# liuzuxin/FSRL

Measured on AMD Instinct MI355X. Metric: policy-updates/sec (PPO-Lagrangian update(), SafetyCarCircle-v0 shape, 256x256 MLP, 20k-step buffer), higher is better.
Workload: dtype f32; 1 GPU; configs[1] PPO-Lag update: repeat 4, clip 0.5, KL stop off, batch 256, N=20000 (20x1000), obs 8/act 2, 256x256; seeds_per_gpu=1, parallelism=independent agents x1

## Files before the change

### fsrl_amd/_lib.py

```python
import ctypes as C
import os

_HERE = os.path.dirname(os.path.abspath(__file__))
LIB_PATH = os.environ.get("FSRL_HIP_LIB") or os.path.join(_HERE, "libfsrl_hip.so")

FSRL_OK, FSRL_EINVAL, FSRL_ENOMEM, FSRL_EHIP, FSRL_ESTATE = 0, -22, -12, -5, -1
PPO_NSTATS = 11
ALGO_PPO_LAG, ALGO_TRPO_LAG, ALGO_CPO, ALGO_SAC_LAG, ALGO_FOCOPS = 0, 1, 2, 3, 4


class Config(C.Structure):
    _fields_ = [("algo", C.c_int32), ("obs_dim", C.c_int32), ("act_dim", C.c_int32),
                ("hidden", C.c_int32), ("n_critics", C.c_int32), ("env_num", C.c_int32),
                ("buffer_size", C.c_int64), ("max_action", C.c_float), ("gamma", C.c_double),
                ("gae_lambda", C.c_double), ("eps_clip", C.c_float), ("dual_clip", C.c_float),
                ("vf_coef", C.c_float), ("max_grad_norm", C.c_float), ("target_kl", C.c_float),
                ("norm_adv", C.c_int32), ("use_lagrangian", C.c_int32), ("lr", C.c_float),
                ("beta1", C.c_float), ("beta2", C.c_float), ("adam_eps", C.c_float), ("recompute_adv", C.c_int32),
                ("unbounded", C.c_int32), ("rew_norm", C.c_int32), ("value_clip", C.c_int32),
                ("hidden1", C.c_int32), ("hidden2", C.c_int32),
                ("n_hidden", C.c_int32), ("hidden_sizes", C.c_int32 * 8), ("force_layered", C.c_int32)]


class ShmEnv(C.Structure):
# ... 11 lines not shown
                ("cost_limit", C.c_double)]


class SacConfig(C.Structure):
    _fields_ = [("actor_lr", C.c_float), ("critic_lr", C.c_float), ("alpha_lr", C.c_float), ("tau", C.c_float),
                ("alpha", C.c_float), ("target_entropy", C.c_float), ("n_step", C.c_int32),
                ("auto_alpha", C.c_int32), ("use_lagrangian", C.c_int32), ("deterministic", C.c_int32),
                ("exploration_sigma", C.c_float), ("actor_mean", C.c_int32)]


class FocopsConfig(C.Structure):
    _fields_ = [("actor_lr", C.c_float), ("critic_lr", C.c_float), ("l2_reg", C.c_float), ("delta", C.c_float),
                ("eta", C.c_float), ("tem_lambda", C.c_float), ("max_grad_norm", C.c_float)]


class CvpoConfig(C.Structure):
    _fields_ = [("actor_lr", C.c_float), ("critic_lr", C.c_float), ("tau", C.c_float), ("n_step", C.c_int32),
                ("double_critic", C.c_int32), ("sample_act_num", C.c_int32), ("estep_iter_num", C.c_int32),
                ("mstep_iter_num", C.c_int32), ("estep_kl", C.c_float), ("estep_dual_max", C.c_float),
                ("estep_dual_lr", C.c_float), ("mstep_kl_mu", C.c_float), ("mstep_kl_std", C.c_float),
                ("mstep_dual_max", C.c_float), ("mstep_dual_lr", C.c_float), ("qc_thres", C.c_double),
                ("actor_mean", C.c_int32)]


class DevEnvConfig(C.Structure):
    _fields_ = [("kind", C.c_int32), ("env_num", C.c_int32), ("obs_dim", C.c_int32), ("act_dim", C.c_int32),
                ("max_episode_steps", C.c_int32), ("seed", C.c_uint64), ("p", C.c_float * 8), ("A", C.c_void_p), ("B", C.c_void_p)]


DEVENV_POINT_CIRCLE, DEVENV_LINEAR = 0, 1

ACTOR_MEAN_DEFAULT, ACTOR_MEAN_UNBOUNDED, ACTOR_MEAN_TANH = 0, 1, 2


def actor_mean_code(unbounded):
    if unbounded is None:
        return ACTOR_MEAN_DEFAULT
    return ACTOR_MEAN_UNBOUNDED if bool(unbounded) else ACTOR_MEAN_TANH


CPO_NSTATS, TRPO_NSTATS, SAC_NSTATS, FOCOPS_NSTATS, CVPO_NSTATS = 17, 11, 10, 8, 17

_P = C.POINTER
_f, _d, _u8, _i32, _i64 = _P(C.c_float), _P(C.c_double), _P(C.c_uint8), _P(C.c_int32), _P(C.c_int64)
_ctx = C.c_void_p

SIGNATURES = {
    "fsrl_last_error": (C.c_char_p, []),
    "fsrl_config_default": (None, [_P(Config)]),
    "fsrl_ctx_create": (C.c_int, [C.c_int, _P(Config), _P(_ctx)]),
    "fsrl_ctx_destroy": (C.c_int, [_ctx]),
    "fsrl_sync": (C.c_int, [_ctx]),
    "fsrl_param_count": (C.c_int64, [_ctx]),
    "fsrl_params_set": (C.c_int, [_ctx, _f, C.c_int64]),
    "fsrl_params_get": (C.c_int, [_ctx, _f, C.c_int64]),
    "fsrl_grads_get": (C.c_int, [_ctx, _f, C.c_int64]),
    "fsrl_optim_reset": (C.c_int, [_ctx]),
    "fsrl_state_snapshot": (C.c_int, [_ctx]),
    "fsrl_state_restore": (C.c_int, [_ctx]),
    "fsrl_train_state_size": (C.c_int64, [_ctx, C.c_int32]),
    "fsrl_train_state_export": (C.c_int, [_ctx, C.c_int32, C.c_void_p, C.c_int64, _i64]),
    "fsrl_train_state_import": (C.c_int, [_ctx, C.c_void_p, C.c_int64]),
    "fsrl_train_state_copy": (C.c_int, [_ctx, _ctx, C.c_int32]),
    "fsrl_ret_rms_get": (C.c_int, [_ctx, _d, C.c_int32]),
    "fsrl_ret_rms_set": (C.c_int, [_ctx, _d, C.c_int32]),
    "fsrl_set_lr": (C.c_int, [_ctx, C.c_int32, C.c_float]),
    "fsrl_get_lr": (C.c_float, [_ctx, C.c_int32]),
    "fsrl_ppo_abort": (C.c_int, [_ctx]),
    "fsrl_store_push": (C.c_int, [_ctx, _i32, C.c_int32, _f, _f, _d, _d, _u8, _u8, _f, _i64, _d, _i32, _i64]),
    "fsrl_store_reset": (C.c_int, [_ctx, C.c_int]),
    "fsrl_store_len": (C.c_int64, [_ctx]),
    "fsrl_store_read": (C.c_int, [_ctx, _i64, C.c_int64, _f, _f, _d, _d, _u8, _u8, _f]),
    "fsrl_store_configure": (C.c_int, [_ctx, C.c_int64, C.c_int32]),
    "fsrl_store_geometry": (C.c_int, [_ctx, _i64, _i32]),
    "fsrl_store_sample0": (C.c_int, [_ctx, _i64, C.c_int64, _i64]),
    "fsrl_actor_forward": (C.c_int, [_ctx, _f, C.c_int32, _f, _f]),
    "fsrl_ppo_begin": (C.c_int, [_ctx, _d, C.c_double, C.c_int32, _i64]),
    "fsrl_ppo_pass": (C.c_int, [_ctx, _i64, C.c_uint64, _i32]),
    "fsrl_ppo_pass_result": (C.c_int, [_ctx, _i32]),
    "fsrl_ppo_end": (C.c_int, [_ctx, _f, C.c_int64, _i64]),
    "fsrl_ppo_update": (C.c_int, [_ctx, _d, C.c_double, C.c_int32, C.c_int32, _i64, C.c_uint64, _f,
                                  C.c_int64, _i64, _i32]),
    "fsrl_ppo_set_plan": (C.c_int, [_ctx, C.c_int32]),
    "fsrl_batch_get": (C.c_int, [_ctx, C.c_char_p, _f, C.c_int64]),
    "fsrl_group_create": (C.c_int, [_P(_ctx), C.c_int32, _P(_ctx)]),
    "fsrl_group_destroy": (C.c_int, [_ctx]),
    "fsrl_group_set_plan": (C.c_int, [_ctx, C.c_int32]),
    "fsrl_group_ppo_update": (C.c_int, [_ctx, _d, _d, C.c_int32, C.c_int32, _P(_i64), C.c_uint64, _P(_f), C.c_int64, _i64,
                                        _i32]),
    "fsrl_group_ppo_update_each": (C.c_int, [_ctx, _d, _d, _i32, _i32, _P(_i64), C.c_uint64, _P(_f), _i64, _i64, _i32]),
    "fsrl_group_collect_step": (C.c_int, [_ctx, _i32, _i32, _f, _f, _d, _d, _u8, _u8, _f, _i64, _d, _i32, _i64, _i32, _f, C.c_int32,
                                          C.c_int32, _f, _f, _f, _f]),
    "fsrl_group_actor_set_resident": (C.c_int, [_ctx, C.c_int32, C.c_double]),
    "fsrl_group_actor_resident_stats": (C.c_int, [_ctx, _i64]),
    "fsrl_group_actor_release": (C.c_int, [_ctx]),
    "fsrl_sac_group_create": (C.c_int, [_P(_ctx), C.c_int32, _P(_ctx)]),
    "fsrl_sac_group_destroy": (C.c_int, [_ctx]),
    "fsrl_sac_group_update": (C.c_int, [_ctx, C.c_int32, _i32, _d, _d]),
    "fsrl_cvpo_group_create": (C.c_int, [_P(_ctx), C.c_int32, _P(_ctx)]),
    "fsrl_cvpo_group_destroy": (C.c_int, [_ctx]),
    "fsrl_cvpo_group_update": (C.c_int, [_ctx, C.c_int32, _i32]),
    "fsrl_collect_group_create": (C.c_int, [_P(_ctx), C.c_int32, _P(_ctx)]),
    "fsrl_collect_group_destroy": (C.c_int, [_ctx]),
    "fsrl_collect_group_step": (C.c_int, [_ctx, _i32, _i32, _f, _f, _d, _d, _u8, _u8, _f, _i64, _d, _i32, _i64, _i32, _f, C.c_int32,
                                          C.c_int32, _f, _f, _f, _f]),
    "fsrl_collect_group_actor_set_resident": (C.c_int, [_ctx, C.c_int32, C.c_double]),
    "fsrl_collect_group_actor_resident_stats": (C.c_int, [_ctx, _i64]),
    "fsrl_collect_group_actor_release": (C.c_int, [_ctx]),
    "fsrl_group_collect_episodes": (C.c_int, [_ctx, _P(_P(ShmEnv)), _i32, _i32, _f, _i32, C.c_int32, C.c_int32, _f, _f, _i64, _d, _i32,
                                              _i32, _d, _i32, _i32, _d, _i32]),
    "fsrl_collect_episodes_group": (C.c_int, [_ctx, _P(_P(ShmEnv)), _i32, _i32, _f, _i32, C.c_int32, C.c_int32, _f, _f, _i64, _d, _i32,
                                              _i32, _d, _i32, _i32, _d, _i32]),
    "fsrl_gae_return": (C.c_int, [_ctx, _f, _f, _d, _u8, C.c_int64, C.c_double, C.c_double, _d]),
    "fsrl_nstep_return": (C.c_int, [_ctx, _d, _u8, C.c_int64, _f, _i64, C.c_int64, C.c_int64, C.c_double, C.c_int32, _d]),
    "fsrl_launch_floors": (C.c_int, [_ctx, C.c_int32, C.c_int32, _d]),
    "fsrl_tr_begin": (C.c_int, [_ctx, _P(TrConfig), _i64]),
    "fsrl_cpo_learn": (C.c_int, [_ctx, C.c_double, C.c_int32, _f]),
    "fsrl_trpo_learn": (C.c_int, [_ctx, _d, C.c_double, C.c_int32, _f]),
    "fsrl_cpo_learn_mb": (C.c_int, [_ctx, C.c_double, C.c_int32, C.c_int32, _i64, C.c_uint64, _f, C.c_int64, _i64]),
    "fsrl_trpo_learn_mb": (C.c_int, [_ctx, _d, C.c_double, C.c_int32, C.c_int32, _i64, C.c_uint64, _f, C.c_int64, _i64]),
    "fsrl_tr_linesearch_evals": (C.c_int32, [_ctx, _i32, C.c_int32]),
    "fsrl_actor_param_count": (C.c_int64, [_ctx]),
    "fsrl_tr_grad": (C.c_int, [_ctx, C.c_int32, _f, C.c_int64]),
    "fsrl_tr_hvp": (C.c_int, [_ctx, _f, _f, C.c_int64]),
    "fsrl_tr_hvp_cached": (C.c_int, [_ctx, _f, _f, C.c_int64]),
    "fsrl_tr_cg": (C.c_int, [_ctx, _f, C.c_int64, C.c_float, C.c_int32, C.c_float, _f, _i32, _f]),
    "fsrl_tr_eval": (C.c_int, [_ctx, _d]),
    "fsrl_tr_set_plan": (C.c_int, [_ctx, C.c_int32, C.c_int32, C.c_int32]),
    "fsrl_tr_set_tile_split": (C.c_int, [_ctx, C.c_int32, C.c_int32]),
    "fsrl_tr_set_co_delay": (C.c_int, [_ctx, C.c_int32, C.c_int32]),
    "fsrl_focops_init": (C.c_int, [_ctx, _P(FocopsConfig)]),
    "fsrl_focops_set_plan": (C.c_int, [_ctx, C.c_int32]),
    "fsrl_focops_set_nu": (C.c_int, [_ctx, C.c_double, C.c_double]),
    "fsrl_sac_init": (C.c_int, [_ctx, _P(SacConfig)]),
    "fsrl_sac_set_plan": (C.c_int, [_ctx, C.c_int32]),
    "fsrl_sac_param_count": (C.c_int64, [_ctx, C.c_int32]),
    "fsrl_sac_params_set": (C.c_int, [_ctx, _f, C.c_int64, _f, C.c_int64, C.c_float]),
    "fsrl_sac_params_put": (C.c_int, [_ctx, C.c_int32, _f, C.c_int64]),
    "fsrl_sac_params_get": (C.c_int, [_ctx, C.c_int32, _f, C.c_int64, _f]),
    "fsrl_sac_update": (C.c_int, [_ctx, C.c_int32, _i64, _f, _f, C.c_uint64, _d, C.c_double, _f]),
    "fsrl_actor_sample": (C.c_int, [_ctx, _f, C.c_int32, C.c_int32, C.c_uint64, _f]),
    "fsrl_collect_step": (C.c_int, [_ctx, _i32, C.c_int32, _f, _f, _d, _d, _u8, _u8, _f, _i64, _d, _i32, _i64,
                                    _f, C.c_int32, C.c_int32, C.c_int32, _f, _f, _f, _f]),
    "fsrl_collect_episodes": (C.c_int, [_ctx, _P(ShmEnv), _i32, C.c_int32, _f, C.c_int32, C.c_int32, C.c_int32, _f, _f, _i64, _d, _i32,
                                        _i32, _d, _i32, _i32]),
    "fsrl_collect_episodes_split": (C.c_int, [_ctx, _P(ShmEnv), _i32, C.c_int32, _f, C.c_int32, C.c_int32, C.c_int32, _f, _f, _i64, _d, _i32,
                                              _i32, _d, _i32, _i32]),
    "fsrl_collect_timing": (C.c_int, [_ctx, _d]),
    "fsrl_actor_set_resident": (C.c_int, [_ctx, C.c_int32, C.c_double]),
    "fsrl_actor_resident_stats": (C.c_int, [_ctx, _i64]),
    "fsrl_actor_release": (C.c_int, [_ctx]),
    "fsrl_collect_run": (C.c_int, [_ctx, _P(ShmEnv), _i32, C.c_int32, _f, _f, _f, C.c_int32, C.c_int32, _f, _f, C.c_int32, _i32, _d, _d, _d,
                                  _u8, _u8, _f]),
    "fsrl_store_sizes": (C.c_int, [_ctx, _i64, C.c_int32]),
    "fsrl_sac_stats_drain": (C.c_int64, [_ctx, _f, C.c_int64]),
    "fsrl_sac_last_sample": (C.c_int, [_ctx, _i64, _f, _f, C.c_int32]),
    "fsrl_sac_last_chain": (C.c_int, [_ctx, _i64, _u8, C.c_int32]),
    "fsrl_per_enable": (C.c_int, [_ctx, C.c_double, C.c_double, C.c_int32]),
    "fsrl_per_set_beta": (C.c_int, [_ctx, C.c_double]),
    "fsrl_per_update_weight": (C.c_int, [_ctx, _i64, _d, C.c_int64]),
    "fsrl_per_state": (C.c_int, [_ctx, _d, C.c_int64, _d, _d, _d]),
    "fsrl_per_last_weights": (C.c_int, [_ctx, _f, C.c_int32]),
    "fsrl_per_last_td": (C.c_int, [_ctx, _f, C.c_int32]),
    "fsrl_sac_actor_forward": (C.c_int, [_ctx, _f, C.c_int32, _f, _f]),
    "fsrl_cvpo_init": (C.c_int, [_ctx, _P(CvpoConfig)]),
    "fsrl_cvpo_pre_update": (C.c_int, [_ctx]),
# ... 76 lines not shown
```

### fsrl_amd/csrc/common.hpp

```cpp
#pragma once
#include <hip/hip_runtime.h>
#include <stdint.h>

#include "../../include/fsrl_hip.h"

#define FSRL_MAX_NETS (1 + FSRL_MAX_CRITICS)
#define FSRL_TILE_M 16
#define FSRL_DOW 32
#define FSRL_MAX_OBS 128
#define FSRL_MAX_ACT 16
#define FSRL_W1_LDS 16
#define FSRL_RD 64
#define FSRL_RD_LOGP 16
#define FSRL_RD_ADV 17
#define FSRL_RD_RET 21
#define FSRL_RD_VOLD 25
#define FSRL_RD_MEAN 32
#define FSRL_RD_STD 48

typedef float f32x4 __attribute__((ext_vector_type(4)));
typedef float f32x2 __attribute__((ext_vector_type(2)));

struct NetOff {
    int sigma;
    int W1, b1, W2, b2, W3, b3;
    int W2f;
    int out;
    int begin, end;
};

struct ModelDesc {
    int Do, Da, H, n_nets;
    int unbounded;
    NetOff net[FSRL_MAX_NETS];
};

__host__ __device__ __forceinline__ int w2f_index(int H, int n, int k) {
    return ((((n >> 4) * (H >> 4) + (k >> 4)) * 64) + ((k >> 2) & 3) * 16 + (n & 15)) * 4 + (k & 3);
}
__device__ __forceinline__ int w2f_mirror_of(const ModelDesc& md, int i) {
    const int HH = md.H * md.H;
    for (int net = 0; net < md.n_nets; ++net) {
        const int o = i - md.net[net].W2;
        if ((unsigned)o < (unsigned)HH) return md.net[net].W2f + w2f_index(md.H, o / md.H, o % md.H);
    }
    return -1;
}

struct PpoStepArgs {
    int mb_start;
    int mb_size;
    int step;
    int mb_index;
    int last_in_pass;
    int first_in_pass;
    int iters_in_pass;
    int pass;
    float rescale;
    float lam[FSRL_MAX_CRITICS];
    float eps_clip, dual_clip, vf_coef, max_action, max_grad_norm, target_kl;
    int norm_adv, use_lagrangian;
    float lr, beta1, beta2, adam_eps;
    float one_minus_b1, one_minus_b2;
    double kl_thresh;
    float step_size;
    float bc2_sqrt;
    int value_clip;
    int fuse_adam;
    int xcd_pair;
    int dbg_phase;
};
#ifdef FSRL_PROBES
#define FSRL_PROBE(sa, n) ((sa).dbg_phase == (n))
#define FSRL_TS(buf, k) do { if ((buf) && threadIdx.x == 0) (buf)[(size_t)blockIdx.x * 16 + (k)] = __builtin_readcyclecounter(); } while (0)
#else
#define FSRL_PROBE(sa, n) false
#define FSRL_TS(buf, k) do { } while (0)
#endif

__device__ __forceinline__ void ppo_adam_math(const float g, float& m, float& v, float& p, const PpoStepArgs& sa) {
#pragma clang fp contract(off)
    m = fmaf(sa.one_minus_b1, g - m, m);
    v = v * sa.beta2;
    v = fmaf(sa.one_minus_b2 * g, g, v);
    const float denom = sqrtf(v) / sa.bc2_sqrt + sa.adam_eps;
    p = p + (-sa.step_size * m) / denom;
}

struct CtrlBlock {
    int stopped_after;
    int pad;
    double kl_sum;
    float last_grad_norm;
    float pad2;
};

__device__ __forceinline__ f32x4 mfma_16x16x4(float a, float b, f32x4 c) {
    return __builtin_amdgcn_mfma_f32_16x16x4f32(a, b, c, 0, 0, 0);
}

__device__ __forceinline__ f32x4 mfma_4x4x1(float a, float b, f32x4 c) {
    return __builtin_amdgcn_mfma_f32_4x4x1f32(a, b, c, 0, 0, 0);
}

__device__ __forceinline__ void store4_next(float* p, const f32x4 v) {
    asm volatile("global_store_dwordx4 %0, %1, off sc1\n\ts_nop 1" ::"v"(p), "v"(v) : "memory");
}
#ifdef FSRL_FB_PLAIN_STORES
__device__ __forceinline__ void store4_fb(float* p, const f32x4 v) { *reinterpret_cast<f32x4*>(p) = v; }
#else
__device__ __forceinline__ void store4_fb(float* p, const f32x4 v) { store4_next(p, v); }
#endif

__host__ __device__ __forceinline__ unsigned div_magic(const int d) { return d > 1 ? 0xFFFFFFFFu / (unsigned)d + 1u : 0u; }
__device__ __forceinline__ int div_by_magic(const unsigned e, const unsigned magic) { return magic ? (int)__umulhi(e, magic) : (int)e; }

#ifndef WG3_NO_BUFFER
typedef unsigned wg3_u32x4 __attribute__((ext_vector_type(4)));
struct Wg3Buf { __amdgpu_buffer_rsrc_t r; };
__device__ __forceinline__ Wg3Buf wg3_buf(const float* base) {
    Wg3Buf b; b.r = __builtin_amdgcn_make_buffer_rsrc(const_cast<float*>(base), 0, 0x7FFFFFFF, 0x00020000); return b;
}
__device__ __forceinline__ Wg3Buf wg3_buf_here(const float* base) {
    unsigned long long p = (unsigned long long)base;
    asm volatile("" : "+s"(p));
    return wg3_buf(reinterpret_cast<const float*>(p));
}
__device__ __forceinline__ f32x4 wg3_ld4(const Wg3Buf& b, const unsigned off_floats) {
    return __builtin_bit_cast(f32x4, __builtin_amdgcn_raw_buffer_load_b128(b.r, off_floats * 4u, 0, 0));
}
__device__ __forceinline__ float wg3_ld1(const Wg3Buf& b, const unsigned off_floats) {
    return __builtin_bit_cast(float, __builtin_amdgcn_raw_buffer_load_b32(b.r, off_floats * 4u, 0, 0));
}
__device__ __forceinline__ float wg3_ld1s(const Wg3Buf& b, const unsigned lane_off_floats, const unsigned uni_off_floats) {
    return __builtin_bit_cast(float, __builtin_amdgcn_raw_buffer_load_b32(b.r, lane_off_floats * 4u, uni_off_floats * 4u, 0));
}
__device__ __forceinline__ f32x4 wg3_ld4s(const Wg3Buf& b, const unsigned lane_off_floats, const unsigned uni_off_floats) {
    return __builtin_bit_cast(f32x4, __builtin_amdgcn_raw_buffer_load_b128(b.r, lane_off_floats * 4u, uni_off_floats * 4u, 0));
}
#else
struct Wg3Buf { const float* p; };
__device__ __forceinline__ Wg3Buf wg3_buf(const float* base) { Wg3Buf b; b.p = base; return b; }
__device__ __forceinline__ Wg3Buf wg3_buf_here(const float* base) { return wg3_buf(base); }
__device__ __forceinline__ f32x4 wg3_ld4(const Wg3Buf& b, const unsigned off_floats) { return *reinterpret_cast<const f32x4*>(b.p + off_floats); }
__device__ __forceinline__ float wg3_ld1(const Wg3Buf& b, const unsigned off_floats) { return b.p[off_floats]; }
__device__ __forceinline__ float wg3_ld1s(const Wg3Buf& b, const unsigned l, const unsigned u) { return b.p[l + u]; }
__device__ __forceinline__ f32x4 wg3_ld4s(const Wg3Buf& b, const unsigned l, const unsigned u) { return *reinterpret_cast<const f32x4*>(b.p + l + u); }
#endif

__device__ __forceinline__ float wave_sum(float v) {
#pragma unroll
    for (int o = 32; o > 0; o >>= 1) v += __shfl_xor(v, o, 64);
    return v;
}

__device__ __forceinline__ double wave_sum_d(double v) {
#pragma unroll
    for (int o = 32; o > 0; o >>= 1) v += __shfl_xor(v, o, 64);
    return v;
}
```

### fsrl_amd/csrc/fsrl_hip.hip

```cpp
#include <hip/hip_runtime.h>

#include <climits>
#include <cstddef>
#include <cmath>
#include <cstdarg>
#include <cstdio>
#include <cstdlib>
#include <cstring>
#include <algorithm>
#include <functional>
#include <string>
#include <vector>

#include "kernels_misc.hpp"
#include "kernels_mlp.hpp"
#include "kernels_fb.hpp"
#include "kernels_fbco.hpp"
#include "kernels_wgrad2.hpp"
#include "kernels_wgrad3.hpp"
#include "kernels_layered.hpp"
#include "kernels_focops_group.hpp"
#include "resident_ring.hpp"
#include "host_decisions.hpp"

static thread_local std::string g_err;
static int fail(int code, const char* fmt, ...) {
    char buf[512];
    va_list ap;
    va_start(ap, fmt);
    vsnprintf(buf, sizeof(buf), fmt, ap);
    va_end(ap);
    g_err = buf;
    return code;
}
#define HIPCHK(expr)                                                                        \
    do {                                                                                    \
        hipError_t _e = (expr);                                                             \
        if (_e != hipSuccess)                                                               \
            return fail(FSRL_EHIP, "%s failed: %s (%s:%d)", #expr, hipGetErrorString(_e),   \
                        __FILE__, __LINE__);                                                \
    } while (0)
#define CHECK_ARG(cond, ...) \
    do { if (!(cond)) return fail(FSRL_EINVAL, __VA_ARGS__); } while (0)

extern "C" const char* fsrl_last_error(void) { return g_err.c_str(); }

static inline int round_up(int x, int m) { return (x + m - 1) / m * m; }

struct TensorMap {
    int api_off, dev_off, rows, cols, dev_ld;
    int n() const { return rows * cols; }
    void to_dev(float* dev, const float* api) const {
        for (int r = 0; r < rows; ++r) memcpy(dev + dev_off + (size_t)r * dev_ld, api + api_off + (size_t)r * cols, (size_t)cols * 4);
    }
    void to_api(float* api, const float* dev) const {
        for (int r = 0; r < rows; ++r) memcpy(api + api_off + (size_t)r * cols, dev + dev_off + (size_t)r * dev_ld, (size_t)cols * 4);
    }
};

struct EnvBook {
    int64_t index = 0, size = 0, last_index = 0;
    int64_t staged = 0;
    double ep_rew = 0.0;
    int32_t ep_len = 0;
    int64_t ep_idx = 0;
};

struct Staging {
    uint8_t* h = nullptr;
    uint8_t* d = nullptr;
    int count = 0;
    hipEvent_t done = nullptr;
    bool in_flight = false;
};
static inline size_t stage_rec_bytes(int Do, int Da) { return ((size_t)24 + 4 * (size_t)(2 * Do + Da) + 7) / 8 * 8; }

struct fsrl_group;
struct fsrl_ctx {
    fsrl_config cfg{};
    fsrl_group* group = nullptr;
    struct CommState* comm = nullptr;
    int device = 0;
    hipStream_t compute = nullptr, side = nullptr;
    ModelDesc md{};
    std::vector<TensorMap> tmap;
    int h1 = 0, h2 = 0;
    int64_t n_api = 0;
    int n_dev = 0;
    int n_alloc = 0;
    float *P = nullptr, *M = nullptr, *V = nullptr, *G = nullptr;
    int64_t adam_t = 0;
    CtrlBlock* ctrl = nullptr;
    CtrlBlock* h_ctrl = nullptr;
    bool verdict_pending = false;

    int64_t sub_size = 0, maxsize = 0;
    float* mbstat = nullptr; size_t mbstat_cap = 0;
    double* d_rms = nullptr;
    double* ret64 = nullptr; int64_t ret64_cap = 0;
    int64_t alloc_rows = 0;
    int active_envs = 0;
    std::vector<EnvBook> env;
    std::vector<uint8_t> h_flags;
    StorePtrs st{};
    static constexpr int STAGE_CAP = 4096;
    Staging stage[2];
    int cur_stage = 0;
    hipEvent_t store_ready = nullptr;

    BatchPtrs b{};
    int* d_indices = nullptr; uint8_t* d_end = nullptr; int* d_seg = nullptr;
    int* h_indices = nullptr; uint8_t* h_end = nullptr; int* h_seg = nullptr;
    float *values = nullptr, *vnext = nullptr, *advs = nullptr, *rets = nullptr, *logp_old = nullptr;
    int64_t N = 0;
    int n_seg = 0;
    bool batch_ready = false;

    int batch_size = 0, mbp_max = 0, n_tiles_max = 0;
    float *A1 = nullptr, *A2 = nullptr, *D1 = nullptr, *D2 = nullptr, *DO = nullptr;
    float *obs_p = nullptr, *rd_p = nullptr;
    float *statp = nullptr, *gsq_part = nullptr;
    int *d_perm = nullptr, *h_perm = nullptr;
    int *d_mbstart = nullptr, *d_mbsize = nullptr, *h_mbplan = nullptr;
    size_t mb_cap = 0;
    std::vector<int> mb_start, mb_size;
    float* d_stats = nullptr; int64_t stats_cap = 0;
    int64_t n_steps = 0;
    int pass_index = 0;
    double lagr[FSRL_MAX_CRITICS] = {0, 0, 0, 0};
    double rescaling = 1.0;
    bool in_update = false;

    void* scratch = nullptr; size_t scratch_bytes = 0;

    bool profiling = false;
    hipEvent_t ev_a = nullptr, ev_b = nullptr, ev_c = nullptr;
    std::vector<hipEvent_t> k_ev;
    size_t k_ev_used = 0;
    double t_process_ms = 0, t_learn_ms = 0, t_fwdbwd_ms = 0, t_fwdbwd_raw_ms = 0;
    int64_t n_fwdbwd = 0;
    uint64_t rng[4] = {0x9E3779B97F4A7C15ull, 0xBF58476D1CE4E5B9ull, 0x94D049BB133111EBull, 1};
    uint64_t shuffle_rng[4] = {0xD6E8FEB86659FD93ull, 0xA0761D6478BD642Full, 0xE7037ED1A0B428DBull, 2};
    struct Parts { int stride = 0; float* p = nullptr; size_t floats = 0; } parts[3];
    float* wg_parts = nullptr;
    int n_cus = 256;
    bool wgrad_xcd = false;
    bool wgrad_stream = false;
    int wgrad_tiles = 1;
    struct FocState* foc = nullptr;
    float* mu_old = nullptr;
    float* sigma_old = nullptr;
    void* h_actor = nullptr; size_t h_actor_bytes = 0;
    int actor_k = 0; size_t actor_ob = 0, actor_mb = 0;
    unsigned* h_done = nullptr; int done_cap = 0;
    unsigned actor_seq = 0; int actor_blocks = 0;
    ResidentRing pa;
    bool pa_req = false;
    int pa_cap = 0;
    void* h_pa = nullptr;
    int probe_phase = 0, probe_wgrad_skip = 0;
    unsigned long long* probe_ts = nullptr;
    bool probe_tile16 = false;
    struct fsrl_sac_group* sac_group = nullptr;
    struct fsrl_cvpo_group* cvpo_group = nullptr;
    struct fsrl_collect_group* cgroup = nullptr;
    int tall_tiles = -1;
    bool no_fuse_adam = false;
    bool no_w2b_early = false;
    bool no_xcd_pair = false;
    bool no_spin = false;
    std::vector<float> act_mu, act_sg;
    std::vector<int> perm_tmp;
    hipEvent_t perm_copied = nullptr; bool perm_in_flight = false;
    uint64_t store_version = 1;
    uint64_t joined_version = 0;
    double t_collect_env = 0.0, t_collect_act = 0.0;
    float* snap = nullptr;
    int64_t snap_adam_t = 0, snap_critic_t = 0, snap_foc_a = 0, snap_foc_c = 0; bool snap_valid = false;
    struct LayState* lay = nullptr;
    struct TrState* tr = nullptr;
    uint64_t theta_version = 1;
    void* sac = nullptr;
    struct fsrl_tap* tap = nullptr;
    struct PerState* per = nullptr;
};
static bool ctx_is_replay(const fsrl_ctx* c);
static void sac_free(fsrl_ctx* c);
static void tr_free(fsrl_ctx* c);
static void foc_free(fsrl_ctx* c);
static void tr_reset_optim(fsrl_ctx* c);
static int64_t tr_critic_steps_taken(fsrl_ctx* c);
static void tr_set_critic_steps(fsrl_ctx* c, int64_t t);
static void foc_steps(fsrl_ctx* c, int64_t* t_actor, int64_t* t_critic, bool set);
static void foc_reset_optim(fsrl_ctx* c);
static void group_detach(fsrl_ctx* c);
static void lay_free(fsrl_ctx* c);
static void lay_build_layout(fsrl_ctx* c, const int* widths, int L);
static int lay_ensure_mb(fsrl_ctx* c, int B);
static int lay_ppo_steps(fsrl_ctx* c);
struct InferArgs;
static int lay_infer(fsrl_ctx* c, const InferArgs& ia, int jobs_y, hipStream_t s);
static void comm_free(fsrl_ctx* c);
static inline bool tap_closed(const fsrl_ctx* c, int e);
static void tap_row(fsrl_ctx* c, int e, int i, const float* act, double rew, double cost, uint8_t fl);
static int tap_flush(fsrl_ctx* c, int w, const uint8_t* recs_d, int stage_rec, int k);
static void tap_ctx_gone(fsrl_ctx* c);
static int per_ingest(fsrl_ctx* c, const uint8_t* recs_d, int rec, int k);
static int per_store_reset(fsrl_ctx* c);
static void per_free(fsrl_ctx* c);
static int focops_pass(fsrl_ctx* c, int32_t* stopped_out);
static int pass_verdict(fsrl_ctx* c, int32_t* stopped_out);

static int flush_stage(fsrl_ctx* c);
static void pactor_release(fsrl_ctx* c);
static void group_actor_release(fsrl_group* g);
static void sac_group_detach(fsrl_ctx* c);
static void cvpo_group_detach(fsrl_ctx* c);
static void collect_group_detach(fsrl_ctx* c);
static void collect_group_actor_release(struct fsrl_collect_group* g);
static int focops_group_check(fsrl_ctx* const* ctxs, int k);
struct GroupUpdate;
static int focops_group_update(GroupUpdate& u);
#define ENTER_DEV(c) do { HIPCHK(hipSetDevice((c)->device)); pactor_release(c); } while (0)

static int join_store(fsrl_ctx* c) {
    if (c->joined_version == c->store_version) return 0;
    int rc = flush_stage(c);
    if (rc) return rc;
    HIPCHK(hipEventRecord(c->store_ready, c->side));
    HIPCHK(hipStreamWaitEvent(c->compute, c->store_ready, 0));
    c->joined_version = c->store_version;
    return 0;
}

static int ensure_scratch(fsrl_ctx* c, size_t bytes) {
    if (c->scratch_bytes >= bytes) return 0;
    if (c->scratch) HIPCHK(hipFree(c->scratch));
    c->scratch = nullptr; c->scratch_bytes = 0;
    HIPCHK(hipMalloc(&c->scratch, bytes));
    c->scratch_bytes = bytes;
    return 0;
}

template <class T>
struct DevTable { T *d = nullptr, *h = nullptr; size_t cap = 0; };
template <class T>
static int table_ensure(DevTable<T>& t, size_t need, size_t grow_to, hipStream_t sync = nullptr) {
    if (need <= t.cap) return 0;
    if (sync) HIPCHK(hipStreamSynchronize(sync));
    if (t.d) HIPCHK(hipFree(t.d));
    if (t.h) HIPCHK(hipHostFree(t.h));
// ... 101 lines not shown
        wa.out = c->wg_parts; wa.split_stride = stride; wa.ks_per_split = rps / 4;
        *nsplit = ns;
        hipLaunchKernelGGL((fb_wgrad2_kernel<256, PAIR2>), dim3(8 * WG2_Q * ((ns + 7) / 8), ny), dim3(1024), 0, c->compute, md, wa, ns, rps);
        HIPCHK(hipGetLastError());
        return 0;
    }
    const WgradBlocks wb = wgrad_blocks(md.Do, H_, PAIR2);
    const int passes = wb.passes, NB = wb.NB;
    const WgradPlan pl = wgrad_plan(wa.rows, NB * ny, c->n_cus);
    int rc = ensure_parts(c, stride, pl.nsplit);
    if (rc) return rc;
    wa.out = c->wg_parts; wa.ks_per_split = pl.ks_per_split; wa.split_stride = stride;
    wa.dbg_skip = c->probe_wgrad_skip;
    wa.aux_passes = passes;
    *nsplit = pl.nsplit;
    return dispatch_H(c->cfg.hidden, [&](auto hc) {
        constexpr int HH = decltype(hc)::value;
        if (xcd_order < 0 ? c->wgrad_xcd : xcd_order != 0) {
            wa.remap_total = NB * ny * pl.nsplit; wa.remap_ny = ny;
            hipLaunchKernelGGL((fb_wgrad_kernel<HH, PAIR2>), dim3(round_up(wa.remap_total, 8)), dim3(1024), 0, c->compute, md, wa, NoRider{});
        } else if (rider && !PAIR2) {
            const int blocks = (rider->sa.B + SG_ROWS - 1) / SG_ROWS;
            rider->x0 = NB; rider->nx = (blocks + ny * pl.nsplit - 1) / (ny * pl.nsplit);
            hipLaunchKernelGGL((fb_wgrad_kernel<HH, false, SgRider>), dim3(NB + rider->nx, ny, pl.nsplit), dim3(1024), 0, c->compute, md, wa, *rider);
            if (rider_done) *rider_done = true;
        } else
        hipLaunchKernelGGL((fb_wgrad_kernel<HH, PAIR2>), dim3(NB, ny, pl.nsplit), dim3(1024), 0, c->compute, md, wa, NoRider{});
        HIPCHK(hipGetLastError());
        return 0;
    });
}

extern "C" void fsrl_config_default(fsrl_config* c) {
    memset(c, 0, sizeof(*c));
    c->algo = FSRL_ALGO_PPO_LAG;
    c->obs_dim = 8; c->act_dim = 2; c->hidden = 128; c->n_critics = 2;
    c->env_num = 20; c->buffer_size = 100000; c->max_action = 1.0f;
    c->gamma = 0.99; c->gae_lambda = 0.95; c->eps_clip = 0.2f; c->dual_clip = 0.0f;
    c->vf_coef = 0.25f; c->max_grad_norm = 0.0f; c->target_kl = 0.02f;
    c->norm_adv = 1; c->use_lagrangian = 1;
    c->lr = 5e-4f; c->beta1 = 0.9f; c->beta2 = 0.999f; c->adam_eps = 1e-8f;
}

static void build_layout(fsrl_ctx* c) {
    const int Do = c->cfg.obs_dim, Da = c->cfg.act_dim, H = c->cfg.hidden;
    ModelDesc& md = c->md;
    md.Do = Do; md.Da = Da; md.H = H; md.n_nets = 1 + c->cfg.n_critics;
    md.unbounded = (c->cfg.unbounded && c->cfg.algo != FSRL_ALGO_SAC_LAG) ? 1 : 0;
    const int h1 = c->h1, h2 = c->h2;
    int api = 0, dev = 0;
    auto add = [&](int rows, int cols, int dev_ld, int dev_n) {
        TensorMap t{api, dev, rows, cols, dev_ld};
        c->tmap.push_back(t);
        api += rows * cols;
        dev = round_up(dev + dev_n, 64);
        return t.dev_off;
    };
    for (int net = 0; net < md.n_nets; ++net) {
        NetOff& no = md.net[net];
        no.begin = dev;
        const int out = (net == 0) ? Da : 1;
        no.out = out;
        no.sigma = (net == 0) ? add(1, Da, Da, Da) : -1;
        no.W1 = add(h1, Do, Do, H * Do); no.b1 = add(1, h1, H, H);
        no.W2 = add(h2, h1, H, H * H);   no.b2 = add(1, h2, H, H);
        no.W3 = add(out, h2, H, out * H); no.b3 = add(1, out, out, out);
        no.end = dev;
    }
    c->n_api = api;
    c->n_dev = round_up(dev, 1024);
    for (int net = 0; net < md.n_nets; ++net) md.net[net].W2f = c->n_dev + net * H * H;
    c->n_alloc = c->n_dev + md.n_nets * H * H;
}

static void fill_mirrors(const ModelDesc& md, std::vector<float>& v) {
    const int H = md.H;
    for (int net = 0; net < md.n_nets; ++net) {
        const NetOff& no = md.net[net];
        for (int n = 0; n < H; ++n)
            for (int k = 0; k < H; ++k) v[(size_t)no.W2f + w2f_index(H, n, k)] = v[(size_t)no.W2 + (size_t)n * H + k];
    }
}

extern "C" int fsrl_ctx_destroy(fsrl_ctx* c) {
    if (!c) return 0;
    (void)hipSetDevice(c->device);
    pactor_release(c);
    (void)hipDeviceSynchronize();
    if (c->group) group_detach(c);
    if (c->sac_group) sac_group_detach(c);
    if (c->cvpo_group) cvpo_group_detach(c);
    if (c->cgroup) collect_group_detach(c);
    if (c->tap) tap_ctx_gone(c);
    comm_free(c);
    tr_free(c);
    sac_free(c);
    per_free(c);
    foc_free(c);
    lay_free(c);
    if (c->h_actor) (void)hipHostFree(c->h_actor);
    if (c->h_done) (void)hipHostFree(c->h_done);
    if (c->h_pa) (void)hipHostFree(c->h_pa);
    if (c->mbstat) (void)hipFree(c->mbstat);
    if (c->d_rms) (void)hipFree(c->d_rms);
    if (c->ret64) (void)hipFree(c->ret64);
    if (c->mu_old) (void)hipFree(c->mu_old);
    if (c->sigma_old) (void)hipFree(c->sigma_old);
    if (c->snap) (void)hipFree(c->snap);
    void* dptrs[] = {c->P, c->M, c->V, c->G, c->ctrl, c->st.obs, c->st.obs_next, c->st.act, c->st.rew,
                     c->st.cost, c->st.flags, c->b.obs, c->b.obs_next, c->b.act, c->b.rew, c->b.cost,
                     c->b.flags, c->d_indices, c->d_end, c->d_seg, c->values, c->vnext, c->advs,
                     c->rets, c->logp_old, c->A1, c->A2, c->D1, c->D2, c->DO, c->obs_p, c->rd_p, c->statp,
                     c->gsq_part, c->d_perm, c->d_mbstart, c->d_mbsize, c->d_stats,
                     c->scratch};
    for (void* p : dptrs) if (p) (void)hipFree(p);
    for (auto& pp : c->parts) if (pp.p) (void)hipFree(pp.p);
    void* hptrs[] = {c->h_ctrl, c->h_indices, c->h_end, c->h_seg, c->h_perm, c->h_mbplan};
    for (void* p : hptrs) if (p) (void)hipHostFree(p);
    for (auto& s : c->stage) {
        if (s.h) (void)hipHostFree(s.h);
        if (s.d) (void)hipFree(s.d);
        if (s.done) (void)hipEventDestroy(s.done);
    }
    for (hipEvent_t e : {c->store_ready, c->ev_a, c->ev_b, c->ev_c, c->perm_copied}) if (e) (void)hipEventDestroy(e);
    for (hipEvent_t e : c->k_ev) (void)hipEventDestroy(e);
    if (c->compute) (void)hipStreamDestroy(c->compute);
    if (c->side) (void)hipStreamDestroy(c->side);
    delete c;
    return 0;
}

extern "C" int fsrl_ctx_create(int device_id, const fsrl_config* cfg, fsrl_ctx** out) {
    CHECK_ARG(cfg && out, "null argument");
    CHECK_ARG(cfg->algo == FSRL_ALGO_PPO_LAG || cfg->algo == FSRL_ALGO_SAC_LAG || cfg->algo == FSRL_ALGO_CPO ||
                  cfg->algo == FSRL_ALGO_TRPO_LAG || cfg->algo == FSRL_ALGO_FOCOPS, "unknown algo %d", cfg->algo);
    CHECK_ARG(cfg->obs_dim >= 1 && cfg->obs_dim <= FSRL_MAX_OBS, "obs_dim must be in [1,%d]", FSRL_MAX_OBS);
    CHECK_ARG(cfg->act_dim >= 1 && cfg->act_dim <= FSRL_MAX_ACT, "act_dim must be in [1,%d]", FSRL_MAX_ACT);
    CHECK_ARG(cfg->n_hidden >= 0 && cfg->n_hidden <= FSRL_MAX_HIDDEN, "n_hidden must be in [0, %d]", FSRL_MAX_HIDDEN);
    bool layered = false;
    int n_hid1 = cfg->hidden1, n_hid2 = cfg->hidden2;
    if (cfg->n_hidden > 0) {
        CHECK_ARG(cfg->hidden1 == 0 && cfg->hidden2 == 0, "give hidden_sizes[n_hidden] or hidden1 / hidden2, not both");
        for (int l = 0; l < cfg->n_hidden; ++l)
            CHECK_ARG(cfg->hidden_sizes[l] >= 1 && cfg->hidden_sizes[l] <= FSRL_MAX_WIDTH, "hidden_sizes[%d] = %d outside [1, %d]", l,
                      cfg->hidden_sizes[l], FSRL_MAX_WIDTH);
        if (cfg->n_hidden == 2 && cfg->hidden_sizes[0] <= 256 && cfg->hidden_sizes[1] <= 256 && !cfg->force_layered) {
            n_hid1 = cfg->hidden_sizes[0]; n_hid2 = cfg->hidden_sizes[1];
        } else {
            layered = true;
        }
    } else {
        CHECK_ARG(!cfg->force_layered, "force_layered needs hidden_sizes[n_hidden]");
    }
    const int h1_ = layered ? 0 : (n_hid1 > 0 ? n_hid1 : cfg->hidden), h2_ = layered ? 0 : (n_hid2 > 0 ? n_hid2 : cfg->hidden);
    if (!layered) {
        CHECK_ARG((n_hid1 > 0) == (n_hid2 > 0), "hidden1 and hidden2 are given together (0, 0 = two layers of `hidden`)");
        CHECK_ARG(h1_ >= 1 && h1_ <= 256 && h2_ >= 1 && h2_ <= 256, "hidden layer widths must be in [1, 256] (two hidden layers)");
    }
    const int Hpad_ = layered ? 0 : std::max(h1_, h2_) <= 64 ? 64 : std::max(h1_, h2_) <= 128 ? 128 : 256;
    CHECK_ARG(layered || n_hid1 == 0 || cfg->hidden == 0 || cfg->hidden == Hpad_ ,
              "hidden = %d does not fit hidden1 / hidden2 = %d / %d (leave hidden 0 or give %d)", cfg->hidden, h1_, h2_, Hpad_);
    CHECK_ARG(!layered || cfg->n_critics < 1 || cfg->n_critics > FSRL_MAX_CRITICS ||
                  (1 + cfg->n_critics) * (cfg->n_hidden + 1) + 1 <= LAY_MAX_JOBS,
              "layered context: (1 + n_critics) * (n_hidden + 1) + 1 = %d weight-gradient jobs exceed the job table of %d "
              "(n_critics = %d, n_hidden = %d)", (1 + cfg->n_critics) * (cfg->n_hidden + 1) + 1, LAY_MAX_JOBS, cfg->n_critics, cfg->n_hidden);
    CHECK_ARG(cfg->n_critics >= 1 && cfg->n_critics <= 2,
              "n_critics must be 1 or 2 (reward [+ one cost], get_metrics base_policy.py:377-382)");
    CHECK_ARG(cfg->env_num >= 1 && cfg->buffer_size >= cfg->env_num, "bad env_num/buffer_size");
    CHECK_ARG(cfg->gamma >= 0.0 && cfg->gamma <= 1.0, "discount factor should be in [0, 1].");
    CHECK_ARG(cfg->gae_lambda >= 0.0 && cfg->gae_lambda <= 1.0, "GAE lambda should be in [0, 1].");
    CHECK_ARG(cfg->dual_clip == 0.0f || cfg->dual_clip > 1.0f,
              "Dual-clip PPO parameter should greater than 1.0.");
    CHECK_ARG(cfg->buffer_size + cfg->env_num < (int64_t)INT_MAX / 2, "buffer too large for 32-bit slot ids");
    CHECK_ARG(cfg->rew_norm || !cfg->value_clip, "value clip is available only when `reward_normalization` is True");
    CHECK_ARG(!cfg->value_clip || cfg->algo == FSRL_ALGO_PPO_LAG, "value_clip is a PPO-Lagrangian option (ppo_lag.py:158-164)");
    CHECK_ARG(!cfg->rew_norm || cfg->algo != FSRL_ALGO_SAC_LAG, "reward_normalization acts on GAE returns: on-policy contexts only");
    int ndev = 0;
    HIPCHK(hipGetDeviceCount(&ndev));
    CHECK_ARG(device_id >= 0 && device_id < ndev, "device %d not present (%d devices)", device_id, ndev);
    HIPCHK(hipSetDevice(device_id));
    int n_cus_probe = 256;
    (void)hipDeviceGetAttribute(&n_cus_probe, hipDeviceAttributeMultiprocessorCount, device_id);
    fsrl_ctx* c = new fsrl_ctx();
    c->cfg = *cfg;
    c->cfg.hidden = Hpad_;
    c->h1 = h1_; c->h2 = h2_;
    c->device = device_id;
    c->n_cus = n_cus_probe > 0 ? n_cus_probe : 256;
    c->probe_tile16 = getenv("FSRL_TILE16") != nullptr;
    c->no_w2b_early = getenv("FSRL_NO_W2B_EARLY") != nullptr;
#ifdef FSRL_PROBES
    { const char* e = getenv("FSRL_DBG_PHASE"); c->probe_phase = e ? atoi(e) : 0; }
    { const char* e = getenv("FSRL_WGRAD_SKIP"); c->probe_wgrad_skip = e ? atoi(e) : 0; }
    c->no_spin = getenv("FSRL_NO_SPIN") != nullptr;
    c->no_xcd_pair = getenv("FSRL_NO_XCD_PAIR") != nullptr;
    c->no_fuse_adam = getenv("FSRL_NO_FUSE_ADAM") != nullptr;
    if (getenv("FSRL_TSTAMP")) {
        (void)hipMalloc(&c->probe_ts, 1024 * 16 * sizeof(unsigned long long));
        (void)hipMemset(c->probe_ts, 0, 1024 * 16 * sizeof(unsigned long long));
    }
#endif
    if (layered) lay_build_layout(c, cfg->hidden_sizes, cfg->n_hidden);
    else build_layout(c);
#define TRY(expr) do { hipError_t _e = (expr); if (_e != hipSuccess) { fail(FSRL_EHIP, "%s failed: %s", #expr, hipGetErrorString(_e)); fsrl_ctx_destroy(c); return FSRL_EHIP; } } while (0)
    TRY(hipStreamCreateWithFlags(&c->compute, hipStreamNonBlocking));
    TRY(hipStreamCreateWithFlags(&c->side, hipStreamNonBlocking));
    const size_t pb = (size_t)c->n_dev * sizeof(float);
    TRY(hipMalloc(&c->P, (size_t)c->n_alloc * sizeof(float))); TRY(hipMemsetAsync(c->P, 0, (size_t)c->n_alloc * sizeof(float), c->compute));
    TRY(hipMalloc(&c->M, pb)); TRY(hipMalloc(&c->V, pb)); TRY(hipMalloc(&c->G, pb));
    TRY(hipMemsetAsync(c->M, 0, pb, c->compute)); TRY(hipMemsetAsync(c->V, 0, pb, c->compute)); TRY(hipMemsetAsync(c->G, 0, pb, c->compute));
    TRY(hipMalloc(&c->ctrl, sizeof(CtrlBlock)));
    if (cfg->rew_norm) {
        TRY(hipMalloc(&c->d_rms, 3 * FSRL_MAX_CRITICS * sizeof(double)));
        double init[3 * FSRL_MAX_CRITICS];
        for (int i = 0; i < FSRL_MAX_CRITICS; ++i) { init[3 * i] = 0.0; init[3 * i + 1] = 1.0; init[3 * i + 2] = 0.0; }
        TRY(hipMemcpy(c->d_rms, init, sizeof(init), hipMemcpyHostToDevice));
    }
    TRY(hipHostMalloc(&c->h_ctrl, sizeof(CtrlBlock)));
    c->sub_size = (cfg->buffer_size + cfg->env_num - 1) / cfg->env_num;
    c->maxsize = c->sub_size * cfg->env_num;
    c->alloc_rows = c->maxsize + cfg->env_num; c->active_envs = cfg->env_num;
    c->env.resize(cfg->env_num);
    c->h_flags.assign((size_t)c->alloc_rows, 0);
    const size_t ms = (size_t)c->alloc_rows;
    const int Do = cfg->obs_dim, Da = cfg->act_dim;
    TRY(hipMalloc(&c->st.obs, ms * Do * 4)); TRY(hipMalloc(&c->st.obs_next, ms * Do * 4));
    TRY(hipMalloc(&c->st.act, ms * Da * 4)); TRY(hipMalloc(&c->st.rew, ms * 8));
    TRY(hipMalloc(&c->st.cost, ms * 8)); TRY(hipMalloc(&c->st.flags, ms));
    TRY(hipMalloc(&c->b.obs, ms * Do * 4)); TRY(hipMalloc(&c->b.obs_next, ms * Do * 4));
    TRY(hipMalloc(&c->b.act, ms * Da * 4)); TRY(hipMalloc(&c->b.rew, ms * 8));
    TRY(hipMalloc(&c->b.cost, ms * 8)); TRY(hipMalloc(&c->b.flags, ms));
    TRY(hipMalloc(&c->d_indices, ms * 4)); TRY(hipMalloc(&c->d_end, ms)); TRY(hipMalloc(&c->d_seg, (ms + 2) * 4));
    TRY(hipHostMalloc(&c->h_indices, ms * 4)); TRY(hipHostMalloc(&c->h_end, ms)); TRY(hipHostMalloc(&c->h_seg, (ms + 2) * 4));
    const int C = cfg->n_critics;
    TRY(hipMalloc(&c->values, ms * C * 4)); TRY(hipMalloc(&c->vnext, ms * C * 4));
    TRY(hipMalloc(&c->advs, ms * C * 4)); TRY(hipMalloc(&c->rets, ms * C * 4));
    TRY(hipMalloc(&c->logp_old, ms * 4));
    TRY(hipMalloc(&c->d_perm, ms * 4)); TRY(hipHostMalloc(&c->h_perm, ms * 4));
    TRY(hipMalloc(&c->obs_p, (ms + 32) * Do * 4)); TRY(hipMemsetAsync(c->obs_p, 0, (ms + 32) * Do * 4, c->compute));
    TRY(hipMalloc(&c->rd_p, (ms + 32) * FSRL_RD * 4)); TRY(hipMemsetAsync(c->rd_p, 0, (ms + 32) * FSRL_RD * 4, c->compute));
    TRY(hipStreamSynchronize(c->compute));
    for (auto& s : c->stage) {
        const size_t k = fsrl_ctx::STAGE_CAP;
        TRY(hipHostMalloc(&s.h, k * stage_rec_bytes(Do, Da)));
        TRY(hipMalloc(&s.d, k * stage_rec_bytes(Do, Da)));
        TRY(hipEventCreateWithFlags(&s.done, hipEventDisableTiming));
    }
    TRY(hipEventCreateWithFlags(&c->store_ready, hipEventDisableTiming));
    TRY(hipEventCreate(&c->ev_a)); TRY(hipEventCreate(&c->ev_b)); TRY(hipEventCreate(&c->ev_c));
    TRY(hipEventCreateWithFlags(&c->perm_copied, hipEventDisableTiming));
    CtrlBlock init{INT_MAX, 0, 0.0, 0.0f, 0.0f};
    TRY(hipMemcpy(c->ctrl, &init, sizeof(init), hipMemcpyHostToDevice));
#undef TRY
    *out = c;
    return 0;
}

extern "C" int fsrl_sync(fsrl_ctx* c) {
    CHECK_ARG(c, "null ctx");
    ENTER_DEV(c);
    HIPCHK(hipStreamSynchronize(c->side));
    HIPCHK(hipStreamSynchronize(c->compute));
    return 0;
}

extern "C" int64_t fsrl_param_count(const fsrl_ctx* c) { return c ? c->n_api : 0; }

static int copy_flat(fsrl_ctx* c, float* dev, float* host_out, const float* host_in, int64_t n) {
    CHECK_ARG(n == c->n_api, "expected %lld parameters, got %lld", (long long)c->n_api, (long long)n);
    ENTER_DEV(c);
    std::vector<float> tmp((size_t)c->n_dev, 0.0f);
    if (host_in) {
        for (const TensorMap& t : c->tmap) t.to_dev(tmp.data(), host_in);
// ... 831 lines not shown
```

### fsrl_amd/csrc/host_decisions.hpp

```cpp
#pragma once
#include <stdint.h>
#include <algorithm>
#include <cmath>
#include <functional>
#include <queue>
#include <vector>

static constexpr float CPO_EPS = 1e-8f;
static inline bool cpo_cost_solve_skipped(float bb, float c_value) { return bb <= CPO_EPS && c_value < 0; }
struct CpoDual { int ocase; float A, B, lam, nu; };
static inline CpoDual cpo_dual_solve(float s_q, float s_r, float s_s, float c_value, float delta, float bb) {
    const float EPS = CPO_EPS;
    float A = 0.f, B = 0.f, lam, nu;
    int ocase = 4;
    if (!cpo_cost_solve_skipped(bb, c_value)) {
        A = s_q - s_r * s_r / s_s;
        B = 2.0f * delta - c_value * c_value / s_s;
        if (c_value < 0 && B < 0) ocase = 3;
        else if (c_value < 0 && B >= 0) ocase = 2;
        else if (c_value >= 0 && B >= 0) ocase = 1;
        else ocase = 0;
    }
    if (ocase == 3 || ocase == 4) {
        lam = std::sqrt(s_q / (2.0f * delta));
// ... 31 lines not shown
    for (int bt = 0; bt < max_backtracks; ++bt) {
        ++r.evals;
        if (try_step(r.beta)) break;
        r.beta *= coeff;
    }
    return r;
}
struct TrpoSearch { float step; int evals; };
template <class Try>
static TrpoSearch trpo_line_search(float step, float coeff, int max_backtracks, Try&& try_step) {
    TrpoSearch r{step, 0};
    for (int i = 0; i < max_backtracks; ++i) {
        ++r.evals;
        if (try_step(r.step)) break;
        else if (i < max_backtracks - 1) r.step *= coeff;
        else r.step = 0.0f;
    }
    return r;
}

static inline void split_plan(int n, int B, std::vector<int>& st, std::vector<int>& sz) {
    st.clear(); sz.clear();
    const bool merge = (n % B) > 0;
    for (int i = 0; i < n; i += B) {
        if (merge && i + 2 * B >= n) { st.push_back(i); sz.push_back(n - i); break; }
        st.push_back(i); sz.push_back(std::min(B, n - i));
    }
}

static inline uint64_t rotl64(uint64_t x, int k) { return (x << k) | (x >> (64 - k)); }
static inline uint64_t xoshiro_next(uint64_t* s) {
    const uint64_t result = rotl64(s[1] * 5, 7) * 9, t = s[1] << 17;
    s[2] ^= s[0]; s[3] ^= s[1]; s[1] ^= s[2]; s[0] ^= s[3]; s[2] ^= t; s[3] = rotl64(s[3], 45);
    return result;
}
enum { PERM_OK = 0, PERM_RANGE, PERM_TWICE };
struct PermFill { int code, index; long long value; };
static inline PermFill perm_fill(int* out, int n, const int64_t* perm, uint64_t* rng, uint64_t seed) {
    if (perm) {
        std::vector<uint8_t> seen((size_t)n, 0);
        for (int i = 0; i < n; ++i) {
            if (!(perm[i] >= 0 && perm[i] < n)) return {PERM_RANGE, i, (long long)perm[i]};
            if (seen[(size_t)perm[i]]) return {PERM_TWICE, i, (long long)perm[i]};
            seen[(size_t)perm[i]] = 1;
            out[i] = (int)perm[i];
        }
        return {PERM_OK, 0, 0};
    }
    if (seed) { rng[0] ^= seed; rng[1] += seed * 0x9E3779B97F4A7C15ull; }
    for (int i = 0; i < n; ++i) out[i] = i;
    for (int i = n - 1; i > 0; --i) std::swap(out[i], out[(int)(xoshiro_next(rng) % (uint64_t)(i + 1))]);
    return {PERM_OK, 0, 0};
}

struct TileSplit { int n32, n16; };
static inline TileSplit mixed_split(int64_t N, int ny, int n_cus, double rho) {
    const int max32 = (int)((N + 31) / 32);
    double best = 1e300; int best32 = 0, best16 = (int)((N + 15) / 16);
    std::vector<double> cu((size_t)std::max(n_cus, 1));
    for (int n32 = 0; n32 <= max32; ++n32) {
        const int64_t rem = N - 32 * (int64_t)n32;
        const int n16 = rem > 0 ? (int)((rem + 15) / 16) : 0;
        if (n16 > 0 && n32 == max32) continue;
        std::fill(cu.begin(), cu.end(), 0.0);
        std::priority_queue<double, std::vector<double>, std::greater<double>> pq(cu.begin(), cu.end());
        double span = 0.0;
        for (int b = 0; b < ny * n32; ++b) { const double e = pq.top() + 1.0; pq.pop(); pq.push(e); span = std::max(span, e); }
        for (int b = 0; b < ny * n16; ++b) { const double e = pq.top() + rho; pq.pop(); pq.push(e); span = std::max(span, e); }
        if (span < best - 1e-9 || (std::fabs(span - best) <= 1e-9 && n32 > best32)) { best = span; best32 = n32; best16 = n16; }
    }
    return {best32, best16};
}
static inline void co_plan(int64_t N, int n_wgs, int* n32_out, int* n16_out) {
    const int64_t tail_rows = std::min<int64_t>(N, 16 * (int64_t)(n_wgs / 2));
    const int n32 = (int)((N - tail_rows) / 32);
    const int64_t rem = N - 32 * (int64_t)n32;
    *n32_out = n32; *n16_out = (int)((rem + 15) / 16);
}
static inline void forced_split(int64_t N, int want32, int* n32_out, int* n16_out) {
    const int n32 = (int)std::min<int64_t>(want32, N / 32);
    const int64_t rem = N - 32 * (int64_t)n32;
    *n32_out = n32; *n16_out = (int)((rem + 15) / 16);
}
```

### fsrl_amd/csrc/host_ppo.inc

```
static int launch_gae(fsrl_ctx* c);
static int perm_upload(fsrl_ctx* c, int n, const int64_t* perm, uint64_t seed) {
    c->perm_tmp.resize((size_t)n);
    const PermFill pf = perm_fill(c->perm_tmp.data(), n, perm, c->shuffle_rng, seed);
    CHECK_ARG(pf.code != PERM_RANGE, "perm[%d]=%lld out of range", pf.index, pf.value);
    CHECK_ARG(pf.code != PERM_TWICE, "perm is not a permutation: %lld appears twice", pf.value);
    if (c->perm_in_flight) { HIPCHK(hipEventSynchronize(c->perm_copied)); c->perm_in_flight = false; }
    memcpy(c->h_perm, c->perm_tmp.data(), (size_t)n * 4);
    HIPCHK(hipMemcpyAsync(c->d_perm, c->h_perm, (size_t)n * 4, hipMemcpyHostToDevice, c->compute));
    HIPCHK(hipEventRecord(c->perm_copied, c->compute));
    c->perm_in_flight = true;
    return 0;
}

static int ensure_ppo_buffers(fsrl_ctx* c, int B) {
    const int mbp = round_up(2 * B, 32);
    if (mbp <= c->mbp_max) return 0;
    HIPCHK(hipStreamSynchronize(c->compute));
    for (float** p : {&c->A1, &c->A2, &c->D1, &c->D2, &c->DO, &c->statp, &c->gsq_part})
        if (*p) { HIPCHK(hipFree(*p)); *p = nullptr; }
    const int H = c->cfg.hidden, nn = c->md.n_nets;
    const size_t act = (size_t)nn * mbp * H * 4;
    HIPCHK(hipMalloc(&c->A1, act)); HIPCHK(hipMalloc(&c->A2, act));
    HIPCHK(hipMalloc(&c->D1, act)); HIPCHK(hipMalloc(&c->D2, act));
    HIPCHK(hipMalloc(&c->DO, (size_t)nn * mbp * FSRL_DOW * 4));
    HIPCHK(hipMalloc(&c->statp, (size_t)(mbp / 4) * nn * 4 * 4));
    HIPCHK(hipMalloc(&c->gsq_part, (size_t)std::max(wg_grid(H, nn), c->n_dev / 256 + 2) * 4));
    c->mbp_max = mbp;
    c->n_tiles_max = mbp / 16;
    return 0;
}

extern "C" int fsrl_ppo_set_plan(fsrl_ctx* c, int32_t tall_tiles) {
    CHECK_ARG(c, "null ctx");
    CHECK_ARG(tall_tiles >= -1 && tall_tiles <= 4096, "tall_tiles: -1 (automatic), 0 (none) or a count");
    c->tall_tiles = tall_tiles;
    return 0;
}

extern "C" int fsrl_ppo_begin(fsrl_ctx* c, const double* lagrangians, double rescaling,
                              int32_t batch_size, int64_t* n_out) {
    CHECK_ARG(c, "null ctx");
    CHECK_ARG(batch_size >= 1, "batch_size must be >= 1");
    CHECK_ARG(!c->in_update, "fsrl_ppo_begin called twice without fsrl_ppo_end");
    ENTER_DEV(c);
    int rc = flush_stage(c);
    if (rc) return rc;
    HIPCHK(hipEventRecord(c->store_ready, c->side));
    HIPCHK(hipStreamWaitEvent(c->compute, c->store_ready, 0));
    const int C = c->cfg.n_critics;
    for (int i = 0; i < FSRL_MAX_CRITICS; ++i) c->lagr[i] = 0.0;
    if (c->cfg.use_lagrangian && C > 1) {
        CHECK_ARG(lagrangians, "lags and values length must be equal");
        for (int i = 0; i < C - 1; ++i) c->lagr[i] = lagrangians[i];
    }
    c->rescaling = rescaling;
    c->batch_size = batch_size;
    const int64_t n = sample0(c, c->h_indices, c->h_end);
    c->N = n;
    if (n_out) *n_out = n;
    c->n_steps = 0;
    c->pass_index = 0;
    c->in_update = true;
    c->verdict_pending = false;
    c->t_fwdbwd_ms = 0; c->n_fwdbwd = 0; c->k_ev_used = 0;
    CtrlBlock init{INT_MAX, 0, 0.0, 0.0f, 0.0f};
    *c->h_ctrl = init;
    hipStream_t s = c->compute;
    HIPCHK(hipMemcpyAsync(c->ctrl, c->h_ctrl, sizeof(CtrlBlock), hipMemcpyHostToDevice, s));
    if (n == 0) { c->batch_ready = true; return 0; }
    int nseg = 0;
    c->h_seg[nseg++] = 0;
    for (int64_t i = 0; i + 1 < n; ++i) if (c->h_end[i]) c->h_seg[nseg++] = (int)i + 1;
    c->h_seg[nseg] = (int)n;
    HIPCHK(hipEventRecord(c->ev_a, s));
    HIPCHK(hipMemcpyAsync(c->d_indices, c->h_indices, (size_t)n * 4, hipMemcpyHostToDevice, s));
    HIPCHK(hipMemcpyAsync(c->d_end, c->h_end, (size_t)n, hipMemcpyHostToDevice, s));
    HIPCHK(hipMemcpyAsync(c->d_seg, c->h_seg, (size_t)(nseg + 1) * 4, hipMemcpyHostToDevice, s));
    const int Do = c->cfg.obs_dim, Da = c->cfg.act_dim;
    {
        const size_t work = (size_t)n * (2 * Do + Da + 1);
        const int blocks = (int)std::min<size_t>(2048, (work + 255) / 256);
        hipLaunchKernelGGL(batch_gather_kernel, dim3(blocks), dim3(256), 0, s, c->st, c->b, c->d_indices,
                           c->d_end, (int)n, Do, Da);
        HIPCHK(hipGetLastError());
    }
    InferArgs ia{};
    ia.obs = c->b.obs; ia.obs_next = c->b.obs_next; ia.act = c->b.act; ia.flags = c->b.flags;
    ia.values = c->values; ia.vnext = c->vnext; ia.logp_old = c->logp_old; ia.mu_out = nullptr;
    if (c->cfg.algo == FSRL_ALGO_FOCOPS) {
        if (!c->mu_old) {
            HIPCHK(hipMalloc(&c->mu_old, (size_t)c->alloc_rows * Da * 4));
            HIPCHK(hipMalloc(&c->sigma_old, FSRL_MAX_ACT * 4));
        }
        ia.mu_out = c->mu_old;
        HIPCHK(hipMemcpyAsync(c->sigma_old, c->P + c->md.net[0].sigma, (size_t)Da * 4, hipMemcpyDeviceToDevice, s));
    }
    ia.N = (int)n; ia.C = C; ia.max_action = c->cfg.max_action;
    rc = launch_infer(c, ia, 2 * C + 1, s);
    if (rc) return rc;
    c->n_seg = nseg;
    rc = launch_gae(c);
    if (rc) return rc;
    HIPCHK(hipEventRecord(c->ev_b, s));
    split_plan((int)n, batch_size, c->mb_start, c->mb_size);
    const int bs_rows = (int)std::min<int64_t>(batch_size, std::max<int64_t>(n, 1));
    rc = c->lay ? lay_ensure_mb(c, bs_rows) : ensure_ppo_buffers(c, bs_rows);
    if (rc) return rc;
    const size_t nmb = c->mb_start.size();
    if (nmb > c->mb_cap) {
        HIPCHK(hipStreamSynchronize(s));
        if (c->d_mbstart) HIPCHK(hipFree(c->d_mbstart));
        if (c->d_mbsize) HIPCHK(hipFree(c->d_mbsize));
        if (c->h_mbplan) HIPCHK(hipHostFree(c->h_mbplan));
        c->d_mbstart = c->d_mbsize = nullptr; c->h_mbplan = nullptr;
        const size_t cap = nmb * 2;
        HIPCHK(hipMalloc(&c->d_mbstart, cap * 4)); HIPCHK(hipMalloc(&c->d_mbsize, cap * 4));
        HIPCHK(hipHostMalloc(&c->h_mbplan, cap * 2 * 4));
        c->mb_cap = cap;
    }
    memcpy(c->h_mbplan, c->mb_start.data(), nmb * 4);
    memcpy(c->h_mbplan + c->mb_cap, c->mb_size.data(), nmb * 4);
    HIPCHK(hipMemcpyAsync(c->d_mbstart, c->h_mbplan, nmb * 4, hipMemcpyHostToDevice, s));
    HIPCHK(hipMemcpyAsync(c->d_mbsize, c->h_mbplan + c->mb_cap, nmb * 4, hipMemcpyHostToDevice, s));
    c->batch_ready = true;
    return 0;
}


static int launch_gae(fsrl_ctx* c) {
    GaeArgs ga{};
    ga.values = c->values; ga.vnext = c->vnext; ga.rew = c->b.rew; ga.cost = c->b.cost; ga.flags = c->b.flags;
    ga.seg_start = c->d_seg; ga.advs = c->advs; ga.rets = c->rets; ga.adv64 = nullptr; ga.N = (int)c->N;
    ga.gamma = c->cfg.gamma; ga.gl = c->cfg.gamma * c->cfg.gae_lambda;
    if (c->cfg.rew_norm) {
        if (c->ret64_cap < c->N) {
            HIPCHK(hipStreamSynchronize(c->compute));
            if (c->ret64) HIPCHK(hipFree(c->ret64));
            c->ret64 = nullptr;
            HIPCHK(hipMalloc(&c->ret64, (size_t)c->cfg.n_critics * c->alloc_rows * 8));
            c->ret64_cap = c->alloc_rows;
        }
        ga.rms = c->d_rms; ga.ret64 = c->ret64;
    }
    hipLaunchKernelGGL(gae_kernel, dim3(c->n_seg, c->cfg.n_critics), dim3(64), 0, c->compute, ga);
    HIPCHK(hipGetLastError());
    if (c->cfg.rew_norm) {
        hipLaunchKernelGGL(ret_rms_update_kernel, dim3(c->cfg.n_critics), dim3(1024), 0, c->compute, c->ret64, c->d_rms,
                           (int)c->N);
        HIPCHK(hipGetLastError());
    }
    return 0;
}

static int ppo_recompute_advantages(fsrl_ctx* c) {
    const int C = c->cfg.n_critics;
    InferArgs ia{};
    ia.obs = c->b.obs; ia.obs_next = c->b.obs_next; ia.act = nullptr; ia.flags = c->b.flags;
    ia.values = c->values; ia.vnext = c->vnext; ia.logp_old = nullptr; ia.mu_out = nullptr;
    ia.N = (int)c->N; ia.C = C; ia.max_action = c->cfg.max_action;
    int rc = launch_infer(c, ia, 2 * C, c->compute);
    if (rc) return rc;
    return launch_gae(c);
}

static int ensure_stats(fsrl_ctx* c, int64_t steps) {
    if (steps <= c->stats_cap) return 0;
    int64_t cap = std::max<int64_t>(steps, c->stats_cap * 2);
    cap = std::max<int64_t>(cap, 1024);
    float* nw = nullptr;
    HIPCHK(hipMalloc(&nw, (size_t)cap * FSRL_PPO_NSTATS * 4));
    if (c->d_stats) {
        HIPCHK(hipStreamSynchronize(c->compute));
        HIPCHK(hipMemcpy(nw, c->d_stats, (size_t)c->stats_cap * FSRL_PPO_NSTATS * 4, hipMemcpyDeviceToDevice));
        HIPCHK(hipFree(c->d_stats));
    }
    c->d_stats = nw;
    c->stats_cap = cap;
    return 0;
}

static int ppo_pass_prepare(fsrl_ctx* c, const int64_t* perm, uint64_t seed) {
    const int n = (int)c->N;
    hipStream_t s = c->compute;
    const int C = c->cfg.n_critics;
    if (c->cfg.recompute_adv && c->pass_index > 0 &&
        (c->cfg.algo == FSRL_ALGO_PPO_LAG || c->cfg.algo == FSRL_ALGO_FOCOPS)) {
        int rc0 = ppo_recompute_advantages(c);
        if (rc0) return rc0;
    }
    int rc = perm_upload(c, n, perm, seed);
    if (rc) return rc;
    const int nmb = (int)c->mb_start.size();
    rc = ensure_stats(c, c->n_steps + nmb);
    if (rc) return rc;
    {
        PrepArgs pa{};
        pa.obs = c->b.obs; pa.act = c->b.act; pa.advs = c->advs; pa.rets = c->rets; pa.logp_old = c->logp_old;
        pa.perm = c->d_perm; pa.mb_start = c->d_mbstart; pa.mb_size = c->d_mbsize; pa.obs_p = c->obs_p;
        pa.rd_p = c->rd_p; pa.N = n; pa.C = C; pa.Do = c->cfg.obs_dim; pa.Da = c->cfg.act_dim;
        pa.norm_adv = c->cfg.norm_adv;
        pa.values = c->cfg.value_clip ? c->values : nullptr;
        pa.mean_old = (c->cfg.algo == FSRL_ALGO_FOCOPS) ? c->mu_old : nullptr; pa.sigma_old = c->sigma_old;
        if ((size_t)nmb > c->mbstat_cap) {
            HIPCHK(hipStreamSynchronize(s));
            if (c->mbstat) HIPCHK(hipFree(c->mbstat));
            c->mbstat = nullptr;
            HIPCHK(hipMalloc(&c->mbstat, (size_t)nmb * 2 * FSRL_MAX_CRITICS * 2 * sizeof(float)));
            c->mbstat_cap = (size_t)nmb * 2;
        }
        pa.mbstat = c->mbstat; pa.batch = c->mb_size[0]; pa.nmb = nmb;
        if (pa.norm_adv) hipLaunchKernelGGL(ppo_adv_stats_kernel, dim3(nmb), dim3(1024), 0, s, pa);
        hipLaunchKernelGGL(ppo_permute_rows_kernel, dim3((n + 63) / 64), dim3(256), 0, s, pa);
        HIPCHK(hipGetLastError());
    }
    return 0;
}

static PpoStepArgs ppo_base_args(const fsrl_ctx* c) {
    PpoStepArgs sa{};
    sa.rescale = (float)c->rescaling;
    for (int i = 0; i < FSRL_MAX_CRITICS; ++i) sa.lam[i] = (float)c->lagr[i];
    sa.eps_clip = c->cfg.eps_clip; sa.dual_clip = c->cfg.dual_clip; sa.vf_coef = c->cfg.vf_coef;
    sa.max_action = c->cfg.max_action; sa.max_grad_norm = c->cfg.max_grad_norm; sa.target_kl = c->cfg.target_kl;
    sa.norm_adv = c->cfg.norm_adv; sa.use_lagrangian = c->cfg.use_lagrangian;
    sa.value_clip = c->cfg.value_clip;
    sa.lr = c->cfg.lr; sa.beta1 = c->cfg.beta1; sa.beta2 = c->cfg.beta2; sa.adam_eps = c->cfg.adam_eps;
    sa.one_minus_b1 = (float)(1.0 - (double)c->cfg.beta1);
    sa.one_minus_b2 = (float)(1.0 - (double)c->cfg.beta2);
    sa.kl_thresh = 1.5 * (double)c->cfg.target_kl;
    sa.pass = c->pass_index;
    sa.dbg_phase = c->probe_phase;
    sa.fuse_adam = (c->cfg.max_grad_norm <= 0.0f && !c->no_fuse_adam) ? 1 : 0;
    return sa;
}

static PpoBatchPtrs ppo_batch_ptrs(const fsrl_ctx* c) {
    PpoBatchPtrs bp{};
    bp.obs_p = c->obs_p; bp.rd_p = c->rd_p; bp.A1 = c->A1; bp.A2 = c->A2; bp.D1 = c->D1; bp.D2 = c->D2;
    bp.DO = c->DO; bp.statp = c->statp; bp.mbp_max = c->mbp_max;
    bp.ts = c->probe_ts;
    return bp;
}
static WgradPtrs ppo_wgrad_ptrs(const fsrl_ctx* c) {
    WgradPtrs wp{};
    wp.A1 = c->A1; wp.A2 = c->A2; wp.D1 = c->D1; wp.D2 = c->D2; wp.DO = c->DO; wp.X = c->obs_p; wp.grad = c->G;
    wp.gsq_part = c->gsq_part; wp.ctrl = c->ctrl; wp.mbp_max = c->mbp_max; wp.P = c->P; wp.statp = c->statp;
    wp.Pw = c->P; wp.M = c->M; wp.V = c->V;
    return wp;
}
static void group_agent_common(const fsrl_ctx* c, GroupAgent& a) {
    memset(&a, 0, sizeof(a));
    a.P = c->P; a.Pw = c->P; a.M = c->M; a.V = c->V; a.G = c->G; a.ctrl = c->ctrl; a.n_dev = c->n_dev;
    a.rescale = (float)c->rescaling;
    for (int j = 0; j < FSRL_MAX_CRITICS; ++j) a.lam[j] = (float)c->lagr[j];
    const PpoStepArgs sa = ppo_base_args(c);
    GroupHyper& h = a.hp;
    h.eps_clip = sa.eps_clip; h.dual_clip = sa.dual_clip; h.vf_coef = sa.vf_coef; h.max_grad_norm = sa.max_grad_norm;
    h.target_kl = sa.target_kl; h.kl_thresh = sa.kl_thresh;
    h.norm_adv = sa.norm_adv; h.use_lagrangian = sa.use_lagrangian; h.value_clip = sa.value_clip;
    h.beta1 = sa.beta1; h.beta2 = sa.beta2; h.adam_eps = sa.adam_eps;
    h.one_minus_b1 = sa.one_minus_b1; h.one_minus_b2 = sa.one_minus_b2;
}
static PpoStepArgs group_base_args(const fsrl_ctx* c0) {
    const PpoStepArgs m0 = ppo_base_args(c0);
    PpoStepArgs sa{};
    sa.max_action = m0.max_action; sa.fuse_adam = m0.fuse_adam; sa.xcd_pair = m0.xcd_pair; sa.dbg_phase = m0.dbg_phase;
    return sa;
}

struct PpoTilePlan { bool rows4, rows8; int n32; };
static PpoTilePlan ppo_tile_plan(const fsrl_ctx* c0, int tiles, int nn, int n_act, int tall_tiles) {
    PpoTilePlan p{false, false, 0};
    if (c0->probe_tile16) return p;
    const size_t per16 = (size_t)tiles * nn * n_act, n_cus = (size_t)c0->n_cus;
    p.rows4 = per16 * 4 <= n_cus;
    p.rows8 = !p.rows4 && per16 * 2 <= n_cus;
    if (!p.rows4 && !p.rows8 && c0->cfg.hidden >= 128 && c0->md.Do <= TileSmem<256, 32>::XK)
        p.n32 = tall_tiles < 0 ? (per16 > n_cus ? tiles / 2 : 0) : std::min(tiles / 2, tall_tiles);
    return p;
}

extern "C" int fsrl_ppo_pass(fsrl_ctx* c, const int64_t* perm, uint64_t seed, int32_t* stopped_out) {
    CHECK_ARG(c, "null ctx");
    if (!c->in_update || !c->batch_ready) return fail(FSRL_ESTATE, "fsrl_ppo_pass before fsrl_ppo_begin");
    c->theta_version += 1;
    ENTER_DEV(c);
    if (stopped_out) *stopped_out = 0;
    const int n = (int)c->N;
    if (n == 0) return 0;
    hipStream_t s = c->compute;
    const int H = c->cfg.hidden, nn = c->md.n_nets;
    int rc = ppo_pass_prepare(c, perm, seed);
    if (rc) return rc;
    const int nmb = (int)c->mb_start.size();
    if (c->cfg.algo == FSRL_ALGO_FOCOPS) return focops_pass(c, stopped_out);
    if (c->lay) {
        rc = lay_ppo_steps(c);
        if (rc) return rc;
        c->n_steps += nmb;
        c->pass_index += 1;
        if (c->cfg.target_kl > 0.0f) return pass_verdict(c, stopped_out);
        return 0;
    }
    const PpoBatchPtrs bp = ppo_batch_ptrs(c);
    WgradPtrs wp = ppo_wgrad_ptrs(c);
    wp.stats = c->d_stats;
    const int nparts = wg_grid(H, nn);

    PpoStepArgs sa = ppo_base_args(c);
    sa.iters_in_pass = nmb;

    for (int mb = 0; mb < nmb; ++mb) {
        sa.mb_start = c->mb_start[mb]; sa.mb_size = c->mb_size[mb]; sa.mb_index = mb;
        sa.step = (int)c->n_steps + mb;
        sa.first_in_pass = (mb == 0); sa.last_in_pass = (mb == nmb - 1);
        c->adam_t += 1;
        const AdamStep as = adam_step(c->cfg.lr, c->cfg.beta1, c->cfg.beta2, c->adam_t);
        sa.step_size = as.step_size; sa.bc2_sqrt = as.bc2_sqrt;
        const int tiles = (sa.mb_size + 15) / 16;
        wp.X = c->obs_p + (size_t)sa.mb_start * c->cfg.obs_dim;
        const bool prof = c->profiling;
        if (prof) {
            while (c->k_ev.size() < c->k_ev_used + 3) {
                hipEvent_t e; HIPCHK(hipEventCreate(&e)); c->k_ev.push_back(e);
            }
            HIPCHK(hipEventRecord(c->k_ev[c->k_ev_used], s));
        }
        const PpoTilePlan tp = ppo_tile_plan(c, tiles, nn, 1, c->tall_tiles);
        const int n32 = tp.n32, stat_tiles = tp.rows4 ? tiles * 4 : tp.rows8 ? tiles * 2 : tiles;
        rc = dispatch_H(H, [&](auto hc) {
            constexpr int HH = decltype(hc)::value;
            sa.xcd_pair = (nn <= 4 && !c->no_xcd_pair) ? 1 : 0;
            auto fb_grid = [&](int nt) { return sa.xcd_pair ? dim3(8 * ((nt + 1) / 2)) : dim3(nt * nn); };
            const bool early = !c->no_w2b_early;
            if (tp.rows4 && early) hipLaunchKernelGGL((ppo_fwd_bwd_kernel<HH, 4, true>), fb_grid(tiles * 4), dim3(4 * HH), 0, s, c->P, c->md, bp, sa);
            else if (tp.rows4) hipLaunchKernelGGL((ppo_fwd_bwd_kernel<HH, 4>), fb_grid(tiles * 4), dim3(4 * HH), 0, s, c->P, c->md, bp, sa);
            else if (tp.rows8 && early) hipLaunchKernelGGL((ppo_fwd_bwd_kernel<HH, 8, true>), fb_grid(tiles * 2), dim3(4 * HH), 0, s, c->P, c->md, bp, sa);
            else if (tp.rows8) hipLaunchKernelGGL((ppo_fwd_bwd_kernel<HH, 8>), fb_grid(tiles * 2), dim3(4 * HH), 0, s, c->P, c->md, bp, sa);
            else if (n32 > 0) {
                if constexpr (HH >= 128)
                    hipLaunchKernelGGL((ppo_fwd_bwd_tall_kernel<HH>), dim3((tiles - n32) * nn), dim3(4 * HH), 0, s, c->P, c->md, bp, sa, n32, tiles - n32);
            } else hipLaunchKernelGGL((ppo_fwd_bwd_kernel<HH, 16>), fb_grid(tiles), dim3(4 * HH), 0, s, c->P, c->md, bp, sa);
            return 0;
        });
        if (rc) return rc;
        if (prof) {
            HIPCHK(hipEventRecord(c->k_ev[c->k_ev_used + 1], s));
            HIPCHK(hipEventRecord(c->k_ev[c->k_ev_used + 2], s));
            c->k_ev_used += 3;
        }
        const bool big = tiles * 16 > 512;
        if (big) {
            FbWgradArgs wa{};
            wgrad_fill_nets(wa, nn, 0, (size_t)H, (size_t)c->mbp_max, c->A1, c->A2, c->D1, c->D2, c->DO);
            wa.obs = wp.X; wa.rows = tiles * 16; wa.N = sa.mb_size;
            int nsplit = 1;
            rc = wgrad_launch<false>(c, c->md, wa, nn, c->n_dev, &nsplit);
            if (rc) return rc;
            const int nsum = (c->n_dev + 255) / 256;
            hipLaunchKernelGGL(fb_sum_parts_kernel, dim3(nsum), dim3(256), 0, s, c->G, c->wg_parts, 0, c->n_dev, nsplit, c->n_dev,
                               c->gsq_part);
            hipLaunchKernelGGL(ppo_stats_kernel, dim3(1), dim3(64), 0, s, c->md, wp, sa, stat_tiles);
            hipLaunchKernelGGL(adam_clip_kernel, dim3((c->n_dev + 4 * ADAM_NT - 1) / (4 * ADAM_NT)), dim3(ADAM_NT), 0, s, c->P, c->M,
                               c->V, c->G, c->gsq_part, nsum, c->n_dev, sa, c->ctrl, c->md);
            HIPCHK(hipGetLastError());
            continue;
        }
        rc = dispatch_H(H, [&](auto hc) {
            constexpr int HH = decltype(hc)::value;
            if (sa.fuse_adam) hipLaunchKernelGGL((ppo_wgrad_kernel<HH, false, true>), dim3(nparts), dim3(1024), 0, s, c->md, wp, tiles * 16, sa, stat_tiles);
            else hipLaunchKernelGGL((ppo_wgrad_kernel<HH, false, false>), dim3(nparts), dim3(1024), 0, s, c->md, wp, tiles * 16, sa, stat_tiles);
            return 0;
        });
        if (rc) return rc;
        if (!sa.fuse_adam)
            hipLaunchKernelGGL(adam_clip_kernel, dim3((c->n_dev + 4 * ADAM_NT - 1) / (4 * ADAM_NT)), dim3(ADAM_NT), 0, s, c->P, c->M, c->V, c->G,
                               c->gsq_part, nparts, c->n_dev, sa, c->ctrl, c->md);
        HIPCHK(hipGetLastError());
    }
    c->n_steps += nmb;
    c->pass_index += 1;
    if (c->cfg.target_kl > 0.0f) return pass_verdict(c, stopped_out);
    return 0;
}

static int pass_verdict(fsrl_ctx* c, int32_t* stopped_out) {
    HIPCHK(hipMemcpyAsync(c->h_ctrl, c->ctrl, sizeof(CtrlBlock), hipMemcpyDeviceToHost, c->compute));
    if (!stopped_out) { c->verdict_pending = true; return 0; }
    HIPCHK(hipStreamSynchronize(c->compute));
    if (c->h_ctrl->stopped_after != INT_MAX) *stopped_out = 1;
    return 0;
}

extern "C" int fsrl_ppo_pass_result(fsrl_ctx* c, int32_t* stopped_out) {
    CHECK_ARG(c && stopped_out, "null argument");
    if (!c->in_update) return fail(FSRL_ESTATE, "fsrl_ppo_pass_result outside an update");
    ENTER_DEV(c);
    if (c->verdict_pending) { HIPCHK(hipStreamSynchronize(c->compute)); c->verdict_pending = false; }
    const bool watched = c->cfg.target_kl > 0.0f || c->cfg.algo == FSRL_ALGO_FOCOPS;
    *stopped_out = (watched && c->pass_index > 0 && c->h_ctrl->stopped_after != INT_MAX) ? 1 : 0;
    return 0;
}

extern "C" int fsrl_ppo_end(fsrl_ctx* c, float* stats_out, int64_t cap_steps, int64_t* n_steps_out) {
    CHECK_ARG(c, "null ctx");
    if (!c->in_update) return fail(FSRL_ESTATE, "fsrl_ppo_end without fsrl_ppo_begin");
    ENTER_DEV(c);
    hipStream_t s = c->compute;
    HIPCHK(hipEventRecord(c->ev_c, s));
    if (stats_out && c->n_steps > 0) {
        CHECK_ARG(cap_steps >= c->n_steps, "stats_out holds %lld steps, need %lld", (long long)cap_steps,
                  (long long)c->n_steps);
        HIPCHK(hipMemcpyAsync(stats_out, c->d_stats, (size_t)c->n_steps * FSRL_PPO_NSTATS * 4,
                              hipMemcpyDeviceToHost, s));
    }
    HIPCHK(hipStreamSynchronize(s));
    if (n_steps_out) *n_steps_out = c->n_steps;
    c->in_update = false;
    if (c->N > 0) {
        float ms = 0;
        if (hipEventElapsedTime(&ms, c->ev_a, c->ev_b) == hipSuccess) c->t_process_ms = ms;
        if (hipEventElapsedTime(&ms, c->ev_b, c->ev_c) == hipSuccess) c->t_learn_ms = ms;
        double tot = 0;
        c->t_fwdbwd_raw_ms = 0;
        for (size_t i = 0; i + 2 < c->k_ev_used; i += 3) {
            float a = 0, b = 0;
            if (hipEventElapsedTime(&a, c->k_ev[i], c->k_ev[i + 1]) == hipSuccess &&
                hipEventElapsedTime(&b, c->k_ev[i + 1], c->k_ev[i + 2]) == hipSuccess)
            { tot += (double)a - 0.5 * (double)b; c->t_fwdbwd_raw_ms += (double)a; }
        }
        c->t_fwdbwd_ms = tot;
        c->n_fwdbwd = (int64_t)(c->k_ev_used / 3);
    }
    return 0;
}

extern "C" int fsrl_ppo_update(fsrl_ctx* c, const double* lagrangians, double rescaling,
                               int32_t batch_size, int32_t repeat, const int64_t* perms, uint64_t seed,
                               float* stats_out, int64_t cap_steps, int64_t* n_steps_out,
                               int32_t* stopped_pass_out) {
    CHECK_ARG(c, "null ctx");
    CHECK_ARG(repeat >= 0, "repeat must be >= 0");
    int64_t n = 0;
    int rc = fsrl_ppo_begin(c, lagrangians, rescaling, batch_size, &n);
    if (rc) return rc;
    if (stopped_pass_out) *stopped_pass_out = -1;
    for (int k = 0; k < repeat; ++k) {
        int32_t stopped = 0;
        rc = fsrl_ppo_pass(c, perms ? perms + (size_t)k * n : nullptr, seed ? seed + k : 0, &stopped);
        if (rc) { c->in_update = false; return rc; }
        if (stopped) { if (stopped_pass_out) *stopped_pass_out = k; break; }
    }
    return fsrl_ppo_end(c, stats_out, cap_steps, n_steps_out);
}

extern "C" int fsrl_batch_get(fsrl_ctx* c, const char* which, float* out, int64_t cap) {
    CHECK_ARG(c && which && out, "null argument");
    if (!c->batch_ready) return fail(FSRL_ESTATE, "no batch: call fsrl_ppo_begin first");
    ENTER_DEV(c);
    const int64_t n = c->N;
    const int C = c->cfg.n_critics;
    const float* src = nullptr;
    int cols = C;
    if (!strcmp(which, "values")) src = c->values;
    else if (!strcmp(which, "rets")) src = c->rets;
    else if (!strcmp(which, "advs")) src = c->advs;
    else if (!strcmp(which, "vnext")) src = c->vnext;
    else if (!strcmp(which, "logp_old")) { src = c->logp_old; cols = 1; }
    else return fail(FSRL_EINVAL, "unknown batch field '%s'", which);
    CHECK_ARG(cap >= n * cols, "out too small");
    HIPCHK(hipStreamSynchronize(c->compute));
    std::vector<float> tmp((size_t)n * cols);
    if (n) HIPCHK(hipMemcpy(tmp.data(), src, (size_t)n * cols * 4, hipMemcpyDeviceToHost));
    for (int64_t r = 0; r < n; ++r)
        for (int k = 0; k < cols; ++k) out[r * cols + k] = tmp[(size_t)k * n + r];
    return 0;
}
```

### fsrl_amd/csrc/kernels_misc.hpp

```cpp
#pragma once
#include "common.hpp"

struct StorePtrs {
    float* obs;
    float* obs_next;
    float* act;
    double* rew;
    double* cost;
    uint8_t* flags;
};

__global__ void store_scatter_kernel(StorePtrs st, const uint8_t* __restrict__ recs, const int rec, int k, int Do, int Da) {
    const int per = 2 * Do + Da + 1;
    for (int e = blockIdx.x * blockDim.x + threadIdx.x; e < k * per; e += gridDim.x * blockDim.x) {
        const int row = e / per, f = e - row * per;
        const uint8_t* r = recs + (size_t)row * rec;
        const size_t dst = (size_t)*reinterpret_cast<const int*>(r + 16);
        const float* x = reinterpret_cast<const float*>(r + 24);
        if (f < Do) st.obs[dst * Do + f] = x[f];
        else if (f < 2 * Do) st.obs_next[dst * Do + (f - Do)] = x[f];
        else if (f < 2 * Do + Da) st.act[dst * Da + (f - 2 * Do)] = x[f];
        else {
            st.rew[dst] = *reinterpret_cast<const double*>(r);
            st.cost[dst] = *reinterpret_cast<const double*>(r + 8);
// ... 149 lines not shown
        for (int w = 0; w < NW; ++w) t += sh[w];
        return t;
    };
    for (int c = 0; c < a.C; ++c) {
        const float* __restrict__ adv = a.advs + (size_t)c * a.N;
        double s = 0.0;
        for (int m = tid; m < n; m += NT) s += (double)adv[a.perm[st + m]];
        const double mean = block_sum(s) / (double)n;
        double q = 0.0;
        for (int m = tid; m < n; m += NT) {
            const double d = (double)adv[a.perm[st + m]] - mean;
            q += d * d;
        }
        const double var = block_sum(q) / (double)(n - 1);
        if (tid == 0) {
            a.mbstat[((size_t)mb * FSRL_MAX_CRITICS + c) * 2 + 0] = (float)mean;
            a.mbstat[((size_t)mb * FSRL_MAX_CRITICS + c) * 2 + 1] = (float)sqrt(var);
        }
    }
}

__global__ __launch_bounds__(256) void ppo_permute_rows_kernel(const PrepArgs a) {
    __shared__ int perm_s[64];
    __shared__ float mean_f[64][FSRL_MAX_CRITICS], sd_f[64][FSRL_MAX_CRITICS];
    const int tid = threadIdx.x;
    const int p0 = blockIdx.x * 64, nc = min(64, a.N - p0);
    if (tid < nc) {
        perm_s[tid] = a.perm[p0 + tid];
        const int mb = min((p0 + tid) / a.batch, a.nmb - 1);
        for (int c = 0; c < a.C; ++c) {
            mean_f[tid][c] = a.norm_adv ? a.mbstat[((size_t)mb * FSRL_MAX_CRITICS + c) * 2 + 0] : 0.0f;
            sd_f[tid][c] = a.norm_adv ? a.mbstat[((size_t)mb * FSRL_MAX_CRITICS + c) * 2 + 1] : 1.0f;
        }
    }
    __syncthreads();
    {
        const int f = tid & 63, mph = tid >> 6;
        const float* __restrict__ src = nullptr;
        int stride = 1, kind = 0;
        int cn = 0;
        float cst = 0.0f;
        if (f < a.Da) { src = a.act + f; stride = a.Da; }
        else if (f == FSRL_RD_LOGP) src = a.logp_old;
        else if (f >= FSRL_RD_ADV && f < FSRL_RD_ADV + a.C) { cn = f - FSRL_RD_ADV; src = a.advs + (size_t)cn * a.N; kind = 1; }
        else if (f >= FSRL_RD_RET && f < FSRL_RD_RET + a.C) src = a.rets + (size_t)(f - FSRL_RD_RET) * a.N;
        else if (a.values && f >= FSRL_RD_VOLD && f < FSRL_RD_VOLD + a.C) src = a.values + (size_t)(f - FSRL_RD_VOLD) * a.N;
        else if (a.mean_old && f >= FSRL_RD_MEAN && f < FSRL_RD_MEAN + a.Da) { src = a.mean_old + (f - FSRL_RD_MEAN); stride = a.Da; }
        else if (a.mean_old && f >= FSRL_RD_STD && f < FSRL_RD_STD + a.Da) cst = expf(a.sigma_old[f - FSRL_RD_STD]);
        float v[16];
#pragma unroll
        for (int u = 0; u < 16; ++u) {
            const int m = mph + 4 * u;
            v[u] = (src != nullptr && m < nc) ? src[(size_t)perm_s[min(m, nc - 1)] * stride] : cst;
        }
#pragma unroll
        for (int u = 0; u < 16; ++u) {
            const int m = mph + 4 * u;
            if (m < nc) {
                float x = v[u];
                if (kind == 1 && a.norm_adv) x = (x - mean_f[m][cn]) / sd_f[m][cn];
                a.rd_p[(size_t)(p0 + m) * FSRL_RD + f] = x;
            }
        }
    }
    for (int e = tid; e < nc * a.Do; e += 256) {
        const int m = e / a.Do, k = e - m * a.Do;
        a.obs_p[(size_t)(p0 + m) * a.Do + k] = a.obs[(size_t)perm_s[m] * a.Do + k];
    }
}

__global__ __launch_bounds__(256) void w2f_sync_kernel(float* __restrict__ P, const ModelDesc md) {
    const int H = md.H, q4 = H * H / 4;
    for (int e = blockIdx.x * 256 + threadIdx.x; e < md.n_nets * q4; e += gridDim.x * 256) {
        const int net = e / q4, g = e - net * q4;
        const int n = (4 * g) / H, k = (4 * g) - n * H;
        const f32x4 v = *reinterpret_cast<const f32x4*>(P + md.net[net].W2 + (size_t)n * H + k);
        *reinterpret_cast<f32x4*>(P + md.net[net].W2f + w2f_index(H, n, k)) = v;
    }
}

#ifndef ADAM_NT
#define ADAM_NT 256
#endif
__device__ __forceinline__ void adam_clip_body(float* __restrict__ P, float* __restrict__ M,
                                               float* __restrict__ V,
                                               const float* __restrict__ G,
                                               const float* __restrict__ gsq_part, int nparts,
                                               int n, const PpoStepArgs& sa,
                                               CtrlBlock* ctrl, const ModelDesc& md) {
    __shared__ double sh[ADAM_NT / 64];
    __shared__ float coef_s;
    const int tid = threadIdx.x;
    if (FSRL_PROBE(sa, 30)) return;
    const int i4 = (blockIdx.x * ADAM_NT + tid) * 4;
    f32x4 g = {0, 0, 0, 0}, m = g, v = g, p = g;
    if (i4 < n) {
        g = *reinterpret_cast<const f32x4*>(G + i4); m = *reinterpret_cast<const f32x4*>(M + i4);
        v = *reinterpret_cast<const f32x4*>(V + i4); p = *reinterpret_cast<const f32x4*>(P + i4);
    }
    float coef = 1.0f;
    if (sa.max_grad_norm > 0.0f) {
        double s = 0.0;
        for (int k = tid; k < nparts; k += ADAM_NT) s += (double)gsq_part[k];
        s = wave_sum_d(s);
        if ((tid & 63) == 0) sh[tid >> 6] = s;
        __syncthreads();
        if (tid == 0) {
            double tot = 0.0;
            for (int w = 0; w < ADAM_NT / 64; ++w) tot += sh[w];
            const float norm = sqrtf((float)tot);
            coef_s = fminf(sa.max_grad_norm / (norm + 1e-6f), 1.0f);
            if (blockIdx.x == 0) ctrl->last_grad_norm = norm;
        }
        __syncthreads();
        coef = coef_s;
    }
    if (i4 < n) {
#pragma unroll
        for (int e = 0; e < 4; ++e) {
            float me = m[e], ve = v[e], pe = p[e];
            ppo_adam_math(g[e] * coef, me, ve, pe, sa);
            m[e] = me; v[e] = ve; p[e] = pe;
        }
        store4_next(M + i4, m);
        store4_next(V + i4, v);
        store4_next(P + i4, p);
        const int mi = w2f_mirror_of(md, i4);
        if (mi >= 0) store4_next(P + mi, p);
    }
    if (sa.last_in_pass && blockIdx.x == 0 && tid == 0 && sa.target_kl > 0.0f) {
        const double mean_kl = ctrl->kl_sum / ((double)sa.iters_in_pass + 1e-7);
        if (mean_kl > sa.kl_thresh) ctrl->stopped_after = sa.pass;
    }
}

__global__ __launch_bounds__(ADAM_NT) void adam_clip_kernel(float* __restrict__ P, float* __restrict__ M,
                                                       float* __restrict__ V,
                                                       const float* __restrict__ G,
                                                       const float* __restrict__ gsq_part, int nparts,
                                                       int n, const PpoStepArgs sa,
                                                       CtrlBlock* ctrl, const ModelDesc md) {
    adam_clip_body(P, M, V, G, gsq_part, nparts, n, sa, ctrl, md);
}

struct NstepArgs {
    const double* metric;
    const uint8_t* end_flag;
    const float* target_q;
    const int64_t* indices;
    double* out;
    int64_t len;
    int bsz, q, n_step;
    double gamma;
};
__global__ __launch_bounds__(256) void nstep_return_kernel(const NstepArgs a) {
#pragma clang fp contract(off)
    const int b = blockIdx.x * blockDim.x + threadIdx.x;
    if (b >= a.bsz) return;
    int gammas = a.n_step;
    double ret = 0.0;
    for (int n = a.n_step - 1; n >= 0; --n) {
        const int64_t now = a.indices[(size_t)n * a.bsz + b];
        if (a.end_flag[now]) { gammas = n + 1; ret = 0.0; }
        const double t = a.gamma * ret;
        ret = a.metric[now] + t;
    }
    double gpow = 1.0;
    for (int i = 0; i < gammas; ++i) gpow = gpow * a.gamma;
    for (int j = 0; j < a.q; ++j) {
        const double prod = (double)a.target_q[(size_t)b * a.q + j] * gpow;
        a.out[(size_t)b * a.q + j] = prod + ret;
    }
}
```

### fsrl_amd/csrc/kernels_mlp.hpp

```cpp
#pragma once
#include <type_traits>
#include "common.hpp"

__host__ __device__ constexpr int tile_rows(int R) { return R > 16 ? R : 16; }

template <int H, int ROWS = 16>
struct TileSmem {
    static constexpr int LD = H + 4;
    static constexpr int XK = (ROWS > 16) ? 64 : FSRL_MAX_OBS;
    float xT[XK * ROWS];
    float h1[ROWS * LD];
    float h2[ROWS * LD];
    float d2[ROWS * LD];
    float out[ROWS * FSRL_MAX_ACT];
    float dout[ROWS * FSRL_DOW];
    float rd[ROWS * FSRL_RD];
    float st[ROWS * 4];
    float w3[FSRL_MAX_ACT * H];
    float b1[H], b2[H], b3[FSRL_MAX_ACT], sig[FSRL_MAX_ACT];
    float w1[H * FSRL_W1_LDS];
};

template <int H>
struct TileGeom {
// ... 846 lines not shown
        }
#pragma unroll
        for (int r = 0; r < 4; ++r) {
            acc[r] += __shfl_xor(acc[r], 16, 64);
            acc[r] += __shfl_xor(acc[r], 32, 64);
            if constexpr (R == 8) { acc8[r] += __shfl_xor(acc8[r], 16, 64); acc8[r] += __shfl_xor(acc8[r], 32, 64); }
        }
        FSRL_TS(bp.ts, 12);
        if (FSRL_PROBE(sa, 7)) { if (acc[0] == 123.f) bp.statp[1] = 1.f; return; }
        if (q == 0) {
            float* __restrict__ D1 = bp.D1 + (nb + row0) * H;
            const int col = wave * 16 + li;
#pragma unroll
            for (int r = 0; r < 4; ++r) {
                D1[(size_t)r * H + col] = (sm.h1[r * LD + col] > 0.0f) ? acc[r] : 0.0f;
                if constexpr (R == 8) D1[(size_t)(4 + r) * H + col] = (sm.h1[(4 + r) * LD + col] > 0.0f) ? acc8[r] : 0.0f;
            }
        }
    } else {
        f32x4 acc = {0.f, 0.f, 0.f, 0.f}, acc2 = {0.f, 0.f, 0.f, 0.f};
        const float* arow = &sm.d2[li * LD + 4 * q];
#pragma unroll
        for (int jc = 0; jc < H / 16; ++jc) {
            const f32x4 a = *reinterpret_cast<const f32x4*>(arow + 16 * jc);
#pragma unroll
            for (int s = 0; s < 4; ++s) acc = mfma_16x16x4(a[s], wb[jc][s], acc);
            if constexpr (R == 32) {
                const f32x4 a2 = *reinterpret_cast<const f32x4*>(arow + 16 * LD + 16 * jc);
#pragma unroll
                for (int s = 0; s < 4; ++s) acc2 = mfma_16x16x4(a2[s], wb[jc][s], acc2);
            }
        }
        if (FSRL_PROBE(sa, 7)) { if (acc[0] == 123.f) bp.statp[1] = 1.f; return; }
        float* __restrict__ D1 = bp.D1 + (nb + row0) * H;
        const int col = wave * 16 + li;
#pragma unroll
        for (int r = 0; r < 4; ++r) {
            const int i = 4 * q + r;
            D1[(size_t)i * H + col] = (sm.h1[i * LD + col] > 0.0f) ? acc[r] : 0.0f;
            if constexpr (R == 32) D1[(size_t)(16 + i) * H + col] = (sm.h1[(16 + i) * LD + col] > 0.0f) ? acc2[r] : 0.0f;
        }
    }
    FSRL_TS(bp.ts, 13);
}

template <int H, int R, bool W2B_EARLY = false>
__global__ __launch_bounds__(4 * H) void ppo_fwd_bwd_kernel(const float* __restrict__ P,
                                                           const ModelDesc md,
                                                           const PpoBatchPtrs bp,
                                                           const PpoStepArgs sa) {
    __shared__ TileSmem<H> sm;
    ppo_fwd_bwd_body<H, R, W2B_EARLY>(sm, P, md, bp, sa);
}

template <int H>
__device__ __forceinline__ void ppo_fwd_bwd_mixed(unsigned char* raw, const float* __restrict__ P, const ModelDesc& md,
                                                  const PpoBatchPtrs& bp, const PpoStepArgs& sa, const int n32, const int per_net) {
    static_assert(sizeof(TileSmem<H, 32>) >= sizeof(TileSmem<H, 16>), "the 16-row layout lives inside the 32-row one");
    const int net = (int)blockIdx.x / per_net, b = (int)blockIdx.x - net * per_net;
    const int row0 = b < n32 ? 32 * b : 32 * n32 + 16 * (b - n32);
    if (net >= md.n_nets || row0 >= ((sa.mb_size + 15) & ~15)) return;
    if (b < n32) ppo_fwd_bwd_body<H, 32>(*reinterpret_cast<TileSmem<H, 32>*>(raw), P, md, bp, sa, row0, net, row0 >> 4);
    else ppo_fwd_bwd_body<H, 16>(*reinterpret_cast<TileSmem<H, 16>*>(raw), P, md, bp, sa, row0, net, row0 >> 4);
}
template <int H>
__global__ __launch_bounds__(4 * H) void ppo_fwd_bwd_tall_kernel(const float* __restrict__ P, const ModelDesc md, const PpoBatchPtrs bp,
                                                                const PpoStepArgs sa, const int n32, const int per_net) {
    __shared__ __align__(16) unsigned char raw[sizeof(TileSmem<H, 32>)];
    ppo_fwd_bwd_mixed<H>(raw, P, md, bp, sa, n32, per_net);
}

struct WgradPtrs {
    const float* A1; const float* A2; const float* D1; const float* D2; const float* DO;
    const float* X;
    float* grad;
    float* gsq_part;
    CtrlBlock* ctrl;
    const float* P;
    const float* statp;
    float* stats;
    int mbp_max;
    float* Pw; float* M; float* V;
    float* gsq_net;
};

__device__ __forceinline__ void ppo_adam_elem(const WgradPtrs& wp, const PpoStepArgs& sa, const int i, const float g,
                                              const int mi = -1) {
    float m = wp.M[i], v = wp.V[i], p = wp.Pw[i];
    ppo_adam_math(g, m, v, p, sa);
    wp.M[i] = m; wp.V[i] = v; wp.Pw[i] = p;
    if (mi >= 0) wp.Pw[mi] = p;
}

__host__ __device__ constexpr int wg_blocks_per_net(int H) { return (H / 32) * (H / 32) + 2 * (H / 32); }
__host__ __device__ constexpr int wg_grid(int H, int n_nets) { return n_nets * wg_blocks_per_net(H) + n_nets + 1; }

#define WG_MAXU 8
#define AUX_MAXU 32

__device__ __forceinline__ void ppo_stats_finalize(const ModelDesc& md, const WgradPtrs& wp,
                                                   const PpoStepArgs& sa, int n_tiles, int lane) {
    const int nn = md.n_nets, C = nn - 1;
    float mine = 0.0f;
    {
        const int g = lane >> 4, fs = lane & 15;
        for (int t0 = 0; t0 < n_tiles; t0 += 32) {
            float v[8];
#pragma unroll
            for (int u = 0; u < 8; ++u) {
                const int t = t0 + g + 4 * u;
                v[u] = (fs < nn * 4 && t < n_tiles) ? wp.statp[(size_t)t * nn * 4 + fs] : 0.0f;
            }
#pragma unroll
            for (int u = 0; u < 8; ++u) mine += v[u];
        }
        mine += __shfl_xor(mine, 16, 64);
        mine += __shfl_xor(mine, 32, 64);
    }
    const float invB = 1.0f / (float)sa.mb_size;
    const float term = __shfl(mine, 0, 64), safety = __shfl(mine, 1, 64), kls = __shfl(mine, 2, 64);
    float vf[FSRL_MAX_CRITICS];
#pragma unroll
    for (int c = 0; c < FSRL_MAX_CRITICS; ++c) vf[c] = __shfl(mine, 4 * (c + 1), 64) * invB;
    if (lane == 0) {
        float ent = 0.0f;
        for (int d = 0; d < md.Da; ++d)
            ent += 1.4189385332046727f + logf(expf(wp.P[md.net[0].sigma + d]));
        const float actor_rew = -term * invB;
        const float actor_safety = sa.use_lagrangian ? safety * invB : 0.0f;
        const float actor_total = sa.rescale * (actor_rew + actor_safety);
        const float kl = kls * invB;
        float vf_total = 0.0f;
#pragma unroll
        for (int c = 0; c < FSRL_MAX_CRITICS; ++c)
            if (c < C) vf_total += vf[c];
        float* o = wp.stats + (size_t)sa.step * FSRL_PPO_NSTATS;
        o[0] = sa.rescale;
        o[1] = (sa.use_lagrangian && C > 1) ? sa.lam[0] : 0.0f;
        o[2] = actor_safety;
        o[3] = actor_rew;
        o[4] = actor_total;
        o[5] = kl;
        o[6] = vf[0];
        o[7] = (C > 1) ? vf[1] : 0.0f;
        o[8] = vf_total;
        o[9] = actor_total + sa.vf_coef * vf_total;
        o[10] = ent;
        wp.ctrl->kl_sum = (sa.first_in_pass ? 0.0 : wp.ctrl->kl_sum) + (double)kl;
    }
}

template <bool BIG, bool FUSE>
__device__ __forceinline__ void ppo_wgrad_extra_block(const ModelDesc& md, const WgradPtrs& wp, const int mbp, const PpoStepArgs& sa,
                                                      const int n_stat_tiles, float* red, const int e) {
    const int CH = BIG ? (mbp + 511) / 512 : 1;
    const int tid = threadIdx.x, lane = tid & 63, wave = tid >> 6;
    if (FSRL_PROBE(sa, 21)) return;
    const bool stats_here = FUSE ? (e == 0) : (e == md.n_nets);
    if (stats_here && wave == 0 && wp.stats) {
        ppo_stats_finalize(md, wp, sa, n_stat_tiles, lane);
        if (FUSE && lane == 0 && sa.last_in_pass && sa.target_kl > 0.0f) {
            const double mean_kl = wp.ctrl->kl_sum / ((double)sa.iters_in_pass + 1e-7);
            if (mean_kl > sa.kl_thresh) wp.ctrl->stopped_after = sa.pass;
        }
    }
    if (e == md.n_nets) {
        if (tid == 0) wp.gsq_part[blockIdx.x] = 0.0f;
        return;
    }
    float sqs = 0.0f;
    {
        const int net = e;
        const NetOff no = md.net[net];
        const float* __restrict__ DOn = wp.DO + (size_t)net * wp.mbp_max * FSRL_DOW;
        const int col = tid & 31, php = tid >> 5;
        float t = 0.0f;
        for (int ch = 0; ch < CH; ++ch) {
            float v[16];
            int rbase = 512 * ch;
            if constexpr (BIG) asm volatile("" : "+s"(rbase));
#pragma unroll
            for (int u = 0; u < 16; ++u) {
                const int r = rbase + php + 32 * u;
                v[u] = (r < mbp) ? DOn[(size_t)r * FSRL_DOW + col] : 0.0f;
            }
#pragma unroll
            for (int u = 0; u < 16; ++u) t += v[u];
        }
        __syncthreads();
        red[php * 33 + col] = t;
        __syncthreads();
        if (tid < 32) {
            float tot = 0.0f;
#pragma unroll
            for (int p2 = 0; p2 < 32; ++p2) tot += red[p2 * 33 + tid];
            if (tid < no.out) {
                wp.grad[no.b3 + tid] = tot; sqs = fmaf(tot, tot, sqs);
                if constexpr (FUSE) ppo_adam_elem(wp, sa, no.b3 + tid, tot);
            }
            if (no.sigma >= 0 && tid >= 16 && tid < 16 + md.Da) {
                wp.grad[no.sigma + tid - 16] = tot; sqs = fmaf(tot, tot, sqs);
                if constexpr (FUSE) ppo_adam_elem(wp, sa, no.sigma + tid - 16, tot);
            }
        }
    }
    if (wave == 0) {
        sqs = wave_sum(sqs);
        if (lane == 0) {
            wp.gsq_part[blockIdx.x] = sqs;
            if (wp.gsq_net) wp.gsq_net[e] = sqs;
        }
    }
}

template <int H, bool BIG, bool FUSE, int U, bool PA, bool PB>
__device__ __forceinline__ void ppo_wgrad_aux(const ModelDesc& md, const WgradPtrs& wp, const int mbp, const PpoStepArgs& sa,
                                              const NetOff& no, const float* __restrict__ A2, const float* __restrict__ D1,
                                              const float* __restrict__ D2, const float* __restrict__ DOb, const int j0,
                                              float* red, float& sq) {
    const int CH = BIG ? (mbp + 64 * U - 1) / (64 * U) : 1;
    const int tid = threadIdx.x, lane = tid & 63, wave = tid >> 6;
    const int c = lane & 15, q = lane >> 4;
    const int Do = md.Do, out = no.out;
    const int KS = mbp >> 2;
    const float* __restrict__ X = wp.X;
    for (int k0 = 0; k0 < (PA ? Do : 1); k0 += 16) {
        const bool first = (k0 == 0);
        f32x4 ax0 = {0, 0, 0, 0}, ax1 = {0, 0, 0, 0}, ad0 = {0, 0, 0, 0}, ad1 = {0, 0, 0, 0};
        f32x2 s1 = {0.f, 0.f}, s2 = {0.f, 0.f};
        for (int ch = 0; ch < CH; ++ch)
        for (int ub = 0; ub < U; ub += 4) {
            int sbase = 16 * U * ch + 16 * ub;
            if constexpr (BIG) asm volatile("" : "+s"(sbase));
            if (sbase + wave >= KS) break;
            f32x2 a1[4], a2[4], a3[4];
            float bx[4], bd[4];
#pragma unroll
            for (int u = 0; u < 4; ++u) {
                const int sidx = sbase + wave + 16 * u;
                a1[u] = f32x2{0.f, 0.f}; a2[u] = f32x2{0.f, 0.f}; a3[u] = f32x2{0.f, 0.f};
                bx[u] = 0.f; bd[u] = 0.f;
                if (sidx < KS) {
                    const size_t r = (size_t)(4 * sidx + q);
                    if constexpr (PA) {
                        a1[u] = *reinterpret_cast<const f32x2*>(D1 + r * H + j0 + 2 * c);
                        if (k0 + c < Do) bx[u] = X[r * Do + k0 + c];
                    }
                    if constexpr (PB) {
                        if (first) {
                            a2[u] = *reinterpret_cast<const f32x2*>(A2 + r * H + j0 + 2 * c);
                            a3[u] = *reinterpret_cast<const f32x2*>(D2 + r * H + j0 + 2 * c);
                            bd[u] = DOb[r * FSRL_DOW + c];
                        }
                    }
                }
            }
#pragma unroll
            for (int u = 0; u < 4; ++u) {
                if constexpr (PA) {
                    ax0 = mfma_16x16x4(a1[u][0], bx[u], ax0);
                    ax1 = mfma_16x16x4(a1[u][1], bx[u], ax1);
                    if (first) s1 += a1[u];
                }
                if constexpr (PB) {
                    if (first) {
                        ad0 = mfma_16x16x4(a2[u][0], bd[u], ad0);
                        ad1 = mfma_16x16x4(a2[u][1], bd[u], ad1);
                        s2 += a3[u];
                    }
                }
            }
        }
        if (first) {
#pragma unroll
            for (int t = 0; t < 2; ++t) {
                if constexpr (PA) { s1[t] += __shfl_xor(s1[t], 16, 64); s1[t] += __shfl_xor(s1[t], 32, 64); }
                if constexpr (PB) { s2[t] += __shfl_xor(s2[t], 16, 64); s2[t] += __shfl_xor(s2[t], 32, 64); }
            }
        }
        float* slot = red + (wave & 7) * 1088;
        __syncthreads();
#pragma unroll
        for (int round = 0; round < 2; ++round) {
            if ((wave >> 3) == round) {
#pragma unroll
                for (int r = 0; r < 4; ++r) {
                    const int jl = 2 * (4 * q + r);
                    if (round == 0) {
                        if constexpr (PA) {
                            slot[(jl + 0) * 16 + c] = ax0[r];
                            slot[(jl + 1) * 16 + c] = ax1[r];
                        }
                        if constexpr (PB) {
                            if (first) {
                                slot[512 + (jl + 0) * 16 + c] = ad0[r];
                                slot[512 + (jl + 1) * 16 + c] = ad1[r];
                            }
                        }
                    } else {
                        if constexpr (PA) {
                            slot[(jl + 0) * 16 + c] += ax0[r];
                            slot[(jl + 1) * 16 + c] += ax1[r];
                        }
                        if constexpr (PB) {
                            if (first) {
                                slot[512 + (jl + 0) * 16 + c] += ad0[r];
                                slot[512 + (jl + 1) * 16 + c] += ad1[r];
                            }
                        }
                    }
                }
                if (first && q == 0) {
                    if (round == 0) {
                        if constexpr (PA) { slot[1024 + 2 * c] = s1[0]; slot[1024 + 2 * c + 1] = s1[1]; }
                        if constexpr (PB) { slot[1056 + 2 * c] = s2[0]; slot[1056 + 2 * c + 1] = s2[1]; }
                    } else {
                        if constexpr (PA) { slot[1024 + 2 * c] += s1[0]; slot[1024 + 2 * c + 1] += s1[1]; }
                        if constexpr (PB) { slot[1056 + 2 * c] += s2[0]; slot[1056 + 2 * c + 1] += s2[1]; }
                    }
                }
            }
            __syncthreads();
        }
        {
            const int e = tid & 511;
            float v = 0.0f;
            const int off = (tid < 512) ? e : 512 + e;
            if ((PA && tid < 512) || (PB && tid >= 512)) {
#pragma unroll
                for (int w = 0; w < 8; ++w) v += red[w * 1088 + off];
            }
            const int jl = e >> 4, kk = e & 15;
            if (tid < 512) {
                if constexpr (PA) {
                    if (k0 + kk < Do) {
                        const int gi = no.W1 + (j0 + jl) * Do + k0 + kk;
                        wp.grad[gi] = v;
                        sq = fmaf(v, v, sq);
                        if constexpr (FUSE) ppo_adam_elem(wp, sa, gi, v);
                    }
                }
            } else if (PB && first && kk < out) {
                const int gi = no.W3 + kk * H + j0 + jl;
                wp.grad[gi] = v;
                sq = fmaf(v, v, sq);
                if constexpr (FUSE) ppo_adam_elem(wp, sa, gi, v);
            }
            if (first && ((PA && tid < 32) || (PB && tid >= 32 && tid < 64))) {
                float bsum = 0.0f;
#pragma unroll
                for (int w = 0; w < 8; ++w) bsum += red[w * 1088 + 1024 + tid];
                const int gi = (tid < 32) ? no.b1 + j0 + tid : no.b2 + j0 + tid - 32;
                wp.grad[gi] = bsum;
                sq = fmaf(bsum, bsum, sq);
                if constexpr (FUSE) ppo_adam_elem(wp, sa, gi, bsum);
            }
        }
    }
}

template <int H, bool BIG, bool FUSE, int U = WG_MAXU>
__device__ __forceinline__ void ppo_wgrad_body(const ModelDesc& md, const WgradPtrs& wp, const int mbp,
                                               const PpoStepArgs& sa, const int n_stat_tiles) {
    const int CH = BIG ? (mbp + 64 * U - 1) / (64 * U) : 1;
    constexpr int TPD = H / 32;
    constexpr int NT2 = TPD * TPD;
    constexpr int NA = H / 32;
    constexpr int PB = NT2 + 2 * NA;
    static_assert(PB == wg_blocks_per_net(H), "host and device agree on the grid");
    __shared__ float red[1024 * 9];
    __shared__ float wsum[16];
    const int tid = threadIdx.x, lane = tid & 63, wave = tid >> 6;
    if (FSRL_PROBE(sa, 20)) return;
    if ((int)blockIdx.x >= md.n_nets * PB) {
        ppo_wgrad_extra_block<BIG, FUSE>(md, wp, mbp, sa, n_stat_tiles, red, (int)blockIdx.x - md.n_nets * PB);
        return;
    }
    const int net = blockIdx.x / PB, rb = blockIdx.x % PB;
    const NetOff no = md.net[net];
    const size_t nb = (size_t)net * wp.mbp_max;
    const float* __restrict__ A1 = wp.A1 + nb * H;
    const float* __restrict__ A2 = wp.A2 + nb * H;
    const float* __restrict__ D1 = wp.D1 + nb * H;
    const float* __restrict__ D2 = wp.D2 + nb * H;
    const float* __restrict__ DOb = wp.DO + nb * FSRL_DOW;
    float sq = 0.0f;

    if (FSRL_PROBE(sa, 23)) return;
    if (FSRL_PROBE(sa, 21) && rb >= NT2) return;
    if (FSRL_PROBE(sa, 22) && rb < NT2) return;
    if (rb < NT2) {
        const int tj = rb / TPD, tk = rb % TPD;
        const int c = lane & 15, q = lane >> 4;
        const float* __restrict__ pa = D2 + tj * 32 + 2 * c;
        const float* __restrict__ pb = A1 + tk * 32 + 2 * c;
        const int KS = mbp >> 2;
        f32x4 acc00 = {0, 0, 0, 0}, acc01 = {0, 0, 0, 0}, acc10 = {0, 0, 0, 0}, acc11 = {0, 0, 0, 0};
        for (int ch = 0; ch < CH; ++ch) {
            int s0 = 16 * U * ch;
            if constexpr (BIG) asm volatile("" : "+s"(s0));
            f32x2 a[U], b[U];
#pragma unroll
            for (int u = 0; u < U; ++u) {
                const int s = s0 + wave + 16 * u;
                if (s < KS) {
                    const size_t r = (size_t)(4 * s + q) * H;
                    a[u] = *reinterpret_cast<const f32x2*>(pa + r);
                    b[u] = *reinterpret_cast<const f32x2*>(pb + r);
                } else {
                    a[u] = f32x2{0.f, 0.f};
                    b[u] = f32x2{0.f, 0.f};
                }
            }
#pragma unroll
            for (int u = 0; u < U; ++u) {
                if (s0 + wave + 16 * u < KS) {
                    acc00 = mfma_16x16x4(a[u][0], b[u][0], acc00);
                    acc01 = mfma_16x16x4(a[u][0], b[u][1], acc01);
                    acc10 = mfma_16x16x4(a[u][1], b[u][0], acc10);
                    acc11 = mfma_16x16x4(a[u][1], b[u][1], acc11);
                }
            }
        }
        float* myred = red + (wave & 7) * (32 * 33);
        if (wave < 8) {
#pragma unroll
            for (int r = 0; r < 4; ++r) {
                const int jl = 2 * (4 * q + r);
                myred[(jl + 0) * 33 + 2 * c + 0] = acc00[r];
                myred[(jl + 0) * 33 + 2 * c + 1] = acc01[r];
                myred[(jl + 1) * 33 + 2 * c + 0] = acc10[r];
                myred[(jl + 1) * 33 + 2 * c + 1] = acc11[r];
            }
        }
        __syncthreads();
        if (wave >= 8) {
#pragma unroll
            for (int r = 0; r < 4; ++r) {
                const int jl = 2 * (4 * q + r);
                myred[(jl + 0) * 33 + 2 * c + 0] += acc00[r];
                myred[(jl + 0) * 33 + 2 * c + 1] += acc01[r];
                myred[(jl + 1) * 33 + 2 * c + 0] += acc10[r];
                myred[(jl + 1) * 33 + 2 * c + 1] += acc11[r];
            }
        }
        __syncthreads();
        {
            const int jl = tid >> 5, kl = tid & 31;
            float v = 0.0f;
#pragma unroll
            for (int w = 0; w < 8; ++w) v += red[w * (32 * 33) + jl * 33 + kl];
            const int gi = no.W2 + (tj * 32 + jl) * H + tk * 32 + kl;
            wp.grad[gi] = v;
            sq = v * v;
            if constexpr (FUSE)
                ppo_adam_elem(wp, sa, gi, v, no.W2f + w2f_index(H, tj * 32 + jl, tk * 32 + kl));
        }
    } else if (rb < NT2 + NA) {
        ppo_wgrad_aux<H, BIG, FUSE, U, true, false>(md, wp, mbp, sa, no, A2, D1, D2, DOb, (rb - NT2) * 32, red, sq);
    } else {
        ppo_wgrad_aux<H, BIG, FUSE, U, false, true>(md, wp, mbp, sa, no, A2, D1, D2, DOb, (rb - NT2 - NA) * 32, red, sq);
    }
    sq = wave_sum(sq);
    __syncthreads();
    if (lane == 0) wsum[wave] = sq;
    __syncthreads();
    if (tid == 0) {
        float t = 0.0f;
#pragma unroll
        for (int w = 0; w < 16; ++w) t += wsum[w];
        wp.gsq_part[blockIdx.x] = t;
    }
}

__global__ __launch_bounds__(64) void ppo_stats_kernel(const ModelDesc md, const WgradPtrs wp, const PpoStepArgs sa,
                                                      const int n_stat_tiles) {
    ppo_stats_finalize(md, wp, sa, n_stat_tiles, (int)threadIdx.x);
}

template <int H, bool BIG, bool FUSE>
__global__ __launch_bounds__(1024) void ppo_wgrad_kernel(const ModelDesc md, const WgradPtrs wp,
                                                        const int mbp, const PpoStepArgs sa,
                                                        const int n_stat_tiles) {
    ppo_wgrad_body<H, BIG, FUSE>(md, wp, mbp, sa, n_stat_tiles);
}

struct GroupHyper {
    double kl_thresh;
    float eps_clip, dual_clip, vf_coef, max_grad_norm, target_kl;
    int norm_adv, use_lagrangian, value_clip;
    float beta1, beta2, adam_eps, one_minus_b1, one_minus_b2;
    int pad;
};
struct GroupAgent {
    const float* P;
    float *Pw, *M, *V, *G;
    PpoBatchPtrs bp;
    WgradPtrs wp;
    const float* gsq_part; CtrlBlock* ctrl;
    float rescale; float lam[FSRL_MAX_CRITICS];
    int n_dev, nparts;
    GroupHyper hp;
};
struct GroupStep {
    int mb_start, mb_size, step, mb_index;
    int first_in_pass, last_in_pass, iters_in_pass, active;
    int pass; float step_size, bc2_sqrt; int pad;
};
__device__ __forceinline__ PpoStepArgs group_step_args(const PpoStepArgs& base, const GroupAgent& a, const GroupStep& st) {
    PpoStepArgs sa = base;
    sa.mb_start = st.mb_start; sa.mb_size = st.mb_size; sa.step = st.step; sa.mb_index = st.mb_index;
    sa.first_in_pass = st.first_in_pass; sa.last_in_pass = st.last_in_pass; sa.iters_in_pass = st.iters_in_pass;
    sa.pass = st.pass; sa.step_size = st.step_size; sa.bc2_sqrt = st.bc2_sqrt;
    sa.rescale = a.rescale;
#pragma unroll
    for (int i = 0; i < FSRL_MAX_CRITICS; ++i) sa.lam[i] = a.lam[i];
    const GroupHyper& h = a.hp;
    sa.eps_clip = h.eps_clip; sa.dual_clip = h.dual_clip; sa.vf_coef = h.vf_coef; sa.max_grad_norm = h.max_grad_norm;
    sa.target_kl = h.target_kl; sa.kl_thresh = h.kl_thresh;
    sa.norm_adv = h.norm_adv; sa.use_lagrangian = h.use_lagrangian; sa.value_clip = h.value_clip;
    sa.beta1 = h.beta1; sa.beta2 = h.beta2; sa.adam_eps = h.adam_eps;
    sa.one_minus_b1 = h.one_minus_b1; sa.one_minus_b2 = h.one_minus_b2;
    return sa;
}

template <int H, int R>
__global__ __launch_bounds__(4 * H) void ppo_fwd_bwd_group_kernel(const ModelDesc md, const GroupAgent* __restrict__ tab,
                                                                 const GroupStep* __restrict__ steps,
                                                                 const PpoStepArgs base) {
    __shared__ TileSmem<H> sm;
    const GroupStep st = steps[blockIdx.y];
    if (!st.active) return;
    const GroupAgent& a = tab[blockIdx.y];
    const PpoStepArgs sa = group_step_args(base, a, st);
    ppo_fwd_bwd_body<H, R>(sm, a.P, md, a.bp, sa);
}

template <int H>
__global__ __launch_bounds__(4 * H) void ppo_fwd_bwd_group_mix_kernel(const ModelDesc md, const GroupAgent* __restrict__ tab,
                                                                     const GroupStep* __restrict__ steps, const PpoStepArgs base,
                                                                     const int n32, const int per_net) {
    __shared__ __align__(16) unsigned char raw[sizeof(TileSmem<H, 32>)];
    const GroupStep st = steps[blockIdx.y];
    if (!st.active) return;
    const GroupAgent& a = tab[blockIdx.y];
    const PpoStepArgs sa = group_step_args(base, a, st);
    ppo_fwd_bwd_mixed<H>(raw, a.P, md, a.bp, sa, n32, per_net);
}

template <int H, bool BIG, bool FUSE, int R>
__global__ __launch_bounds__(1024, BIG ? 4 : 8) void ppo_wgrad_group_kernel(const ModelDesc md, const GroupAgent* __restrict__ tab,
                                                              const GroupStep* __restrict__ steps,
                                                              const PpoStepArgs base) {
    const GroupStep st = steps[blockIdx.y];
    if (!st.active) return;
    const GroupAgent& a = tab[blockIdx.y];
    const PpoStepArgs sa = group_step_args(base, a, st);
    WgradPtrs wp = a.wp;
    wp.X = a.bp.obs_p + (size_t)st.mb_start * md.Do;
    const int tiles = (st.mb_size + 15) >> 4;
    ppo_wgrad_body<H, BIG, FUSE, BIG ? WG_MAXU : 4>(md, wp, tiles * 16, sa, tiles * (16 / R));
}

__global__ __launch_bounds__(ADAM_NT) void adam_clip_group_kernel(const ModelDesc md, const GroupAgent* __restrict__ tab,
                                                                 const GroupStep* __restrict__ steps,
                                                                 const PpoStepArgs base) {
    const GroupStep st = steps[blockIdx.y];
// ... 6 lines not shown
```

### fsrl_amd/engine.py

```python
import ctypes as C
from dataclasses import dataclass
from typing import Optional, Sequence

import numpy as np

from . import _lib

_f32p, _f64p = C.POINTER(C.c_float), C.POINTER(C.c_double)
_u8p, _i32p, _i64p = C.POINTER(C.c_uint8), C.POINTER(C.c_int32), C.POINTER(C.c_int64)


def _ptr(a, t):
    return a.ctypes.data_as(t) if a is not None else None


@dataclass
class EngineConfig:
    obs_dim: int = 8
    act_dim: int = 2
    hidden: int = 128
    hidden_sizes: Optional[Sequence[int]] = None
    force_layered: bool = False
    n_critics: int = 2
    env_num: int = 20
# ... 355 lines not shown
        st = None if state is None else np.ascontiguousarray(state, np.float32)
        tt = None if t is None else np.ascontiguousarray(t, np.int32)
        od = None if ordinal is None else np.ascontiguousarray(ordinal, np.int64)
        _lib.check(self.lib.fsrl_devenv_set_state(h, _ptr(st, _f32p), _ptr(tt, _i32p), _ptr(od, _i64p)))

    def collect_device(self, h, n_episode, deterministic=False, bound_method=1, low=None, high=None, max_steps_per_launch=0):
        lo = np.ascontiguousarray(low, np.float32) if low is not None else None
        hi = np.ascontiguousarray(high, np.float32) if low is not None else None
        steps, cost = C.c_int64(), C.c_double()
        nt, ntr, nep, nl = C.c_int32(), C.c_int32(), C.c_int32(), C.c_int32()
        ep_rew, ep_len = np.zeros(max(int(n_episode), 1), np.float64), np.zeros(max(int(n_episode), 1), np.int32)
        _lib.check(self.lib.fsrl_collect_device(
            self._ctx, h, int(n_episode), int(bool(deterministic)), int(bound_method), _ptr(lo, _f32p), _ptr(hi, _f32p),
            int(max_steps_per_launch), C.byref(steps), C.byref(cost), C.byref(nt), C.byref(ntr), _ptr(ep_rew, _f64p),
            _ptr(ep_len, _i32p), C.byref(nep), C.byref(nl)))
        k = nep.value
        return dict(steps=int(steps.value), total_cost=float(cost.value), terminated=int(nt.value), truncated=int(ntr.value),
                    ep_rews=ep_rew[:k], ep_lens=ep_len[:k], launches=int(nl.value))

    def actor_set_resident(self, on=True, idle_timeout_us=0.0):
        _lib.check(self.lib.fsrl_actor_set_resident(self._ctx, int(bool(on)), float(idle_timeout_us)))

    def actor_release(self):
        self.lib.fsrl_actor_release(self._ctx)

    def actor_resident_stats(self):
        out = np.zeros(3, np.int64)
        _lib.check(self.lib.fsrl_actor_resident_stats(self._ctx, _ptr(out, _i64p)))
        return dict(launches=int(out[0]), requests=int(out[1]), live=bool(out[2]))

    def store_sizes(self, n=None):
        n = self.cfg.env_num if n is None else int(n)
        out = np.empty(n, np.int64)
        _lib.check(self.lib.fsrl_store_sizes(self._ctx, _ptr(out, _i64p), n))
        return out

    def focops_init(self, actor_lr=5e-4, critic_lr=1e-3, l2_reg=1e-3, delta=0.02, eta=0.02, tem_lambda=0.95,
                    max_grad_norm=0.5):
        cfg = _lib.FocopsConfig(actor_lr, critic_lr, l2_reg, delta, eta, tem_lambda, float(max_grad_norm or 0.0))
        _lib.check(self.lib.fsrl_focops_init(self._ctx, C.byref(cfg)))

    def focops_set_plan(self, four_launch: int = 0):
        _lib.check(self.lib.fsrl_focops_set_plan(self._ctx, int(four_launch)))

    def focops_update(self, nu, nu_loss, batch_size, repeat, perms=None, seed=0):
        _lib.check(self.lib.fsrl_focops_set_nu(self._ctx, float(nu), float(nu_loss)))
        stats, stopped = self.ppo_update([0.0], 1.0, batch_size, repeat, perms=perms, seed=seed)
        return stats[:, :_lib.FOCOPS_NSTATS], stopped

    def ppo_begin(self, lagrangians: Sequence[float], rescaling: float, batch_size: int) -> int:
        lag = np.ascontiguousarray(lagrangians, np.float64).reshape(-1)
        n = C.c_int64()
        _lib.check(self.lib.fsrl_ppo_begin(self._ctx, _ptr(lag, _f64p) if lag.size else None,
                                           float(rescaling), int(batch_size), C.byref(n)))
        self._n = n.value
        return n.value

    def ppo_pass(self, perm=None, seed: int = 0, wait: bool = True) -> bool:
        stopped = C.c_int32()
        if perm is not None:
            perm = np.ascontiguousarray(perm, np.int64)
            assert perm.size == self._n, "permutation length != batch length"
        _lib.check(self.lib.fsrl_ppo_pass(self._ctx, _ptr(perm, _i64p), int(seed), C.byref(stopped) if wait else None))
        return bool(stopped.value)

    def ppo_pass_result(self) -> bool:
        stopped = C.c_int32()
        _lib.check(self.lib.fsrl_ppo_pass_result(self._ctx, C.byref(stopped)))
        return bool(stopped.value)

    def ppo_end(self):
        n = C.c_int64()
        _lib.check(self.lib.fsrl_ppo_end(self._ctx, None, 0, C.byref(n)))
        return n.value

    def ppo_end_stats(self, max_steps: int):
        n = C.c_int64()
        out = np.empty((max(max_steps, 1), _lib.PPO_NSTATS), np.float32)
        _lib.check(self.lib.fsrl_ppo_end(self._ctx, _ptr(out, _f32p), out.shape[0], C.byref(n)))
        return out[:n.value]

    def ppo_set_plan(self, tall_tiles: int = -1):
        _lib.check(self.lib.fsrl_ppo_set_plan(self._ctx, int(tall_tiles)))

    def ppo_update(self, lagrangians, rescaling, batch_size, repeat, perms=None, seed=0):
        n = self.ppo_begin(lagrangians, rescaling, batch_size)
        stopped_pass = -1
        steps_per_pass = max(1, -(-n // max(batch_size, 1)))
        try:
            for k in range(repeat):
                if self.ppo_pass(None if perms is None else perms[k], seed + k if seed else 0):
                    stopped_pass = k
                    break
            stats = self.ppo_end_stats(steps_per_pass * max(repeat, 1))
        except BaseException:
            self.ppo_abort()
            raise
        return stats, stopped_pass

    def batch_get(self, which: str):
        n = self._n
        cols = 1 if which == "logp_old" else self.cfg.n_critics
        out = np.empty((n, cols), np.float32)
        _lib.check(self.lib.fsrl_batch_get(self._ctx, which.encode(), _ptr(out, _f32p), out.size))
        return out[:, 0] if which == "logp_old" else out

    def gae_return(self, v, v_next, rew, end_flag, gamma, gae_lambda):
        v = np.ascontiguousarray(v, np.float32); v_next = np.ascontiguousarray(v_next, np.float32)
        rew = np.ascontiguousarray(rew, np.float64)
        end = np.ascontiguousarray(end_flag).astype(np.uint8)
        out = np.empty(rew.size, np.float64)
        _lib.check(self.lib.fsrl_gae_return(self._ctx, _ptr(v, _f32p), _ptr(v_next, _f32p),
                                            _ptr(rew, _f64p), _ptr(end, _u8p), rew.size, float(gamma),
                                            float(gae_lambda), _ptr(out, _f64p)))
        return out

    def launch_floors(self, mb_rows=256, iters=200):
        out = np.zeros(4, np.float64)
        _lib.check(self.lib.fsrl_launch_floors(self._ctx, int(mb_rows), int(iters), _ptr(out, _f64p)))
        return dict(zip(("fwdbwd", "wgrad", "adam", "triple"), out.tolist()))

    def nstep_return(self, metric, end_flag, target_q, indices, gamma, n_step):
        metric = np.ascontiguousarray(metric, np.float64)
        end = np.ascontiguousarray(end_flag).astype(np.uint8)
        tq = np.ascontiguousarray(target_q, np.float32)
        shape = tq.shape
        bsz = shape[0] if tq.ndim else 0
        tq2 = tq.reshape(bsz, -1) if bsz else tq.reshape(0, 1)
        idx = np.ascontiguousarray(indices, np.int64).reshape(int(n_step), bsz) if n_step >= 1 else np.zeros((0, bsz), np.int64)
        out = np.empty(tq2.shape, np.float64)
        _lib.check(self.lib.fsrl_nstep_return(self._ctx, _ptr(metric, _f64p), _ptr(end, _u8p), metric.size,
                                              _ptr(tq2, _f32p), _ptr(idx, _i64p), bsz, tq2.shape[1], float(gamma),
                                              int(n_step), _ptr(out, _f64p)))
        return out.reshape(shape)

    def tr_begin(self, target_kl=0.01, backtrack_coeff=0.8, damping=0.1, l2_reg=0.0, critic_lr=1e-3,
                 max_backtracks=10, optim_critic_iters=10, cg_iters=10, norm_adv=True,
                 cost_limit=float("inf")) -> int:
        cfg = _lib.TrConfig(target_kl, backtrack_coeff, damping, l2_reg, critic_lr, max_backtracks,
                            optim_critic_iters, cg_iters, int(norm_adv),
                            cost_limit if np.isfinite(cost_limit) else 1e300)
        n = C.c_int64()
        _lib.check(self.lib.fsrl_tr_begin(self._ctx, C.byref(cfg), C.byref(n)))
        self._n = n.value
        return n.value

    @property
    def n_actor_params(self) -> int:
        return int(self.lib.fsrl_actor_param_count(self._ctx))

    def tr_linesearch_evals(self, cap=64):
        out = np.zeros(cap, np.int32)
        n = int(self.lib.fsrl_tr_linesearch_evals(self._ctx, _ptr(out, _i32p), cap))
        return out[:n]

    def tr_grad(self, which: int):
        out = np.empty(self.n_actor_params, np.float32)
        _lib.check(self.lib.fsrl_tr_grad(self._ctx, int(which), _ptr(out, _f32p), out.size))
        return out

    def tr_hvp(self, v):
        v = np.ascontiguousarray(v, np.float32)
        out = np.empty_like(v)
        _lib.check(self.lib.fsrl_tr_hvp(self._ctx, _ptr(v, _f32p), _ptr(out, _f32p), v.size))
        return out

# ... 584 lines not shown
```

### include/fsrl_hip.h

```cpp
#ifndef FSRL_HIP_H
#define FSRL_HIP_H

#include <stdint.h>

#ifdef __cplusplus
extern "C" {
#endif

#define FSRL_OK 0
#define FSRL_EINVAL (-22)
#define FSRL_ENOMEM (-12)
#define FSRL_EHIP (-5)
#define FSRL_ESTATE (-1)

#define FSRL_ALGO_PPO_LAG 0
#define FSRL_ALGO_TRPO_LAG 1
#define FSRL_ALGO_CPO 2
#define FSRL_ALGO_SAC_LAG 3
#define FSRL_ALGO_FOCOPS 4

#define FSRL_MAX_CRITICS 4
#define FSRL_MAX_HIDDEN 8
#define FSRL_MAX_WIDTH 4096
#define FSRL_PPO_NSTATS 11
// ... 44 lines not shown
int fsrl_optim_reset(fsrl_ctx* ctx);
int fsrl_state_snapshot(fsrl_ctx* ctx);
int fsrl_state_restore(fsrl_ctx* ctx);
int64_t fsrl_train_state_size(fsrl_ctx* ctx, int32_t with_store);
int fsrl_train_state_export(fsrl_ctx* ctx, int32_t with_store, void* out, int64_t cap, int64_t* written);
int fsrl_train_state_import(fsrl_ctx* ctx, const void* blob, int64_t n);
int fsrl_train_state_copy(fsrl_ctx* dst, fsrl_ctx* src, int32_t with_store);
int fsrl_ret_rms_get(fsrl_ctx* ctx, double* out, int32_t n);
int fsrl_ret_rms_set(fsrl_ctx* ctx, const double* in, int32_t n);
int fsrl_set_lr(fsrl_ctx* ctx, int32_t group, float lr);
float fsrl_get_lr(const fsrl_ctx* ctx, int32_t group);

int fsrl_store_push(fsrl_ctx* ctx, const int32_t* env_ids, int32_t k, const float* obs,
                    const float* act, const double* rew, const double* cost,
                    const uint8_t* terminated, const uint8_t* truncated,
                    const float* obs_next, int64_t* ptr_out, double* ep_rew_out,
                    int32_t* ep_len_out, int64_t* ep_idx_out);
int fsrl_store_reset(fsrl_ctx* ctx, int keep_statistics);
int64_t fsrl_store_len(const fsrl_ctx* ctx);
int fsrl_store_read(fsrl_ctx* ctx, const int64_t* indices, int64_t n, float* obs_out, float* act_out, double* rew_out,
                    double* cost_out, uint8_t* terminated_out, uint8_t* truncated_out, float* obs_next_out);
int fsrl_store_configure(fsrl_ctx* ctx, int64_t total_size, int32_t buffer_num);
int fsrl_store_geometry(const fsrl_ctx* ctx, int64_t* sub_size_out, int32_t* buffer_num_out);
int fsrl_store_sample0(fsrl_ctx* ctx, int64_t* indices_out, int64_t cap, int64_t* n_out);

int fsrl_actor_forward(fsrl_ctx* ctx, const float* obs, int32_t k, float* mu_out,
                       float* sigma_out);
int fsrl_actor_sample(fsrl_ctx* ctx, const float* obs, int32_t k, int32_t deterministic, uint64_t seed,
                      float* act_out);
int fsrl_collect_step(fsrl_ctx* ctx, const int32_t* env_ids, int32_t k, const float* obs, const float* act,
                      const double* rew, const double* cost, const uint8_t* terminated, const uint8_t* truncated,
                      const float* obs_next, int64_t* ptr_out, double* ep_rew_out, int32_t* ep_len_out,
                      int64_t* ep_idx_out, const float* obs_act, int32_t k_act, int32_t deterministic,
                      int32_t bound_method, const float* act_low, const float* act_high, float* act_out,
                      float* env_act_out);
typedef struct fsrl_shm_env {
    float* obs;
    float* act;
    double* rew; double* cost;
    uint8_t* term; uint8_t* trunc; uint8_t* active;
    uint32_t* hs;
    uint32_t* want;
    const int32_t* owner;
    const int32_t* lane_of_worker;
    int32_t env_num, obs_dim, act_dim, workers, n_lanes;
    uint32_t gen[2];
    uint32_t spin;
    const uint32_t* err;
    const int32_t* pids;
} fsrl_shm_env;
int fsrl_collect_run(fsrl_ctx* ctx, fsrl_shm_env* env, const int32_t* ready, int32_t n, float* obs, float* act,
                     float* env_act, int32_t deterministic, int32_t bound_method, const float* act_low,
                     const float* act_high, int32_t max_steps, int32_t* steps_out, double* cost_sum_out, double* rew_out,
                     double* cost_out, uint8_t* term_out, uint8_t* trunc_out, float* obs_next_out);
int fsrl_collect_episodes(fsrl_ctx* ctx, fsrl_shm_env* env, const int32_t* ready, int32_t n, const float* obs, int32_t n_episode,
                          int32_t deterministic, int32_t bound_method, const float* act_low, const float* act_high,
                          int64_t* steps_out, double* total_cost_out, int32_t* term_count_out, int32_t* trunc_count_out,
                          double* ep_rew_out, int32_t* ep_len_out, int32_t* episodes_out);

int fsrl_collect_episodes_split(fsrl_ctx* ctx, fsrl_shm_env* env, const int32_t* ready, int32_t n, const float* obs, int32_t n_episode,
                                int32_t deterministic, int32_t bound_method, const float* act_low, const float* act_high,
                                int64_t* steps_out, double* total_cost_out, int32_t* term_count_out, int32_t* trunc_count_out,
                                double* ep_rew_out, int32_t* ep_len_out, int32_t* episodes_out);
int fsrl_collect_timing(fsrl_ctx* ctx, double* out2);
int fsrl_actor_set_resident(fsrl_ctx* ctx, int32_t on, double idle_timeout_us);
int fsrl_actor_resident_stats(fsrl_ctx* ctx, int64_t* out3);
int fsrl_actor_release(fsrl_ctx* ctx);

int fsrl_store_sizes(const fsrl_ctx* ctx, int64_t* sizes_out, int32_t n);

int fsrl_ppo_begin(fsrl_ctx* ctx, const double* lagrangians, double rescaling,
                   int32_t batch_size, int64_t* n_out);
int fsrl_ppo_pass(fsrl_ctx* ctx, const int64_t* perm, uint64_t seed, int32_t* stopped_out);
int fsrl_ppo_pass_result(fsrl_ctx* ctx, int32_t* stopped_out);
int fsrl_ppo_end(fsrl_ctx* ctx, float* stats_out, int64_t cap_steps, int64_t* n_steps_out);
int fsrl_ppo_abort(fsrl_ctx* ctx);
int fsrl_ppo_update(fsrl_ctx* ctx, const double* lagrangians, double rescaling,
                    int32_t batch_size, int32_t repeat, const int64_t* perms, uint64_t seed,
                    float* stats_out, int64_t cap_steps, int64_t* n_steps_out,
                    int32_t* stopped_pass_out);

int fsrl_ppo_set_plan(fsrl_ctx* ctx, int32_t tall_tiles);

typedef struct fsrl_group fsrl_group;
int fsrl_group_create(fsrl_ctx** ctxs, int32_t k, fsrl_group** out);
int fsrl_group_destroy(fsrl_group* group);
int fsrl_group_set_plan(fsrl_group* group, int32_t tall_tiles);
int fsrl_group_ppo_update(fsrl_group* group, const double* lagrangians, const double* rescaling, int32_t batch_size,
                          int32_t repeat, const int64_t* const* perms, uint64_t seed, float* const* stats_out,
                          int64_t cap_steps, int64_t* n_steps_out, int32_t* stopped_pass_out);
int fsrl_group_ppo_update_each(fsrl_group* group, const double* lagrangians, const double* rescaling, const int32_t* batch_sizes,
                               const int32_t* repeats, const int64_t* const* perms, uint64_t seed, float* const* stats_out,
                               const int64_t* cap_steps, int64_t* n_steps_out, int32_t* stopped_pass_out);
int fsrl_group_collect_step(fsrl_group* group, const int32_t* k, const int32_t* env_ids, const float* obs, const float* act,
                            const double* rew, const double* cost, const uint8_t* terminated, const uint8_t* truncated,
                            const float* obs_next, int64_t* ptr_out, double* ep_rew_out, int32_t* ep_len_out,
                            int64_t* ep_idx_out, const int32_t* k_act, const float* obs_act, int32_t deterministic,
                            int32_t bound_method, const float* act_low, const float* act_high, float* act_out,
                            float* env_act_out);
int fsrl_group_actor_set_resident(fsrl_group* group, int32_t on, double idle_timeout_us);
int fsrl_group_actor_resident_stats(fsrl_group* group, int64_t* out3);
int fsrl_group_actor_release(fsrl_group* group);

int fsrl_batch_get(fsrl_ctx* ctx, const char* which, float* out, int64_t cap);

int fsrl_gae_return(fsrl_ctx* ctx, const float* v, const float* v_next, const double* rew,
                    const uint8_t* end_flag, int64_t n, double gamma, double gae_lambda,
                    double* adv_out);

int fsrl_nstep_return(fsrl_ctx* ctx, const double* metric, const uint8_t* end_flag, int64_t len,
                      const float* target_q, const int64_t* indices, int64_t bsz, int64_t q, double gamma,
                      int32_t n_step, double* out);

typedef struct fsrl_tr_config {
    float target_kl;
    float backtrack_coeff;
    float damping;
    float l2_reg;
    float critic_lr;
    int32_t max_backtracks;
    int32_t optim_critic_iters;
    int32_t cg_iters;
    int32_t norm_adv;
    double cost_limit;
} fsrl_tr_config;

#define FSRL_CPO_NSTATS 17
#define FSRL_TRPO_NSTATS 11

int fsrl_tr_begin(fsrl_ctx* ctx, const fsrl_tr_config* cfg, int64_t* n_out);
int fsrl_cpo_learn(fsrl_ctx* ctx, double ave_cost_return, int32_t repeat, float* stats_out);
int fsrl_trpo_learn(fsrl_ctx* ctx, const double* lagrangians, double rescaling, int32_t repeat,
                    float* stats_out);
int fsrl_cpo_learn_mb(fsrl_ctx* ctx, double ave_cost_return, int32_t repeat, int32_t batch_size, const int64_t* perms,
                      uint64_t seed, float* stats_out, int64_t cap_rows, int64_t* n_rows_out);
int fsrl_trpo_learn_mb(fsrl_ctx* ctx, const double* lagrangians, double rescaling, int32_t repeat, int32_t batch_size,
                       const int64_t* perms, uint64_t seed, float* stats_out, int64_t cap_rows, int64_t* n_rows_out);
int32_t fsrl_tr_linesearch_evals(fsrl_ctx* ctx, int32_t* out, int32_t cap);
int64_t fsrl_actor_param_count(const fsrl_ctx* ctx);
int fsrl_tr_grad(fsrl_ctx* ctx, int32_t which, float* out, int64_t n);
int fsrl_tr_hvp(fsrl_ctx* ctx, const float* v, float* out, int64_t n);
int fsrl_tr_hvp_cached(fsrl_ctx* ctx, const float* v, float* out, int64_t n);
int fsrl_tr_cg(fsrl_ctx* ctx, const float* rhs, int64_t n, float damping, int32_t nsteps, float tol, float* x_out,
               int32_t* iters_out, float* rs_out);
int fsrl_tr_eval(fsrl_ctx* ctx, double* stats8);
int fsrl_tr_set_plan(fsrl_ctx* ctx, int32_t tile_rows, int32_t hvp, int32_t wgrad);
int fsrl_tr_set_tile_split(fsrl_ctx* ctx, int32_t n32_tile, int32_t n32_hvp);
int fsrl_tr_set_co_delay(fsrl_ctx* ctx, int32_t tile_periods, int32_t hvp_periods);

typedef struct fsrl_focops_config {
    float actor_lr, critic_lr;
    float l2_reg;
    float delta;
    float eta;
    float tem_lambda;
    float max_grad_norm;
} fsrl_focops_config;
#define FSRL_FOCOPS_NSTATS 8
int fsrl_focops_init(fsrl_ctx* ctx, const fsrl_focops_config* cfg);
int fsrl_focops_set_plan(fsrl_ctx* ctx, int32_t four_launch);
int fsrl_focops_set_nu(fsrl_ctx* ctx, double nu, double nu_loss);

typedef struct fsrl_sac_config {
    float actor_lr, critic_lr, alpha_lr;
    float tau;
    float alpha;
// ... 153 lines not shown
```

Baseline: 133.9 updates/s.

## Fuse grad-norm clipping and Adam into wgrad kernel via cross-block exchange

Adds a CLIP variant of the weight-gradient kernel. Each block holds its pending gradients in registers, exchanges partial squared norms with the other blocks through global slots using an epoch and a bounded spin, then applies the clip coefficient and Adam in place, which removes the separate adam_clip_kernel launch per minibatch. The cross-block wait is only safe when every block is co-resident, so the host snapshots params and Adam state at the start of each update. If a block times out and the control block is marked poisoned, the host restores the snapshot and replays the recorded permutations on the unfused path, which adds snapshot copies and a costly fallback.

```diff
diff --git a/fsrl_amd/_lib.py b/fsrl_amd/_lib.py
--- a/fsrl_amd/_lib.py
+++ b/fsrl_amd/_lib.py
@@ -117,6 +117,8 @@
     "fsrl_ppo_update": (C.c_int, [_ctx, _d, C.c_double, C.c_int32, C.c_int32, _i64, C.c_uint64, _f,
                                   C.c_int64, _i64, _i32]),
     "fsrl_ppo_set_plan": (C.c_int, [_ctx, C.c_int32]),
+    "fsrl_ppo_set_clip_fuse": (C.c_int, [_ctx, C.c_int32, C.c_int32]),
+    "fsrl_ppo_clip_fuse_stats": (C.c_int, [_ctx, _i64, _f]),
     "fsrl_batch_get": (C.c_int, [_ctx, C.c_char_p, _f, C.c_int64]),
     "fsrl_group_create": (C.c_int, [_P(_ctx), C.c_int32, _P(_ctx)]),
     "fsrl_group_destroy": (C.c_int, [_ctx]),
diff --git a/fsrl_amd/csrc/common.hpp b/fsrl_amd/csrc/common.hpp
--- a/fsrl_amd/csrc/common.hpp
+++ b/fsrl_amd/csrc/common.hpp
@@ -69,6 +69,8 @@
     int fuse_adam;
     int xcd_pair;
     int dbg_phase;
+    unsigned clip_epoch;
+    int clip_limit;
 };
 #ifdef FSRL_PROBES
 #define FSRL_PROBE(sa, n) ((sa).dbg_phase == (n))
@@ -89,7 +91,7 @@
 
 struct CtrlBlock {
     int stopped_after;
-    int pad;
+    int poisoned;
     double kl_sum;
     float last_grad_norm;
     float pad2;
diff --git a/fsrl_amd/csrc/fsrl_hip.hip b/fsrl_amd/csrc/fsrl_hip.hip
--- a/fsrl_amd/csrc/fsrl_hip.hip
+++ b/fsrl_amd/csrc/fsrl_hip.hip
@@ -12,6 +12,7 @@
 #include <string>
 #include <vector>
 
+#include <atomic>
 #include "kernels_misc.hpp"
 #include "kernels_mlp.hpp"
 #include "kernels_fb.hpp"
@@ -167,6 +168,18 @@
     int tall_tiles = -1;
     bool no_fuse_adam = false;
     bool no_w2b_early = false;
+    bool counted_live = false;
+    int clip_fuse_mode = -1;
+    int clip_fuse_limit = CLIP_FUSE_DEFAULT_TICKS;
+    bool no_clip_fuse = false;
+    bool clip_fuse_dead = false;
+    bool clip_fuse_active = false;
+    int64_t clip_fuse_fallbacks = 0, clip_fuse_steps = 0;
+    unsigned clip_epoch = 0;
+    unsigned long long* clip_slots = nullptr;
+    float* clip_snap = nullptr;
+    int64_t clip_snap_adam_t = 0;
+    std::vector<std::vector<int>> clip_perms;
     bool no_xcd_pair = false;
     bool no_spin = false;
     std::vector<float> act_mu, act_sg;
@@ -434,6 +447,8 @@
     }
 }
 
+static std::atomic<int> g_live_ctx[64];
+static int live_contexts_on(int device) { return (device >= 0 && device < 64) ? g_live_ctx[device].load() : 2; }
 extern "C" int fsrl_ctx_destroy(fsrl_ctx* c) {
     if (!c) return 0;
     (void)hipSetDevice(c->device);
@@ -459,6 +474,8 @@
     if (c->mu_old) (void)hipFree(c->mu_old);
     if (c->sigma_old) (void)hipFree(c->sigma_old);
     if (c->snap) (void)hipFree(c->snap);
+    if (c->clip_snap) (void)hipFree(c->clip_snap);
+    if (c->clip_slots) (void)hipFree(c->clip_slots);
     void* dptrs[] = {c->P, c->M, c->V, c->G, c->ctrl, c->st.obs, c->st.obs_next, c->st.act, c->st.rew,
                      c->st.cost, c->st.flags, c->b.obs, c->b.obs_next, c->b.act, c->b.rew, c->b.cost,
                      c->b.flags, c->d_indices, c->d_end, c->d_seg, c->values, c->vnext, c->advs,
@@ -478,6 +495,7 @@
     for (hipEvent_t e : c->k_ev) (void)hipEventDestroy(e);
     if (c->compute) (void)hipStreamDestroy(c->compute);
     if (c->side) (void)hipStreamDestroy(c->side);
+    if (c->counted_live && c->device >= 0 && c->device < 64) g_live_ctx[c->device].fetch_sub(1);
     delete c;
     return 0;
 }
@@ -538,9 +556,11 @@
     c->cfg.hidden = Hpad_;
     c->h1 = h1_; c->h2 = h2_;
     c->device = device_id;
+    if (device_id >= 0 && device_id < 64) { g_live_ctx[device_id].fetch_add(1); c->counted_live = true; }
     c->n_cus = n_cus_probe > 0 ? n_cus_probe : 256;
     c->probe_tile16 = getenv("FSRL_TILE16") != nullptr;
     c->no_w2b_early = getenv("FSRL_NO_W2B_EARLY") != nullptr;
+    c->no_clip_fuse = getenv("FSRL_NO_CLIP_FUSE") != nullptr;
 #ifdef FSRL_PROBES
     { const char* e = getenv("FSRL_DBG_PHASE"); c->probe_phase = e ? atoi(e) : 0; }
     { const char* e = getenv("FSRL_WGRAD_SKIP"); c->probe_wgrad_skip = e ? atoi(e) : 0; }
diff --git a/fsrl_amd/csrc/host_decisions.hpp b/fsrl_amd/csrc/host_decisions.hpp
--- a/fsrl_amd/csrc/host_decisions.hpp
+++ b/fsrl_amd/csrc/host_decisions.hpp
@@ -137,3 +137,32 @@
     const int64_t rem = N - 32 * (int64_t)n32;
     *n32_out = n32; *n16_out = (int)((rem + 15) / 16);
 }
+
+static constexpr int CLIP_FUSE_DEFAULT_TICKS = 5000;
+static constexpr int CLIP_FUSE_MAX_OBS = 64;
+struct ClipFuseFacts {
+    int mode;
+    bool env_off;
+    bool dead;
+    bool ppo_lag, layered, grouped;
+    bool recompute_adv, rew_norm;
+    float max_grad_norm;
+    int nparts, n_cus;
+    int obs_dim;
+    int live_contexts;
+};
+static inline bool clip_fuse_update_ok(const ClipFuseFacts& f) {
+    if (f.mode == 0 || f.env_off || f.dead) return false;
+    if (f.mode < 0 && f.live_contexts > 1) return false;
+    if (!f.ppo_lag || f.layered || f.grouped) return false;
+    if (!(f.max_grad_norm > 0.0f)) return false;
+    if (f.recompute_adv || f.rew_norm) return false;
+    if (f.nparts > f.n_cus || f.nparts > 1024) return false;
+    return f.obs_dim <= CLIP_FUSE_MAX_OBS;
+}
+static inline bool clip_fuse_step_ok(bool update_ok, int rows_pad) { return update_ok && rows_pad <= 512; }
+static inline bool clip_fuse_must_replay(bool active, int poisoned) { return active && poisoned != 0; }
+struct ClipFuseReplay { long long adam_t, n_steps; int pass_index, passes; };
+static inline ClipFuseReplay clip_fuse_replay_plan(long long snap_adam_t, int passes_enqueued) {
+    return {snap_adam_t, 0, 0, passes_enqueued};
+}
diff --git a/fsrl_amd/csrc/host_ppo.inc b/fsrl_amd/csrc/host_ppo.inc
--- a/fsrl_amd/csrc/host_ppo.inc
+++ b/fsrl_amd/csrc/host_ppo.inc
@@ -1,9 +1,14 @@
 static int launch_gae(fsrl_ctx* c);
+static int perm_send(fsrl_ctx* c, int n);
+static int clip_fuse_begin(fsrl_ctx* c);
 static int perm_upload(fsrl_ctx* c, int n, const int64_t* perm, uint64_t seed) {
     c->perm_tmp.resize((size_t)n);
     const PermFill pf = perm_fill(c->perm_tmp.data(), n, perm, c->shuffle_rng, seed);
     CHECK_ARG(pf.code != PERM_RANGE, "perm[%d]=%lld out of range", pf.index, pf.value);
     CHECK_ARG(pf.code != PERM_TWICE, "perm is not a permutation: %lld appears twice", pf.value);
+    return perm_send(c, n);
+}
+static int perm_send(fsrl_ctx* c, int n) {
     if (c->perm_in_flight) { HIPCHK(hipEventSynchronize(c->perm_copied)); c->perm_in_flight = false; }
     memcpy(c->h_perm, c->perm_tmp.data(), (size_t)n * 4);
     HIPCHK(hipMemcpyAsync(c->d_perm, c->h_perm, (size_t)n * 4, hipMemcpyHostToDevice, c->compute));
@@ -67,7 +72,11 @@
     *c->h_ctrl = init;
     hipStream_t s = c->compute;
     HIPCHK(hipMemcpyAsync(c->ctrl, c->h_ctrl, sizeof(CtrlBlock), hipMemcpyHostToDevice, s));
+    c->clip_fuse_active = false;
+    c->clip_perms.clear();
     if (n == 0) { c->batch_ready = true; return 0; }
+    rc = clip_fuse_begin(c);
+    if (rc) return rc;
     int nseg = 0;
     c->h_seg[nseg++] = 0;
     for (int64_t i = 0; i + 1 < n; ++i) if (c->h_end[i]) c->h_seg[nseg++] = (int)i + 1;
@@ -179,7 +188,7 @@
     return 0;
 }
 
-static int ppo_pass_prepare(fsrl_ctx* c, const int64_t* perm, uint64_t seed) {
+static int ppo_pass_prepare(fsrl_ctx* c, const int64_t* perm, uint64_t seed, const std::vector<int>* kept = nullptr) {
     const int n = (int)c->N;
     hipStream_t s = c->compute;
     const int C = c->cfg.n_critics;
@@ -188,8 +197,11 @@
         int rc0 = ppo_recompute_advantages(c);
         if (rc0) return rc0;
     }
-    int rc = perm_upload(c, n, perm, seed);
-    if (rc) return rc;
+    int rc;
+    if (kept) { c->perm_tmp = *kept; rc = perm_send(c, n); }
+    else rc = perm_upload(c, n, perm, seed);
+    if (rc) return rc;
+    if (c->clip_fuse_active && !kept) c->clip_perms.push_back(c->perm_tmp);
     const int nmb = (int)c->mb_start.size();
     rc = ensure_stats(c, c->n_steps + nmb);
     if (rc) return rc;
@@ -280,6 +292,7 @@
     return p;
 }
 
+static int ppo_pass_enqueue(fsrl_ctx* c, const int64_t* perm, uint64_t seed, const std::vector<int>* kept);
 extern "C" int fsrl_ppo_pass(fsrl_ctx* c, const int64_t* perm, uint64_t seed, int32_t* stopped_out) {
     CHECK_ARG(c, "null ctx");
     if (!c->in_update || !c->batch_ready) return fail(FSRL_ESTATE, "fsrl_ppo_pass before fsrl_ppo_begin");
@@ -288,23 +301,35 @@
     if (stopped_out) *stopped_out = 0;
     const int n = (int)c->N;
     if (n == 0) return 0;
-    hipStream_t s = c->compute;
-    const int H = c->cfg.hidden, nn = c->md.n_nets;
-    int rc = ppo_pass_prepare(c, perm, seed);
-    if (rc) return rc;
-    const int nmb = (int)c->mb_start.size();
-    if (c->cfg.algo == FSRL_ALGO_FOCOPS) return focops_pass(c, stopped_out);
+    int rc;
+    if (c->cfg.algo == FSRL_ALGO_FOCOPS || c->lay) {
+        rc = ppo_pass_prepare(c, perm, seed);
+        if (rc) return rc;
+        if (c->cfg.algo == FSRL_ALGO_FOCOPS) return focops_pass(c, stopped_out);
+    }
     if (c->lay) {
         rc = lay_ppo_steps(c);
         if (rc) return rc;
-        c->n_steps += nmb;
+        c->n_steps += (int)c->mb_start.size();
         c->pass_index += 1;
         if (c->cfg.target_kl > 0.0f) return pass_verdict(c, stopped_out);
         return 0;
     }
+    rc = ppo_pass_enqueue(c, perm, seed, nullptr);
+    if (rc) return rc;
+    if (c->cfg.target_kl > 0.0f) return pass_verdict(c, stopped_out);
+    return 0;
+}
+static int ppo_pass_enqueue(fsrl_ctx* c, const int64_t* perm, uint64_t seed, const std::vector<int>* kept) {
+    hipStream_t s = c->compute;
+    const int H = c->cfg.hidden, nn = c->md.n_nets;
+    int rc = ppo_pass_prepare(c, perm, seed, kept);
+    if (rc) return rc;
+    const int nmb = (int)c->mb_start.size();
     const PpoBatchPtrs bp = ppo_batch_ptrs(c);
     WgradPtrs wp = ppo_wgrad_ptrs(c);
     wp.stats = c->d_stats;
+    wp.clip_slots = c->clip_slots;
     const int nparts = wg_grid(H, nn);
 
     PpoStepArgs sa = ppo_base_args(c);
@@ -350,6 +375,13 @@
             c->k_ev_used += 3;
         }
         const bool big = tiles * 16 > 512;
+        const bool clip_step = clip_fuse_step_ok(c->clip_fuse_active, tiles * 16);
+        if (clip_step) {
+            c->clip_epoch += 1;
+            if (c->clip_epoch == 0) c->clip_epoch = 1;
+            sa.clip_epoch = c->clip_epoch; sa.clip_limit = c->clip_fuse_limit;
+            c->clip_fuse_steps += 1;
+        }
         if (big) {
             FbWgradArgs wa{};
             wgrad_fill_nets(wa, nn, 0, (size_t)H, (size_t)c->mbp_max, c->A1, c->A2, c->D1, c->D2, c->DO);
@@ -369,18 +401,88 @@
         rc = dispatch_H(H, [&](auto hc) {
             constexpr int HH = decltype(hc)::value;
             if (sa.fuse_adam) hipLaunchKernelGGL((ppo_wgrad_kernel<HH, false, true>), dim3(nparts), dim3(1024), 0, s, c->md, wp, tiles * 16, sa, stat_tiles);
+            else if (clip_step) hipLaunchKernelGGL((ppo_wgrad_kernel<HH, false, true, true>), dim3(nparts), dim3(1024), 0, s, c->md, wp, tiles * 16, sa, stat_tiles);
             else hipLaunchKernelGGL((ppo_wgrad_kernel<HH, false, false>), dim3(nparts), dim3(1024), 0, s, c->md, wp, tiles * 16, sa, stat_tiles);
             return 0;
         });
         if (rc) return rc;
-        if (!sa.fuse_adam)
+        if (!sa.fuse_adam && !clip_step)
             hipLaunchKernelGGL(adam_clip_kernel, dim3((c->n_dev + 4 * ADAM_NT - 1) / (4 * ADAM_NT)), dim3(ADAM_NT), 0, s, c->P, c->M, c->V, c->G,
                                c->gsq_part, nparts, c->n_dev, sa, c->ctrl, c->md);
         HIPCHK(hipGetLastError());
     }
     c->n_steps += nmb;
     c->pass_index += 1;
-    if (c->cfg.target_kl > 0.0f) return pass_verdict(c, stopped_out);
+    return 0;
+}
+
+static int clip_fuse_begin(fsrl_ctx* c) {
+    ClipFuseFacts f{};
+    f.mode = c->clip_fuse_mode; f.env_off = c->no_clip_fuse; f.dead = c->clip_fuse_dead;
+    f.ppo_lag = c->cfg.algo == FSRL_ALGO_PPO_LAG; f.layered = c->lay != nullptr; f.grouped = c->group != nullptr;
+    f.recompute_adv = c->cfg.recompute_adv != 0; f.rew_norm = c->cfg.rew_norm != 0;
+    f.max_grad_norm = c->cfg.max_grad_norm;
+    f.nparts = c->lay ? 0 : wg_grid(c->cfg.hidden, c->md.n_nets); f.n_cus = c->n_cus; f.obs_dim = c->cfg.obs_dim;
+    f.live_contexts = live_contexts_on(c->device);
+    if (!clip_fuse_update_ok(f)) return 0;
+    hipStream_t s = c->compute;
+    if (!c->clip_slots) {
+        HIPCHK(hipMalloc(&c->clip_slots, (size_t)1024 * CLIP_SLOT_STRIDE * sizeof(unsigned long long)));
+        HIPCHK(hipMemsetAsync(c->clip_slots, 0, (size_t)1024 * CLIP_SLOT_STRIDE * sizeof(unsigned long long), s));
+    }
+    if (!c->clip_snap) HIPCHK(hipMalloc(&c->clip_snap, ((size_t)c->n_alloc + 2 * (size_t)c->n_dev) * 4));
+    HIPCHK(hipMemcpyAsync(c->clip_snap, c->P, (size_t)c->n_alloc * 4, hipMemcpyDeviceToDevice, s));
+    HIPCHK(hipMemcpyAsync(c->clip_snap + c->n_alloc, c->M, (size_t)c->n_dev * 4, hipMemcpyDeviceToDevice, s));
+    HIPCHK(hipMemcpyAsync(c->clip_snap + c->n_alloc + c->n_dev, c->V, (size_t)c->n_dev * 4, hipMemcpyDeviceToDevice, s));
+    c->clip_snap_adam_t = c->adam_t;
+    c->clip_fuse_active = true;
+    return 0;
+}
+static int clip_fuse_check(fsrl_ctx* c) {
+    if (!clip_fuse_must_replay(c->clip_fuse_active, c->h_ctrl->poisoned)) return 0;
+    hipStream_t s = c->compute;
+    const ClipFuseReplay rp = clip_fuse_replay_plan(c->clip_snap_adam_t, c->pass_index);
+    c->clip_fuse_active = false; c->clip_fuse_dead = true;
+    c->clip_fuse_fallbacks += 1;
+    HIPCHK(hipMemcpyAsync(c->P, c->clip_snap, (size_t)c->n_alloc * 4, hipMemcpyDeviceToDevice, s));
+    HIPCHK(hipMemcpyAsync(c->M, c->clip_snap + c->n_alloc, (size_t)c->n_dev * 4, hipMemcpyDeviceToDevice, s));
+    HIPCHK(hipMemcpyAsync(c->V, c->clip_snap + c->n_alloc + c->n_dev, (size_t)c->n_dev * 4, hipMemcpyDeviceToDevice, s));
+    c->adam_t = rp.adam_t; c->n_steps = rp.n_steps; c->pass_index = rp.pass_index;
+    c->k_ev_used = 0;
+    CtrlBlock init{INT_MAX, 0, 0.0, 0.0f, 0.0f};
+    *c->h_ctrl = init;
+    HIPCHK(hipMemcpyAsync(c->ctrl, c->h_ctrl, sizeof(CtrlBlock), hipMemcpyHostToDevice, s));
+    HIPCHK(hipStreamSynchronize(s));
+    for (int k = 0; k < rp.passes; ++k) {
+        int rc = ppo_pass_enqueue(c, nullptr, 0, &c->clip_perms[(size_t)k]);
+        if (rc) return rc;
+    }
+    HIPCHK(hipMemcpyAsync(c->h_ctrl, c->ctrl, sizeof(CtrlBlock), hipMemcpyDeviceToHost, s));
+    HIPCHK(hipStreamSynchronize(s));
+    c->clip_perms.clear();
+    return 0;
+}
+extern "C" int fsrl_ppo_set_clip_fuse(fsrl_ctx* c, int32_t mode, int32_t limit_ticks) {
+    CHECK_ARG(c, "null ctx");
+    CHECK_ARG(mode >= -1 && mode <= 1, "mode: -1 (automatic), 0 (off) or 1 (on)");
+    CHECK_ARG(limit_ticks <= 100000000, "limit_ticks: at most 10^8 (one second)");
+    CHECK_ARG(!c->in_update, "fsrl_ppo_set_clip_fuse inside an update");
+    c->clip_fuse_mode = mode;
+    c->clip_fuse_limit = limit_ticks < 0 ? CLIP_FUSE_DEFAULT_TICKS : limit_ticks;
+    return 0;
+}
+extern "C" int fsrl_ppo_clip_fuse_stats(fsrl_ctx* c, int64_t* out, float* grad_norm_out) {
+    CHECK_ARG(c && out, "null argument");
+    if (grad_norm_out) {
+        CHECK_ARG(!c->in_update, "the gradient norm is read between updates");
+        ENTER_DEV(c);
+        CtrlBlock cb;
+        HIPCHK(hipStreamSynchronize(c->compute));
+        HIPCHK(hipMemcpy(&cb, c->ctrl, sizeof(CtrlBlock), hipMemcpyDeviceToHost));
+        *grad_norm_out = cb.last_grad_norm;
+    }
+    out[0] = (c->clip_fuse_mode != 0 && !c->no_clip_fuse && !c->clip_fuse_dead) ? 1 : 0;
+    out[1] = c->clip_fuse_fallbacks; out[2] = c->clip_fuse_steps; out[3] = c->clip_fuse_active ? 1 : 0;
     return 0;
 }
 
@@ -388,6 +490,8 @@
     HIPCHK(hipMemcpyAsync(c->h_ctrl, c->ctrl, sizeof(CtrlBlock), hipMemcpyDeviceToHost, c->compute));
     if (!stopped_out) { c->verdict_pending = true; return 0; }
     HIPCHK(hipStreamSynchronize(c->compute));
+    int rc = clip_fuse_check(c);
+    if (rc) return rc;
     if (c->h_ctrl->stopped_after != INT_MAX) *stopped_out = 1;
     return 0;
 }
@@ -396,7 +500,11 @@
     CHECK_ARG(c && stopped_out, "null argument");
     if (!c->in_update) return fail(FSRL_ESTATE, "fsrl_ppo_pass_result outside an update");
     ENTER_DEV(c);
-    if (c->verdict_pending) { HIPCHK(hipStreamSynchronize(c->compute)); c->verdict_pending = false; }
+    if (c->verdict_pending) {
+        HIPCHK(hipStreamSynchronize(c->compute)); c->verdict_pending = false;
+        int rc = clip_fuse_check(c);
+        if (rc) return rc;
+    }
     const bool watched = c->cfg.target_kl > 0.0f || c->cfg.algo == FSRL_ALGO_FOCOPS;
     *stopped_out = (watched && c->pass_index > 0 && c->h_ctrl->stopped_after != INT_MAX) ? 1 : 0;
     return 0;
@@ -408,6 +516,8 @@
     ENTER_DEV(c);
     hipStream_t s = c->compute;
     HIPCHK(hipEventRecord(c->ev_c, s));
+    const bool look = c->clip_fuse_active;
+    if (look) HIPCHK(hipMemcpyAsync(c->h_ctrl, c->ctrl, sizeof(CtrlBlock), hipMemcpyDeviceToHost, s));
     if (stats_out && c->n_steps > 0) {
         CHECK_ARG(cap_steps >= c->n_steps, "stats_out holds %lld steps, need %lld", (long long)cap_steps,
                   (long long)c->n_steps);
@@ -415,6 +525,18 @@
                               hipMemcpyDeviceToHost, s));
     }
     HIPCHK(hipStreamSynchronize(s));
+    if (look) {
+        c->verdict_pending = false;
+        const int64_t before = c->clip_fuse_fallbacks;
+        int rc = clip_fuse_check(c);
+        if (rc) { c->in_update = false; return rc; }
+        if (c->clip_fuse_fallbacks != before) {
+            HIPCHK(hipEventRecord(c->ev_c, s));
+            if (stats_out && c->n_steps > 0)
+                HIPCHK(hipMemcpyAsync(stats_out, c->d_stats, (size_t)c->n_steps * FSRL_PPO_NSTATS * 4, hipMemcpyDeviceToHost, s));
+            HIPCHK(hipStreamSynchronize(s));
+        }
+    }
     if (n_steps_out) *n_steps_out = c->n_steps;
     c->in_update = false;
     if (c->N > 0) {
diff --git a/fsrl_amd/csrc/kernels_misc.hpp b/fsrl_amd/csrc/kernels_misc.hpp
--- a/fsrl_amd/csrc/kernels_misc.hpp
+++ b/fsrl_amd/csrc/kernels_misc.hpp
@@ -255,6 +255,26 @@
 #ifndef ADAM_NT
 #define ADAM_NT 256
 #endif
+__device__ __forceinline__ void clip_coef_from_parts(const float* __restrict__ parts, const int nparts, const float max_norm,
+                                                     double* sh, float* out) {
+    const int tid = threadIdx.x;
+    if (tid < ADAM_NT) {
+        double s = 0.0;
+        for (int k = tid; k < nparts; k += ADAM_NT) s += (double)parts[k];
+        s = wave_sum_d(s);
+        if ((tid & 63) == 0) sh[tid >> 6] = s;
+    }
+    __syncthreads();
+    if (tid == 0) {
+        double tot = 0.0;
+        for (int w = 0; w < ADAM_NT / 64; ++w) tot += sh[w];
+        const float norm = sqrtf((float)tot);
+        out[0] = fminf(max_norm / (norm + 1e-6f), 1.0f);
+        out[1] = norm;
+    }
+    __syncthreads();
+}
+
 __device__ __forceinline__ void adam_clip_body(float* __restrict__ P, float* __restrict__ M,
                                                float* __restrict__ V,
                                                const float* __restrict__ G,
@@ -262,7 +282,7 @@
                                                int n, const PpoStepArgs& sa,
                                                CtrlBlock* ctrl, const ModelDesc& md) {
     __shared__ double sh[ADAM_NT / 64];
-    __shared__ float coef_s;
+    __shared__ float coef_s[2];
     const int tid = threadIdx.x;
     if (FSRL_PROBE(sa, 30)) return;
     const int i4 = (blockIdx.x * ADAM_NT + tid) * 4;
@@ -273,20 +293,9 @@
     }
     float coef = 1.0f;
     if (sa.max_grad_norm > 0.0f) {
-        double s = 0.0;
-        for (int k = tid; k < nparts; k += ADAM_NT) s += (double)gsq_part[k];
-        s = wave_sum_d(s);
-        if ((tid & 63) == 0) sh[tid >> 6] = s;
-        __syncthreads();
-        if (tid == 0) {
-            double tot = 0.0;
-            for (int w = 0; w < ADAM_NT / 64; ++w) tot += sh[w];
-            const float norm = sqrtf((float)tot);
-            coef_s = fminf(sa.max_grad_norm / (norm + 1e-6f), 1.0f);
-            if (blockIdx.x == 0) ctrl->last_grad_norm = norm;
-        }
-        __syncthreads();
-        coef = coef_s;
+        clip_coef_from_parts(gsq_part, nparts, sa.max_grad_norm, sh, coef_s);
+        coef = coef_s[0];
+        if (blockIdx.x == 0 && tid == 0) ctrl->last_grad_norm = coef_s[1];
     }
     if (i4 < n) {
 #pragma unroll
diff --git a/fsrl_amd/csrc/kernels_mlp.hpp b/fsrl_amd/csrc/kernels_mlp.hpp
--- a/fsrl_amd/csrc/kernels_mlp.hpp
+++ b/fsrl_amd/csrc/kernels_mlp.hpp
@@ -952,7 +952,68 @@
     int mbp_max;
     float* Pw; float* M; float* V;
     float* gsq_net;
+    unsigned long long* clip_slots;
 };
+
+#define CLIP_SLOT_STRIDE 16
+#define CLIP_NP 5
+struct ClipPend {
+    int i[CLIP_NP];
+    float g[CLIP_NP], m[CLIP_NP], v[CLIP_NP], p[CLIP_NP];
+    int mi;
+};
+template <int S>
+__device__ __forceinline__ void clip_pend_load(ClipPend& cp, const WgradPtrs& wp, const int gi) {
+    cp.i[S] = gi; cp.g[S] = 0.0f; cp.m[S] = 0.0f; cp.v[S] = 0.0f; cp.p[S] = 0.0f;
+    if (gi >= 0) { cp.m[S] = wp.M[gi]; cp.v[S] = wp.V[gi]; cp.p[S] = wp.Pw[gi]; }
+}
+__device__ __forceinline__ bool clip_exchange(const WgradPtrs& wp, const PpoStepArgs& sa, const float part, float* vals,
+                                              const bool reports, float& coef) {
+    __shared__ double sh[ADAM_NT / 64];
+    __shared__ float out[2];
+    __shared__ int bail;
+    const int tid = threadIdx.x, nparts = (int)gridDim.x;
+    if (tid == 0) {
+        bail = sa.clip_limit <= 0 ? 1 : 0;
+        __hip_atomic_store(wp.clip_slots + (size_t)blockIdx.x * CLIP_SLOT_STRIDE,
+                           ((unsigned long long)sa.clip_epoch << 32) | (unsigned long long)__float_as_uint(part), __ATOMIC_RELAXED,
+                           __HIP_MEMORY_SCOPE_AGENT);
+    }
+    __syncthreads();
+    if (tid < nparts && sa.clip_limit > 0) {
+        const unsigned long long* slot = wp.clip_slots + (size_t)tid * CLIP_SLOT_STRIDE;
+        const long long t0 = wall_clock64();
+        unsigned long long w;
+        while (true) {
+            w = __hip_atomic_load(slot, __ATOMIC_RELAXED, __HIP_MEMORY_SCOPE_AGENT);
+            if ((unsigned)(w >> 32) == sa.clip_epoch) break;
+            if (wall_clock64() - t0 > (long long)sa.clip_limit ||
+                __hip_atomic_load(&wp.ctrl->poisoned, __ATOMIC_RELAXED, __HIP_MEMORY_SCOPE_AGENT) != 0) { bail = 1; break; }
+            __builtin_amdgcn_s_sleep(1);
+        }
+        vals[tid] = __uint_as_float((unsigned)w);
+    }
+    __syncthreads();
+    if (bail) {
+        if (tid == 0) __hip_atomic_store(&wp.ctrl->poisoned, 1, __ATOMIC_RELAXED, __HIP_MEMORY_SCOPE_AGENT);
+        return false;
+    }
+    clip_coef_from_parts(vals, nparts, sa.max_grad_norm, sh, out);
+    coef = out[0];
+    if (reports && tid == 0) wp.ctrl->last_grad_norm = out[1];
+    return true;
+}
+__device__ __forceinline__ void clip_pend_apply(const ClipPend& cp, const WgradPtrs& wp, const PpoStepArgs& sa, const float coef) {
+#pragma unroll
+    for (int s = 0; s < CLIP_NP; ++s) {
+        if (cp.i[s] >= 0) {
+            float m = cp.m[s], v = cp.v[s], p = cp.p[s];
+            ppo_adam_math(cp.g[s] * coef, m, v, p, sa);
+            wp.M[cp.i[s]] = m; wp.V[cp.i[s]] = v; wp.Pw[cp.i[s]] = p;
+            if (s == 0 && cp.mi >= 0) wp.Pw[cp.mi] = p;
+        }
+    }
+}
 
 __device__ __forceinline__ void ppo_adam_elem(const WgradPtrs& wp, const PpoStepArgs& sa, const int i, const float g,
                                               const int mi = -1) {
@@ -1020,9 +1081,9 @@
     }
 }
 
-template <bool BIG, bool FUSE>
+template <bool BIG, bool FUSE, bool CLIP = false>
 __device__ __forceinline__ void ppo_wgrad_extra_block(const ModelDesc& md, const WgradPtrs& wp, const int mbp, const PpoStepArgs& sa,
-                                                      const int n_stat_tiles, float* red, const int e) {
+                                                      const int n_stat_tiles, float* red, const int e, ClipPend& cp, float& part) {
     const int CH = BIG ? (mbp + 511) / 512 : 1;
     const int tid = threadIdx.x, lane = tid & 63, wave = tid >> 6;
     if (FSRL_PROBE(sa, 21)) return;
@@ -1036,6 +1097,7 @@
     }
     if (e == md.n_nets) {
         if (tid == 0) wp.gsq_part[blockIdx.x] = 0.0f;
+        part = 0.0f;
         return;
     }
     float sqs = 0.0f;
@@ -1044,6 +1106,10 @@
         const NetOff no = md.net[net];
         const float* __restrict__ DOn = wp.DO + (size_t)net * wp.mbp_max * FSRL_DOW;
         const int col = tid & 31, php = tid >> 5;
+        if constexpr (CLIP) {
+            clip_pend_load<0>(cp, wp, tid < no.out ? no.b3 + tid : -1);
+            clip_pend_load<1>(cp, wp, (no.sigma >= 0 && tid >= 16 && tid < 16 + md.Da) ? no.sigma + tid - 16 : -1);
+        }
         float t = 0.0f;
         for (int ch = 0; ch < CH; ++ch) {
             float v[16];
@@ -1066,11 +1132,13 @@
             for (int p2 = 0; p2 < 32; ++p2) tot += red[p2 * 33 + tid];
             if (tid < no.out) {
                 wp.grad[no.b3 + tid] = tot; sqs = fmaf(tot, tot, sqs);
-                if constexpr (FUSE) ppo_adam_elem(wp, sa, no.b3 + tid, tot);
+                if constexpr (CLIP) cp.g[0] = tot;
+                else if constexpr (FUSE) ppo_adam_elem(wp, sa, no.b3 + tid, tot);
             }
             if (no.sigma >= 0 && tid >= 16 && tid < 16 + md.Da) {
                 wp.grad[no.sigma + tid - 16] = tot; sqs = fmaf(tot, tot, sqs);
-                if constexpr (FUSE) ppo_adam_elem(wp, sa, no.sigma + tid - 16, tot);
+                if constexpr (CLIP) cp.g[1] = tot;
+                else if constexpr (FUSE) ppo_adam_elem(wp, sa, no.sigma + tid - 16, tot);
             }
         }
     }
@@ -1078,22 +1146,36 @@
         sqs = wave_sum(sqs);
         if (lane == 0) {
             wp.gsq_part[blockIdx.x] = sqs;
+            part = sqs;
             if (wp.gsq_net) wp.gsq_net[e] = sqs;
         }
     }
 }
 
-template <int H, bool BIG, bool FUSE, int U, bool PA, bool PB>
+template <int H, bool BIG, bool FUSE, int U, bool PA, bool PB, bool CLIP = false>
 __device__ __forceinline__ void ppo_wgrad_aux(const ModelDesc& md, const WgradPtrs& wp, const int mbp, const PpoStepArgs& sa,
                                               const NetOff& no, const float* __restrict__ A2, const float* __restrict__ D1,
                                               const float* __restrict__ D2, const float* __restrict__ DOb, const int j0,
-                                              float* red, float& sq) {
+                                              float* red, float& sq, ClipPend& cp) {
     const int CH = BIG ? (mbp + 64 * U - 1) / (64 * U) : 1;
     const int tid = threadIdx.x, lane = tid & 63, wave = tid >> 6;
     const int c = lane & 15, q = lane >> 4;
     const int Do = md.Do, out = no.out;
     const int KS = mbp >> 2;
     const float* __restrict__ X = wp.X;
+    if constexpr (CLIP) {
+        const int e = tid & 511, jl = e >> 4, kk = e & 15;
+        if constexpr (PA) {
+            clip_pend_load<0>(cp, wp, (tid < 512 && kk < Do) ? no.W1 + (j0 + jl) * Do + kk : -1);
+            clip_pend_load<1>(cp, wp, (tid < 512 && 16 + kk < Do) ? no.W1 + (j0 + jl) * Do + 16 + kk : -1);
+            clip_pend_load<2>(cp, wp, (tid < 512 && 32 + kk < Do) ? no.W1 + (j0 + jl) * Do + 32 + kk : -1);
+            clip_pend_load<3>(cp, wp, (tid < 512 && 48 + kk < Do) ? no.W1 + (j0 + jl) * Do + 48 + kk : -1);
+            clip_pend_load<4>(cp, wp, tid < 32 ? no.b1 + j0 + tid : -1);
+        }
+        if constexpr (PB)
+            clip_pend_load<0>(cp, wp, (tid >= 512 && kk < out) ? no.W3 + kk * H + j0 + jl
+                                                               : (tid >= 32 && tid < 64) ? no.b2 + j0 + tid - 32 : -1);
+    }
     for (int k0 = 0; k0 < (PA ? Do : 1); k0 += 16) {
         const bool first = (k0 == 0);
         f32x4 ax0 = {0, 0, 0, 0}, ax1 = {0, 0, 0, 0}, ad0 = {0, 0, 0, 0}, ad1 = {0, 0, 0, 0};
@@ -1207,14 +1289,18 @@
                         const int gi = no.W1 + (j0 + jl) * Do + k0 + kk;
                         wp.grad[gi] = v;
                         sq = fmaf(v, v, sq);
-                        if constexpr (FUSE) ppo_adam_elem(wp, sa, gi, v);
+                        if constexpr (CLIP) {
+                            const int it = k0 >> 4;
+                            if (it == 0) cp.g[0] = v; else if (it == 1) cp.g[1] = v; else if (it == 2) cp.g[2] = v; else cp.g[3] = v;
+                        } else if constexpr (FUSE) ppo_adam_elem(wp, sa, gi, v);
                     }
                 }
             } else if (PB && first && kk < out) {
                 const int gi = no.W3 + kk * H + j0 + jl;
                 wp.grad[gi] = v;
                 sq = fmaf(v, v, sq);
-                if constexpr (FUSE) ppo_adam_elem(wp, sa, gi, v);
+                if constexpr (CLIP) cp.g[0] = v;
+                else if constexpr (FUSE) ppo_adam_elem(wp, sa, gi, v);
             }
             if (first && ((PA && tid < 32) || (PB && tid >= 32 && tid < 64))) {
                 float bsum = 0.0f;
@@ -1223,13 +1309,14 @@
                 const int gi = (tid < 32) ? no.b1 + j0 + tid : no.b2 + j0 + tid - 32;
                 wp.grad[gi] = bsum;
                 sq = fmaf(bsum, bsum, sq);
-                if constexpr (FUSE) ppo_adam_elem(wp, sa, gi, bsum);
-            }
-        }
-    }
-}
-
-template <int H, bool BIG, bool FUSE, int U = WG_MAXU>
+                if constexpr (CLIP) { if (tid < 32) cp.g[4] = bsum; else cp.g[0] = bsum; }
+                else if constexpr (FUSE) ppo_adam_elem(wp, sa, gi, bsum);
+            }
+        }
+    }
+}
+
+template <int H, bool BIG, bool FUSE, int U = WG_MAXU, bool CLIP = false>
 __device__ __forceinline__ void ppo_wgrad_body(const ModelDesc& md, const WgradPtrs& wp, const int mbp,
                                                const PpoStepArgs& sa, const int n_stat_tiles) {
     const int CH = BIG ? (mbp + 64 * U - 1) / (64 * U) : 1;
@@ -1241,9 +1328,22 @@
     __shared__ float red[1024 * 9];
     __shared__ float wsum[16];
     const int tid = threadIdx.x, lane = tid & 63, wave = tid >> 6;
+    static_assert(!CLIP || (FUSE && !BIG), "the clip exchange belongs to the fused-Adam form of the one-burst kernel");
     if (FSRL_PROBE(sa, 20)) return;
+    ClipPend cp;
+    if constexpr (CLIP) {
+#pragma unroll
+        for (int s = 0; s < CLIP_NP; ++s) cp.i[s] = -1;
+        cp.mi = -1;
+    }
     if ((int)blockIdx.x >= md.n_nets * PB) {
-        ppo_wgrad_extra_block<BIG, FUSE>(md, wp, mbp, sa, n_stat_tiles, red, (int)blockIdx.x - md.n_nets * PB);
+        const int e = (int)blockIdx.x - md.n_nets * PB;
+        float part = 0.0f;
+        ppo_wgrad_extra_block<BIG, FUSE, CLIP>(md, wp, mbp, sa, n_stat_tiles, red, e, cp, part);
+        if constexpr (CLIP) {
+            float coef = 1.0f;
+            if (clip_exchange(wp, sa, part, red, e == 0, coef) && e < md.n_nets) clip_pend_apply(cp, wp, sa, coef);
+        }
         return;
     }
     const int net = blockIdx.x / PB, rb = blockIdx.x % PB;
@@ -1266,6 +1366,11 @@
         const float* __restrict__ pb = A1 + tk * 32 + 2 * c;
         const int KS = mbp >> 2;
         f32x4 acc00 = {0, 0, 0, 0}, acc01 = {0, 0, 0, 0}, acc10 = {0, 0, 0, 0}, acc11 = {0, 0, 0, 0};
+        if constexpr (CLIP) {
+            const int gi = no.W2 + (tj * 32 + (tid >> 5)) * H + tk * 32 + (tid & 31);
+            clip_pend_load<0>(cp, wp, gi);
+            cp.mi = no.W2f + w2f_index(H, tj * 32 + (tid >> 5), tk * 32 + (tid & 31));
+        }
         for (int ch = 0; ch < CH; ++ch) {
             int s0 = 16 * U * ch;
             if constexpr (BIG) asm volatile("" : "+s"(s0));
@@ -1323,23 +1428,28 @@
             const int gi = no.W2 + (tj * 32 + jl) * H + tk * 32 + kl;
             wp.grad[gi] = v;
             sq = v * v;
-            if constexpr (FUSE)
+            if constexpr (CLIP) cp.g[0] = v;
+            else if constexpr (FUSE)
                 ppo_adam_elem(wp, sa, gi, v, no.W2f + w2f_index(H, tj * 32 + jl, tk * 32 + kl));
         }
     } else if (rb < NT2 + NA) {
-        ppo_wgrad_aux<H, BIG, FUSE, U, true, false>(md, wp, mbp, sa, no, A2, D1, D2, DOb, (rb - NT2) * 32, red, sq);
+        ppo_wgrad_aux<H, BIG, FUSE, U, true, false, CLIP>(md, wp, mbp, sa, no, A2, D1, D2, DOb, (rb - NT2) * 32, red, sq, cp);
     } else {
-        ppo_wgrad_aux<H, BIG, FUSE, U, false, true>(md, wp, mbp, sa, no, A2, D1, D2, DOb, (rb - NT2 - NA) * 32, red, sq);
+        ppo_wgrad_aux<H, BIG, FUSE, U, false, true, CLIP>(md, wp, mbp, sa, no, A2, D1, D2, DOb, (rb - NT2 - NA) * 32, red, sq, cp);
     }
     sq = wave_sum(sq);
     __syncthreads();
     if (lane == 0) wsum[wave] = sq;
     __syncthreads();
+    float t = 0.0f;
     if (tid == 0) {
-        float t = 0.0f;
 #pragma unroll
         for (int w = 0; w < 16; ++w) t += wsum[w];
         wp.gsq_part[blockIdx.x] = t;
+    }
+    if constexpr (CLIP) {
+        float coef = 1.0f;
+        if (clip_exchange(wp, sa, t, red, false, coef)) clip_pend_apply(cp, wp, sa, coef);
     }
 }
 
@@ -1348,11 +1458,11 @@
     ppo_stats_finalize(md, wp, sa, n_stat_tiles, (int)threadIdx.x);
 }
 
-template <int H, bool BIG, bool FUSE>
+template <int H, bool BIG, bool FUSE, bool CLIP = false>
 __global__ __launch_bounds__(1024) void ppo_wgrad_kernel(const ModelDesc md, const WgradPtrs wp,
                                                         const int mbp, const PpoStepArgs sa,
                                                         const int n_stat_tiles) {
-    ppo_wgrad_body<H, BIG, FUSE>(md, wp, mbp, sa, n_stat_tiles);
+    ppo_wgrad_body<H, BIG, FUSE, WG_MAXU, CLIP>(md, wp, mbp, sa, n_stat_tiles);
 }
 
 struct GroupHyper {
diff --git a/fsrl_amd/engine.py b/fsrl_amd/engine.py
--- a/fsrl_amd/engine.py
+++ b/fsrl_amd/engine.py
@@ -461,6 +461,16 @@
 
     def ppo_set_plan(self, tall_tiles: int = -1):
         _lib.check(self.lib.fsrl_ppo_set_plan(self._ctx, int(tall_tiles)))
+
+    def ppo_set_clip_fuse(self, mode: int = -1, limit_ticks: int = -1):
+        _lib.check(self.lib.fsrl_ppo_set_clip_fuse(self._ctx, int(mode), int(limit_ticks)))
+
+    def ppo_clip_fuse_stats(self):
+        out = (C.c_int64 * 4)()
+        gn = C.c_float()
+        _lib.check(self.lib.fsrl_ppo_clip_fuse_stats(self._ctx, out, C.byref(gn)))
+        return dict(available=bool(out[0]), fallbacks=int(out[1]), steps=int(out[2]), last_update_fused=bool(out[3]),
+                    grad_norm=np.float32(gn.value))
 
     def ppo_update(self, lagrangians, rescaling, batch_size, repeat, perms=None, seed=0):
         n = self.ppo_begin(lagrangians, rescaling, batch_size)
diff --git a/include/fsrl_hip.h b/include/fsrl_hip.h
--- a/include/fsrl_hip.h
+++ b/include/fsrl_hip.h
@@ -150,6 +150,9 @@
 
 int fsrl_ppo_set_plan(fsrl_ctx* ctx, int32_t tall_tiles);
 
+int fsrl_ppo_set_clip_fuse(fsrl_ctx* ctx, int32_t mode, int32_t limit_ticks);
+int fsrl_ppo_clip_fuse_stats(fsrl_ctx* ctx, int64_t* out, float* grad_norm_out);
+
 typedef struct fsrl_group fsrl_group;
 int fsrl_group_create(fsrl_ctx** ctxs, int32_t k, fsrl_group** out);
 int fsrl_group_destroy(fsrl_group* group);
```

After: 141.8 updates/s (median of 6 runs). 5.9% higher.
